# kylewray/epic

Measured on AMD Instinct MI355X. Metric: cell_updates_per_s_log_harmonic_relax_8192sq, higher is better.
Workload: dtype f32

## Files before the change

### epic_amd/csrc/driver.h

```cpp
#pragma once
#include <hip/hip_runtime.h>
#include <stdio.h>
#include <stdlib.h>
#include <string.h>

#include <algorithm>
#include <atomic>
#include <chrono>
#include <condition_variable>
#include <functional>
#include <map>
#include <string>
#include <thread>
#include <vector>
#include <mutex>
#include <tuple>
#include <unordered_map>

#include "../../include/epic/epic_abi.h"
#include "../../include/epic_hip.h"
#include "driver_config.h"
#include "kernels.h"

namespace epic_drv __attribute__((visibility("hidden"))) {

using epic::Harmonic;

struct DeviceGuard {
    int prev = -1;
    DeviceGuard() { if (hipGetDevice(&prev) != hipSuccess) { (void)hipGetLastError(); prev = -1; } }
    ~DeviceGuard() { if (prev >= 0) (void)hipSetDevice(prev); }
};
struct Crew;

struct Track {
    uint32_t *wake = nullptr;
    int phase = 0, rpt = 0, force = 2;
    size_t tiles = 0;
    static constexpr size_t kL = epic_hip::kWakeListCount, kCS = epic_hip::kWakeCounterStride;
    uint32_t *counter(int set) const { return wake + kL * kCS * set; }
    unsigned long long *total() const { return reinterpret_cast<unsigned long long *>(wake + 3 * kL * kCS); }
    uint32_t *queued(int i) const { return wake + 3 * kL * kCS + 2 + (size_t)i * tiles; }
    uint32_t *list(int i) const { return wake + 3 * kL * kCS + 2 + 2 * tiles + (size_t)i * kL * epic_hip::sweep_2d_list_cap(tiles); }
    static size_t words(size_t tiles) { return 3 * kL * kCS + 2 + 2 * tiles + 2 * kL * epic_hip::sweep_2d_list_cap(tiles); }
    static size_t zeroed_words(size_t tiles) { return 3 * kL * kCS + 2 + 2 * tiles; }
    void release()
    {
        if (wake) (void)hipFree(wake);
        wake = nullptr;
        tiles = 0;
    }
    epic_hip::Activity next(size_t tiles_now, int rpt_now, hipStream_t stream, bool *changed)
    {
        epic_hip::Activity act = {nullptr, nullptr, nullptr, nullptr, nullptr, nullptr, nullptr, nullptr};
        if (tiles_now != tiles || rpt_now != rpt) {
            if (changed) *changed = true;
            release();
            if (hipMalloc((void **)&wake, words(tiles_now) * sizeof(uint32_t)) == hipSuccess &&
                hipMemsetAsync(wake, 0, zeroed_words(tiles_now) * sizeof(uint32_t), stream) == hipSuccess) {
                tiles = tiles_now;
                rpt = rpt_now;
                phase = 0;
                force = 2;
            } else {
                (void)hipGetLastError();
                release();
            }
        }
        if (tiles) {
            const int li = phase & 1, ci = phase % 3;
            act.list_in = force > 0 ? nullptr : list(li);
            act.count_in = counter(ci);
            act.list_out = list(li ^ 1);
            act.count_out = counter((ci + 1) % 3);
            act.count_zero = counter((ci + 2) % 3);
            act.queued_in = queued(li);
            act.queued_out = queued(li ^ 1);
            act.total = total();
        }
        return act;
    }
    void advance()
    {
        phase = (phase + 1) % 6;
        if (force > 0) force--;
    }
    epic_hip::Activity upcoming() const
    {
        epic_hip::Activity act = {nullptr, nullptr, nullptr, nullptr, nullptr, nullptr, nullptr, nullptr};
        if (tiles) {
            act.list_out = list(phase & 1);
            act.count_out = counter(phase % 3);
            act.queued_out = queued(phase & 1);
        }
        return act;
    }
};

struct Ctx {
    int n = 0;
    int m[4] = {0, 0, 0, 0};
    int rows = 0;
    int cols = 0;
    int pitch = 0;
    float *buf[2] = {nullptr, nullptr};
    int cur = 0;
    uint32_t *maskw = nullptr;
    unsigned *d_m = nullptr;
    unsigned *d_delta = nullptr;
    float *h_delta = nullptr;
    float *h_tile_delta = nullptr;
    int tile_delta_n = 0;
    float *spare = nullptr;
    hipEvent_t ev_blk[2] = {nullptr, nullptr};
    hipStream_t stream = nullptr;
    int rows_per_task = 0;
    int tuned_rows[3] = {0, 0, 0};
    unsigned finish_from = 0;
    int math = 0;
    struct Replay { hipGraphExec_t exec; int cur_flip; double work; int tile_delta_n; };
    std::map<std::tuple<unsigned, int, int, int, int, int, int>, Replay> graphs;
    bool graphs_broken = false;
    int track_mode = 2;
    bool track = false;
    Track trk;
    Track trk_f;
    int last_lists = 0;
    unsigned seq_next = 0;
    bool seq_valid = false;
    int pair_rows = 0;
    static constexpr size_t kL = Track::kL, kCS = Track::kCS;
    double work_full = 0.0;
    bool redblack = true;
    struct Slab {
        int dev = 0;
        int lo = 0, hi = 0;
        int g_top = 0, g_bot = 0;
        int rows = 0;
        float *buf[2] = {nullptr, nullptr};
        uint32_t *maskw = nullptr;
        unsigned *d_delta = nullptr;
        float *h_delta = nullptr;
        hipStream_t stream = nullptr, comm = nullptr;
        hipEvent_t ev_prev = nullptr, ev_band = nullptr, ev_comm = nullptr, ev_stage = nullptr;
        Track trk;
        Track trk_f;
        bool peer_up = true;
        float *bounce[2] = {nullptr, nullptr};
        int first() const { return g_top; }
        int last() const { return rows - 1 - g_bot; }
        int top() const { return lo - g_top; }
    };
    std::vector<Slab> slabs;
    struct Probe { hipEvent_t int0 = nullptr, int1 = nullptr, cp0 = nullptr, cp1 = nullptr; };
    std::vector<Probe> probe;
    bool plan_failed = false;
    int slab_n = 0;
    Crew *crew = nullptr;
    std::vector<int> devices;
    int halo = 8, since = 0;
    int halo_env = 0;
    Config cfg;
    unsigned pending = 0, pending_first = 0, pending_cap = 1;
    bool defer_bypass = false;
    struct Ahead { bool live = false; unsigned first = 0, count = 0; } ahead;
    unsigned tick_plain = 0;
    bool multi() const { return !slabs.empty(); }
    size_t u_bytes() const { return (size_t)rows * pitch * sizeof(float); }
    static size_t mask_words_both_2d(int rows, int pitch) { return epic_hip::mask_words_2d(rows, pitch) + epic_hip::mask_words_fused_2d(rows, pitch); }
    size_t mask_bytes() const
    {
        if (n == 4) return 64;
        return sizeof(uint32_t) * (n == 2 ? mask_words_both_2d(rows, pitch) : epic_hip::mask_words_3d(m[0], m[1], pitch));
    }
    uint32_t *maskf() const { return n == 2 && maskw ? maskw + epic_hip::mask_words_2d(rows, pitch) : nullptr; }
    uint32_t *maskf(const Slab &sl) const { return sl.maskw ? sl.maskw + epic_hip::mask_words_2d(sl.rows, pitch) : nullptr; }
};

constexpr float kTolFinishOptionalBelow = 1e-5f;
constexpr size_t kTileDeltaCap = 4096;

void report(const char *fn, const char *msg);
void free_spare(Ctx *c);
Ctx *find_ctx(Harmonic *h);
bool dims_from(const Harmonic *h, Ctx *c);
bool dims_into_ctx(const Harmonic *h, Ctx *c);
bool same_dims(const Harmonic *h, const Ctx *c);
Ctx *get_ctx(Harmonic *h, bool create);
void drop_ctx_if_empty(Harmonic *h);
bool ready(const Harmonic *h, const Ctx *c);
float *current_u(const Ctx *c);
bool has_delta(const Ctx *c);
int upload_u(Harmonic *h, Ctx *c, const char *fn);
int upload_locked(Harmonic *h, Ctx *c, const char *fn);
void apply_config(Ctx *c);

void resolve_tracking(Ctx *c);
int auto_rows_per_task(const Ctx *c);
int fused_rows_per_task(const Ctx *c);
long long fuse_from_cells(const Ctx *c);
long long tile_up_to_cells(const Ctx *c);
long long tracked_pairs_from_cells(const Ctx *c);
bool fuses_tol(const Ctx *c);
bool fuses_jacobi(const Ctx *c);
bool fuses_rb_tol(const Ctx *c);
bool fuses_rb_precise(const Ctx *c);
int jacobi_fused_rows_per_task(const Ctx *c);
void tune_fused_rows(Ctx *c, int kind, unsigned iteration);
epic_hip::TilePlan tile_plan(const Ctx *c);
bool tile_checks(const Ctx *c, const epic_hip::TilePlan &tp);
bool rb_pairs_tracked(const Ctx *c);
bool rb_pairs_tracked_multi(const Ctx *c);
int rb_pairs_rows_per_task(const Ctx *c);
void rb_pairs_choose_rows(Ctx *c);
bool bypass_lists_for_batch(Ctx *c, bool pairs = false);
const char *plain_batch_path(const Ctx *c);

void note_iterations(Ctx *c, unsigned first, unsigned count);
hipError_t enqueue_sweep(Ctx *c, bool check, unsigned iteration);
hipError_t enqueue_check_sweep(Ctx *c, unsigned iteration);
void fold_listed_work(Ctx *c);
void drop_graphs(Ctx *c);
hipError_t enqueue_plain_run(Ctx *c, unsigned count, unsigned first, bool check_last = false);
hipError_t enqueue_rb_pairs_tracked(Ctx *c, unsigned npairs, unsigned first, bool check_last, bool bypass);
hipError_t enqueue_plain_batch(Ctx *c, unsigned count, unsigned first, bool check_last = false);
bool tiles_pipeline_ready(Ctx *c);
hipError_t enqueue_ahead(Ctx *c, unsigned first);
int read_tile_delta(Harmonic *h, Ctx *c, const char *fn, hipEvent_t after = nullptr);
int read_delta(Harmonic *h, Ctx *c, const char *fn);
void force_all(Ctx *c);
bool due_tiles(Ctx *c, unsigned long long *due, unsigned long long *tiles, bool forced_runs_all);

int run_block(Harmonic *h, Ctx *c, unsigned plain, unsigned first, bool check, const char *fn, int bypass, bool run_ahead = false);
inline bool jacobi_reference_checks(const Ctx *c) { return c->cfg.jacobi_ref_checks && !c->redblack && c->n != 4; }
unsigned defer_cap(const Harmonic *h, const Ctx *c);
int flush_pending(Harmonic *h, Ctx *c, const char *fn);

bool multi_plan(Ctx *c);
void multi_destroy(Ctx *c);
bool multi_holds_anything(const Ctx *c);
bool multi_ready(const Ctx *c);
void multi_sync(Ctx *c);
void multi_free_u(Ctx *c);
void multi_free_mask(Ctx *c);
void multi_free_delta(Ctx *c);
size_t unit_floats(const Ctx *c);
size_t unit_rows(const Ctx *c);
size_t slab_mask_words(const Ctx *c, const Ctx::Slab &sl);
bool multi_has_threads(const Ctx *c);
hipError_t multi_sweep(Ctx *c, bool check, unsigned iteration);
hipError_t multi_run(Ctx *c, unsigned count, unsigned first, bool check_first);
hipError_t multi_run_pairs(Ctx *c, unsigned npairs, unsigned first, bool check_last);
int multi_read_delta(Harmonic *h, Ctx *c, const char *fn);
int multi_upload_u(Harmonic *h, Ctx *c, const char *fn);
int multi_upload_locked(Harmonic *h, Ctx *c, const char *fn);
int multi_get_values(Harmonic *h, Ctx *c, const char *fn);
int multi_set_cells(Ctx *c, unsigned k, const unsigned *v, const unsigned *types, const char *fn);

}
```

### epic_amd/csrc/driver_config.cpp

```cpp
#include "driver_config.h"

#include <stdio.h>
#include <stdlib.h>
#include <string.h>

#include <memory>
#include <mutex>

namespace epic_drv {

namespace {
bool g_study = false;
std::mutex g_ignored_mu;
bool g_ignored_said = false;
const char *env(const char *name) { return getenv(name); }
const char *senv(const char *name)
{
    const char *v = getenv(name);
    if (v && !g_study) {
        std::lock_guard<std::mutex> lk(g_ignored_mu);
        if (!g_ignored_said) {
            g_ignored_said = true;
            fprintf(stderr, "Warning[epic_hip]: %s is a study knob and is ignored without EPIC_HIP_STUDY=1 (INTEGRATION.md section 6); further ones are not reported.\n", name);
        }
        return nullptr;
    }
    return v;
}
bool given(const char *name) { return env(name) != nullptr; }
bool sgiven(const char *name) { return senv(name) != nullptr; }
bool is_zero(const char *name) { const char *e = env(name); return e && e[0] == '0'; }
bool sis_zero(const char *name) { const char *e = senv(name); return e && e[0] == '0'; }
int sint_of(const char *name, int dflt) { const char *e = senv(name); return e ? atoi(e) : dflt; }
}

Config Config::from_env()
{
    Config c;
    {
        const char *st = env("EPIC_HIP_STUDY");
        c.study = g_study = st != nullptr && st[0] != '0';
    }
    const char *e = env("EPIC_HIP_MATH");
    if (e && strcmp(e, "fast") == 0) c.math = 1;
    if (e && strcmp(e, "tol") == 0) c.math = 4;
    e = env("EPIC_HIP_SCHEME");
    if (e && strcmp(e, "redblack") == 0) c.redblack = true;
    if (e && strcmp(e, "jacobi") == 0) c.redblack = false;
    e = env("EPIC_HIP_JACOBI_CHECKS");
    c.jacobi_ref_checks = e && (strcmp(e, "reference") == 0 || strcmp(e, "1") == 0);
    e = env("EPIC_HIP_TRACK");
    if (e && (strcmp(e, "0") == 0 || strcmp(e, "1") == 0)) c.track_mode = atoi(e);
    c.rows_per_task = sint_of("EPIC_HIP_ROWS_PER_TASK", 0);
    e = env("EPIC_HIP_HALO");
    if (e && atoi(e) >= 1) c.halo = atoi(e);
    e = env("EPIC_HIP_DEVICES");
    if (e && *e) {
        c.devices_text = e;
        for (const char *p = e; *p;) {
            char *end = nullptr;
            const long d = strtol(p, &end, 10);
            if (end == p || d < 0 || d > 1023) { c.devices_malformed = true; break; }
            c.devices.push_back((int)d);
            p = (*end == ',') ? end + 1 : end;
            if (*end && *end != ',') { c.devices_malformed = true; break; }
        }
        if (c.devices.size() > 64) c.devices_malformed = true;
        if (c.devices_malformed) c.devices.clear();
    }
    c.no_peer = given("EPIC_HIP_NO_PEER");
    e = env("EPIC_HIP_THREADS");
    c.threads = !(e && atoi(e) == 0);
    e = env("EPIC_HIP_SPIN_US");
    if (e && atoi(e) >= 0) c.spin_us = atoi(e) > 100000 ? 100000 : atoi(e);
    c.no_fuse = sgiven("EPIC_HIP_NO_FUSE");
    c.no_graph = sgiven("EPIC_HIP_NO_GRAPH");
    e = senv("EPIC_HIP_FUSE_MIN_CELLS");
    if (e && atoll(e) >= 0) c.fuse_min_cells = atoll(e);
    e = senv("EPIC_HIP_FUSED_ROWS");
    if (e && atoi(e) > 0) c.fused_rows = atoi(e);
    c.tune = !sis_zero("EPIC_HIP_TUNE");
    c.tune_debug = sgiven("EPIC_HIP_TUNE_DEBUG");
    c.tile = !sis_zero("EPIC_HIP_TILE");
    e = senv("EPIC_HIP_TILE_MAX_CELLS");
    if (e && atoll(e) >= 0) c.tile_max_cells = atoll(e);
    c.tile_rows = sint_of("EPIC_HIP_TILE_ROWS", 0);
    c.tile_width = sint_of("EPIC_HIP_TILE_WIDTH", 0);
    e = senv("EPIC_HIP_TILE_HALO");
    if (e && atoi(e) > 0) c.tile_halo = atoi(e);
    c.tile_pipeline = !sis_zero("EPIC_HIP_TILE_PIPELINE");
    c.defer = !is_zero("EPIC_HIP_DEFER");
    c.track_pairs = !sis_zero("EPIC_HIP_TRACK_PAIRS");
    e = senv("EPIC_HIP_TRACK_PAIR_ROWS");
    if (e && atoi(e) > 0) c.track_pair_rows = atoi(e);
    e = senv("EPIC_HIP_TRACK_SWITCH");
    if (e) c.track_switch = atof(e);
    e = env("EPIC_HIP_TOL_FINISH");
    if (e) c.tol_finish = e[0] == '0' ? 0 : 1;
    e = senv("EPIC_HIP_TOL_FINISH_FACTOR");
    if (e) {
        const float v = (float)atof(e);
        if (v >= 1.0f && v <= 1e9f) c.tol_finish_factor = v;
    }
    c.launch.flags = sint_of("EPIC_HIP_FLAGS", 7);
    e = senv("EPIC_HIP_LIST_WAVES");
    if (e && atol(e) >= 4) c.launch.list_waves = (size_t)atol(e);
    c.launch.pair3d = !sis_zero("EPIC_HIP_3D_PAIR");
    e = senv("EPIC_HIP_3D_PAIR_ROWS");
    if (e && atoi(e) > 0) c.launch.pair3d_rows = atoi(e);
    e = senv("EPIC_HIP_3D_MARCH");
    c.launch.march_x0 = e && e[0] == 'x' && e[1] == '0';
    return c;
}

std::string Config::json() const
{
    std::string dev;
    for (char ch : devices_text.substr(0, 256)) {
        if (ch == '"' || ch == '\\') { dev += '\\'; dev += ch; }
        else if ((unsigned char)ch < 0x20) dev += ' ';
        else dev += ch;
    }
    char t[1536];
    std::string out = "{";
    snprintf(t, sizeof t, "\"study\": %s, \"math\": %d, \"scheme\": \"%s\", \"jacobi_checks\": \"%s\", \"track_mode\": %d, \"rows_per_task\": %d, \"devices\": \"",
             study ? "true" : "false", math, redblack ? "redblack" : "jacobi", jacobi_ref_checks ? "reference" : "jacobi", track_mode, rows_per_task);
    out += t;
    out += dev;
    snprintf(t, sizeof t,
             "\", \"halo\": %d, \"no_peer\": %s, "
             "\"threads\": %s, \"spin_us\": %d, \"no_fuse\": %s, \"no_graph\": %s, \"fuse_min_cells\": %lld, \"fused_rows\": %d, \"tune\": %s, "
             "\"tile\": %s, \"tile_max_cells\": %lld, \"tile_rows\": %d, \"tile_width\": %d, \"tile_halo\": %d, \"tile_pipeline\": %s, \"defer\": %s, "
             "\"track_pairs\": %s, \"track_pair_rows\": %d, \"track_switch\": %g, \"tol_finish\": %d, \"tol_finish_factor\": %g, "
             "\"flags\": %d, \"list_waves\": %zu, \"pair3d\": %s, \"pair3d_rows\": %d, \"march_x0\": %s}",
             halo, no_peer ? "true" : "false",
             threads ? "true" : "false", spin_us, no_fuse ? "true" : "false", no_graph ? "true" : "false", fuse_min_cells, fused_rows,
             tune ? "true" : "false", tile ? "true" : "false", tile_max_cells, tile_rows, tile_width, tile_halo, tile_pipeline ? "true" : "false",
             defer ? "true" : "false",
             track_pairs ? "true" : "false", track_pair_rows, track_switch, tol_finish, (double)tol_finish_factor, launch.flags, launch.list_waves,
             launch.pair3d ? "true" : "false", launch.pair3d_rows, launch.march_x0 ? "true" : "false");
    out += t;
    return out;
}

namespace {
std::mutex g_process_mu;
Config *g_process = nullptr;
std::vector<std::unique_ptr<Config>> g_process_all;
}

void reload_process_config()
{
    std::unique_ptr<Config> fresh(new Config(Config::from_env()));
    std::lock_guard<std::mutex> lk(g_process_mu);
    g_process = fresh.get();
    g_process_all.push_back(std::move(fresh));
}

const Config &process_config()
{
    {
        std::lock_guard<std::mutex> lk(g_process_mu);
        if (g_process) return *g_process;
    }
    reload_process_config();
    std::lock_guard<std::mutex> lk(g_process_mu);
    return *g_process;
}

}

namespace epic_hip {
const LaunchKnobs &process_launch_knobs() { return epic_drv::process_config().launch; }
}
```

### epic_amd/csrc/driver_config.h

```cpp
#pragma once
#include <stddef.h>

#include <string>
#include <vector>

namespace epic_hip {
struct LaunchKnobs {
    int flags = 7;
    size_t list_waves = 0;
    bool pair3d = true;
    int pair3d_rows = 0;
    bool march_x0 = false;
};
const LaunchKnobs &process_launch_knobs();
}

namespace epic_drv {

struct Config {
    bool study = false;
    int math = 0;
    bool redblack = true;
    bool jacobi_ref_checks = false;
    int track_mode = 2;
    int rows_per_task = 0;
    std::string devices_text;
    std::vector<int> devices;
    bool devices_malformed = false;
    int halo = 0;
    bool no_peer = false;
    bool threads = true;
    int spin_us = 20;
    bool no_fuse = false;
    bool no_graph = false;
    long long fuse_min_cells = -1;
    int fused_rows = 0;
    bool tune = true;
    bool tune_debug = false;
    bool tile = true;
    long long tile_max_cells = -1;
    int tile_rows = 0, tile_width = 0, tile_halo = 0;
    bool tile_pipeline = true;
    bool defer = true;
    bool track_pairs = true;
    int track_pair_rows = 0;
    double track_switch = -1.0;
    int tol_finish = -1;
    float tol_finish_factor = 0.0f;
    epic_hip::LaunchKnobs launch;

    static Config from_env();
    std::string json() const;
};

const Config &process_config();
void reload_process_config();

}
```

### epic_amd/csrc/driver_enqueue.hip

```cpp
#include "driver.h"

namespace epic_drv {

static void expect_iteration(Ctx *c, unsigned first)
{
    if (c->track && c->redblack && c->seq_valid && ((first ^ c->seq_next) & 1u)) {
        force_all(c);
        c->seq_valid = false;
    }
}
void note_iterations(Ctx *c, unsigned first, unsigned count)
{
    expect_iteration(c, first);
    c->seq_next = first + count;
    c->seq_valid = true;
}

hipError_t enqueue_sweep(Ctx *c, bool check, unsigned iteration)
{
    if (c->n == 4) return hipSuccess;
    if (c->multi()) return multi_sweep(c, check, iteration);
    note_iterations(c, iteration, 1);
    hipError_t e;
    if (check) {
        e = hipMemsetAsync(c->d_delta, 0, sizeof(unsigned), c->stream);
        if (e != hipSuccess) return e;
    }
    const float *in = c->buf[c->cur];
    float *out = c->buf[c->cur ^ 1];
    epic_hip::Activity act = {nullptr, nullptr, nullptr, nullptr, nullptr, nullptr, nullptr, nullptr};
    if (c->track) {
        const int rpt = c->n == 2 ? auto_rows_per_task(c) : 32;
        const size_t tiles = c->n == 2 ? epic_hip::sweep_2d_tiles(c->rows, c->pitch, rpt)
                                       : epic_hip::sweep_3d_tiles(c->m[0], c->m[1], c->pitch);
        if (tiles != c->trk.tiles || rpt != c->trk.rpt) {
            drop_graphs(c);
            fold_listed_work(c);
        }
        if (c->last_lists == 2) c->trk.force = std::max(c->trk.force, 1);
        act = c->trk.next(tiles, rpt, c->stream, nullptr);
        c->last_lists = act.list_out ? 1 : 0;
    }
    if (!act.list_in) c->work_full += 1.0;
    auto advance = [&](hipError_t e) {
        if (e == hipSuccess && act.list_out) c->trk.advance();
        return e;
    };
    if (c->redblack) {
        float *inout = c->buf[c->cur];
        if (c->n == 2)
            return advance(epic_hip::launch_sweep_2d(inout, inout, c->maskw, c->rows, c->pitch, 0, c->rows,
                                                     auto_rows_per_task(c), c->math, (int)(iteration & 1u),
                                                     check ? c->d_delta : nullptr, c->stream, &act));
        return advance(epic_hip::launch_sweep_3d(inout, inout, c->maskw, c->m[0], c->m[1], c->pitch, 0, c->m[0], c->math,
                                                 (int)(iteration & 1u), check ? c->d_delta : nullptr, c->stream, &act, -1, -1, &c->cfg.launch));
    }
    if (c->n == 2)
        e = advance(epic_hip::launch_sweep_2d(in, out, c->maskw, c->rows, c->pitch, 0, c->rows, auto_rows_per_task(c),
                                              c->math, -1, check ? c->d_delta : nullptr, c->stream, &act));
    else
        e = advance(epic_hip::launch_sweep_3d(in, out, c->maskw, c->m[0], c->m[1], c->pitch, 0, c->m[0], c->math, -1,
                                              check ? c->d_delta : nullptr, c->stream, &act, -1, -1, &c->cfg.launch));
    if (e == hipSuccess) c->cur ^= 1;
    return e;
}

hipError_t enqueue_check_sweep(Ctx *c, unsigned iteration)
{
    if (!jacobi_reference_checks(c)) return enqueue_sweep(c, true, iteration);
    c->redblack = true;
    force_all(c);
    const hipError_t e = enqueue_sweep(c, true, iteration);
    c->redblack = false;
    force_all(c);
    return e;
}

void fold_listed_work(Ctx *c)
{
    auto fold = [&](Track &t, hipStream_t stream, double share) {
        if (!t.wake || t.tiles == 0) return;
        unsigned long long n = 0;
        if (hipStreamSynchronize(stream) == hipSuccess && hipMemcpy(&n, t.total(), sizeof n, hipMemcpyDeviceToHost) == hipSuccess &&
            hipMemset(t.total(), 0, sizeof n) == hipSuccess)
            c->work_full += share * (double)n / (double)t.tiles;
        else
            (void)hipGetLastError();
    };
    if (!c->multi()) {
        fold(c->trk, c->stream, 1.0);
        fold(c->trk_f, c->stream, 2.0);
        return;
    }
    DeviceGuard g;
    const int units = c->n == 2 ? c->rows : c->m[0];
    for (auto &sl : c->slabs)
        if (hipSetDevice(sl.dev) == hipSuccess) {
            fold(sl.trk, sl.stream, (double)sl.rows / (double)units);
            fold(sl.trk_f, sl.stream, 2.0 * (double)sl.rows / (double)units);
        }
}

void drop_graphs(Ctx *c)
{
    for (auto &g : c->graphs) (void)hipGraphExecDestroy(g.second.exec);
    c->graphs.clear();
}

hipError_t enqueue_plain_run(Ctx *c, unsigned count, unsigned first, bool check_last)
{
    if (c->n == 4) return check_last ? hipErrorInvalidValue : hipSuccess;
    if (c->multi()) return check_last ? hipErrorInvalidValue : multi_run(c, count, first, false);
    const epic_hip::TilePlan tp = tile_plan(c);
    if (check_last && !tile_checks(c, tp)) return hipErrorInvalidValue;
    if (tp.halo > 0 && (count >= 2 || check_last)) {
        const unsigned total = count + (check_last ? 1u : 0u);
        for (unsigned i = 0; i < total;) {
            const unsigned k = std::min<unsigned>(total - i, (unsigned)tp.halo);
            hipError_t e = epic_hip::launch_tile_2d(c->buf[c->cur], c->buf[c->cur ^ 1], c->maskw, c->rows, c->pitch, tp, (int)k, c->math,
                                                    c->redblack ? (int)((first + i) & 1u) : -1, nullptr, c->stream,
                                                    check_last && i + k == total ? c->h_tile_delta : nullptr);
            if (e != hipSuccess) return e;
            c->cur ^= 1;
            c->work_full += (double)k;
            i += k;
        }
        if (check_last) c->tile_delta_n = tp.tiles_r * tp.tiles_c;
        return hipSuccess;
    }
    const bool no_fuse = c->cfg.no_fuse;
    const bool fuse = fuses_rb_precise(c);
    unsigned i = 0;
    if (!no_fuse && fuses_jacobi(c)) {
        if (count >= 2) tune_fused_rows(c, 0, first);
        while (i < count) {
            if (count - i >= 2) {
                hipError_t e = epic_hip::launch_jacobi_fused_2d(c->buf[c->cur], c->buf[c->cur ^ 1], c->maskw, c->rows, c->pitch,
                                                                jacobi_fused_rows_per_task(c), c->math, c->stream, -1, c->maskf());
                if (e != hipSuccess) return e;
                c->cur ^= 1;
                c->work_full += 2.0;
                i += 2;
            } else {
                hipError_t e = enqueue_sweep(c, false, first + i);
                if (e != hipSuccess) return e;
                i++;
            }
        }
        return hipSuccess;
    }
    if (!no_fuse && fuses_rb_tol(c) && count - i >= 2) tune_fused_rows(c, 1, first);
    if (fuse && count - i >= 2) tune_fused_rows(c, 2, first);
    while (!no_fuse && fuses_rb_tol(c) && count - i >= 2) {
        hipError_t e = epic_hip::launch_jacobi_fused_2d(c->buf[c->cur], c->buf[c->cur ^ 1], c->maskw, c->rows, c->pitch,
                                                        jacobi_fused_rows_per_task(c), c->math, c->stream, (int)((first + i) & 1u),
                                                        c->maskf());
        if (e != hipSuccess) return e;
        c->cur ^= 1;
        c->work_full += 2.0;
        i += 2;
    }
    while (fuse && count - i >= 2) {
        hipError_t e = epic_hip::launch_rb_fused_2d(c->buf[c->cur], c->buf[c->cur ^ 1], c->maskw, c->rows, c->pitch,
                                                    fused_rows_per_task(c), c->math, (int)((first + i) & 1u), c->stream, c->maskf());
        if (e != hipSuccess) return e;
        c->cur ^= 1;
        c->work_full += 2.0;
        i += 2;
    }
    for (; i < count; i++) {
        hipError_t e = enqueue_sweep(c, false, first + i);
        if (e != hipSuccess) return e;
    }
    return hipSuccess;
}

hipError_t enqueue_rb_pairs_tracked(Ctx *c, unsigned npairs, unsigned first, bool check_last, bool bypass)
{
    note_iterations(c, first, 2 * npairs);
    const bool tol = c->math == 4;
    const int rpt = !bypass ? rb_pairs_rows_per_task(c) : tol ? jacobi_fused_rows_per_task(c) : fused_rows_per_task(c);
    const size_t tiles = epic_hip::rb_fused_2d_tiles(c->rows, c->pitch, rpt);
    for (unsigned p = 0; p < npairs; ++p) {
        const bool check = check_last && p + 1 == npairs;
        hipError_t e;
        if (check && (e = hipMemsetAsync(c->d_delta, 0, sizeof(unsigned), c->stream)) != hipSuccess) return e;
        epic_hip::Activity act = {nullptr, nullptr, nullptr, nullptr, nullptr, nullptr, nullptr, nullptr};
        if (!bypass) {
            if (tiles != c->trk_f.tiles || rpt != c->trk_f.rpt) fold_listed_work(c);
            if (c->last_lists != 2) c->trk_f.force = std::max(c->trk_f.force, 1);
            act = c->trk_f.next(tiles, rpt, c->stream, nullptr);
        }
        const int parity = (int)((first + 2 * p) & 1u);
        e = tol ? epic_hip::launch_jacobi_fused_2d(c->buf[c->cur], c->buf[c->cur ^ 1], c->maskw, c->rows, c->pitch, rpt, c->math, c->stream,
                                                   c->redblack ? parity : -1, c->maskf(), act.list_out ? &act : nullptr, check ? c->d_delta : nullptr)
                : epic_hip::launch_rb_fused_2d(c->buf[c->cur], c->buf[c->cur ^ 1], c->maskw, c->rows, c->pitch, rpt, c->math, parity, c->stream,
                                               c->maskf(), act.list_out ? &act : nullptr, check ? c->d_delta : nullptr);
        if (e != hipSuccess) return e;
        if (!act.list_in) c->work_full += 2.0;
        if (act.list_out) { c->trk_f.advance(); c->last_lists = 2; }
        else c->last_lists = 0;
        c->cur ^= 1;
    }
    return hipSuccess;
}

hipError_t enqueue_plain_batch(Ctx *c, unsigned count, unsigned first, bool check_last)
{
    if (c->n == 4) return enqueue_plain_run(c, count, first, check_last);
    expect_iteration(c, first);
    const bool small = (long long)c->rows * c->pitch <= (1ll << 22);
    const bool no_graph = c->cfg.no_graph;
    if (!small || count < 8 || no_graph || c->multi() || (c->track && (c->trk.force > 0 || c->trk.tiles == 0)))
        return enqueue_plain_run(c, count, first, check_last);
    const epic_hip::TilePlan tp = tile_plan(c);
    if (tp.halo > 0 && count + (check_last ? 1u : 0u) <= (unsigned)tp.halo) return enqueue_plain_run(c, count, first, check_last);
    const int fuse_cfg = tp.halo > 0 ? -((tp.halo * 1024 + tp.tile_rows) * 4 + tp.tile_cols / 64) : fuses_tol(c) ? jacobi_fused_rows_per_task(c) : 0;
    const auto key = std::make_tuple(2u * count + (check_last ? 1u : 0u), c->cur + 2 * (c->track ? 1 + c->trk.phase : 0), (int)(first & 1u), c->math,
                                     (int)c->redblack, auto_rows_per_task(c), fuse_cfg);
    if (c->graphs_broken) return enqueue_plain_run(c, count, first, check_last);
    auto it = c->graphs.find(key);
    if (it == c->graphs.end()) {
        const int cur0 = c->cur, phase0 = c->trk.phase, force0 = c->trk.force;
        const double work0 = c->work_full;
        hipGraph_t graph = nullptr;
        hipGraphExec_t exec = nullptr;
        hipError_t e = hipStreamBeginCapture(c->stream, hipStreamCaptureModeThreadLocal);
        if (e == hipSuccess) {
            e = enqueue_plain_run(c, count, first, check_last);
            hipError_t e2 = hipStreamEndCapture(c->stream, &graph);
            if (e == hipSuccess) e = e2;
        }
        const int cur_flip = c->cur ^ cur0;
        c->cur = cur0;
        c->trk.phase = phase0;
        c->trk.force = force0;
        const double work = c->work_full - work0;
        c->work_full = work0;
        if (e == hipSuccess) e = hipGraphInstantiate(&exec, graph, nullptr, nullptr, 0);
        if (graph) (void)hipGraphDestroy(graph);
        if (e != hipSuccess) {
            (void)hipGetLastError();
            c->graphs_broken = true;
            return enqueue_plain_run(c, count, first, check_last);
        }
        if (c->graphs.size() >= 16) drop_graphs(c);
        it = c->graphs.emplace(key, Ctx::Replay{exec, cur_flip, work, check_last ? c->tile_delta_n : 0}).first;
    }
    hipError_t e = hipGraphLaunch(it->second.exec, c->stream);
    if (e != hipSuccess) {
        (void)hipGetLastError();
        c->graphs_broken = true;
        return enqueue_plain_run(c, count, first, check_last);
    }
    c->seq_next = first + count + (check_last ? 1u : 0u);
    c->seq_valid = true;
    c->cur ^= it->second.cur_flip;
    c->work_full += it->second.work;
    if (check_last) c->tile_delta_n = it->second.tile_delta_n;
    if (c->track) c->trk.phase = (int)((c->trk.phase + count) % 6);
    return hipSuccess;
}

bool tiles_pipeline_ready(Ctx *c)
{
    if (!c->cfg.tile_pipeline) return false;
    for (hipEvent_t &ev : c->ev_blk)
        if (!ev && hipEventCreateWithFlags(&ev, hipEventDisableTiming) != hipSuccess) {
            (void)hipGetLastError();
            ev = nullptr;
            return false;
        }
    if (!c->spare) {
        if (hipMalloc((void **)&c->spare, c->u_bytes()) != hipSuccess) {
            (void)hipGetLastError();
            c->spare = nullptr;
            return false;
        }
        if (epic_hip::launch_fill(c->spare, (size_t)c->rows * c->pitch, -1e6f, c->stream) != hipSuccess) {
            (void)hipGetLastError();
            free_spare(c);
            return false;
        }
    }
    return true;
}

hipError_t enqueue_ahead(Ctx *c, unsigned first)
{
    c->ahead.live = false;
    const epic_hip::TilePlan tp = tile_plan(c);
    if (tp.halo <= 0 || !c->spare) return hipErrorInvalidValue;
    hipError_t e = epic_hip::launch_tile_2d(c->buf[c->cur], c->spare, c->maskw, c->rows, c->pitch, tp, tp.halo, c->math,
                                            c->redblack ? (int)(first & 1u) : -1, nullptr, c->stream, nullptr);
    if (e != hipSuccess) return e;
    c->ahead.live = true;
    c->ahead.first = first;
    c->ahead.count = (unsigned)tp.halo;
    return hipSuccess;
}

int read_tile_delta(Harmonic *h, Ctx *c, const char *fn, hipEvent_t after)
{
    hipError_t e = hipSuccess;
    if (after) {
        const auto until = std::chrono::steady_clock::now() + std::chrono::microseconds(200);
        do e = hipEventQuery(after);
        while (e == hipErrorNotReady && std::chrono::steady_clock::now() < until);
        if (e == hipErrorNotReady) { (void)hipGetLastError(); e = hipEventSynchronize(after); }
    } else {
        e = hipStreamSynchronize(c->stream);
    }
    if (e != hipSuccess) {
        report(fn, "Failed to synchronize the device after the 'update and check' kernel.");
        return EPIC_ERROR_DEVICE_SYNCHRONIZE;
    }
    float d = 0.0f;
    for (int t = 0; t < c->tile_delta_n; ++t) d = std::max(d, c->h_tile_delta[t]);
    h->delta = d;
    return EPIC_SUCCESS;
}

int read_delta(Harmonic *h, Ctx *c, const char *fn)
{
    if (c->n == 4) return EPIC_SUCCESS;
    if (c->multi()) return multi_read_delta(h, c, fn);
    if (hipMemcpyAsync(c->h_delta, c->d_delta, sizeof(float), hipMemcpyDeviceToHost, c->stream) != hipSuccess) {
        report(fn, "Failed to copy memory from device to host for the max delta.");
        return EPIC_ERROR_MEMCPY_TO_HOST;
    }
    if (hipStreamSynchronize(c->stream) != hipSuccess) {
        report(fn, "Failed to synchronize the device after the 'update and check' kernel.");
        return EPIC_ERROR_DEVICE_SYNCHRONIZE;
    }
    h->delta = *c->h_delta;
    return EPIC_SUCCESS;
}

void force_all(Ctx *c)
{
    c->trk.force = 2;
    c->trk_f.force = std::max(c->trk_f.force, 1);
    c->last_lists = 0;
    for (auto &sl : c->slabs) {
        sl.trk.force = 2;
        sl.trk_f.force = std::max(sl.trk_f.force, 1);
    }
}

bool due_tiles(Ctx *c, unsigned long long *due, unsigned long long *tiles, bool forced_runs_all)
{
    *due = *tiles = 0;
    auto one = [&](const Track &t) {
        if (t.tiles == 0) return false;
        uint32_t counts[Ctx::kL * Ctx::kCS];
        if (hipMemcpy(counts, t.counter(t.phase % 3), sizeof(counts), hipMemcpyDeviceToHost) != hipSuccess) {
            (void)hipGetLastError();
            return false;
        }
        unsigned long long d = 0;
        for (size_t i = 0; i < Ctx::kL; i++) d += counts[i * Ctx::kCS];
        *due += (forced_runs_all && t.force > 0) ? t.tiles : d;
        *tiles += t.tiles;
        return true;
    };
    if (!c->multi()) return one(c->last_lists == 2 ? c->trk_f : c->trk);
    DeviceGuard g;
    for (auto &sl : c->slabs)
        if (hipSetDevice(sl.dev) != hipSuccess || hipStreamSynchronize(sl.stream) != hipSuccess || !one(c->last_lists == 2 ? sl.trk_f : sl.trk)) return false;
    return true;
}

}
```

### epic_amd/csrc/driver_multi.hip

```cpp
#include "driver.h"

namespace epic_drv {

struct Crew {
    int spin_us = 20;
    template <class F> void spin_for(F done) const
    {
        if (spin_us <= 0 || done()) return;
        const auto until = std::chrono::steady_clock::now() + std::chrono::microseconds(spin_us);
        for (;;) {
            for (int i = 0; i < 32; i++) {
                if (done()) return;
                __builtin_ia32_pause();
            }
            if (std::chrono::steady_clock::now() >= until) return;
        }
    }
    std::vector<std::thread> threads;
    std::mutex mu;
    std::condition_variable cv_go, cv_done;
    std::atomic<unsigned> generation{0};
    std::atomic<int> pending{0};
    std::function<hipError_t(int)> job;
    std::vector<hipError_t> result;
    bool quit = false;

    void start(const std::vector<int> &devices)
    {
        result.assign(devices.size(), hipSuccess);
        for (size_t k = 0; k < devices.size(); k++)
            threads.emplace_back([this, k, dev = devices[k]] {
                (void)hipSetDevice(dev);
                unsigned seen = 0;
                for (;;) {
                    spin_for([&] { return generation.load(std::memory_order_acquire) != seen; });
                    if (generation.load(std::memory_order_acquire) == seen) {
                        std::unique_lock<std::mutex> lk(mu);
                        cv_go.wait(lk, [&] { return generation.load(std::memory_order_acquire) != seen; });
                    }
                    seen = generation.load(std::memory_order_acquire);
                    if (quit) return;
                    result[k] = job((int)k);
                    if (pending.fetch_sub(1, std::memory_order_acq_rel) == 1) {
                        std::lock_guard<std::mutex> lk(mu);
                        cv_done.notify_all();
                    }
                }
            });
    }
    hipError_t run(std::function<hipError_t(int)> f)
    {
        {
            std::lock_guard<std::mutex> lk(mu);
            job = std::move(f);
            pending.store((int)threads.size(), std::memory_order_release);
            generation.fetch_add(1, std::memory_order_acq_rel);
        }
        cv_go.notify_all();
        spin_for([&] { return pending.load(std::memory_order_acquire) == 0; });
        if (pending.load(std::memory_order_acquire) != 0) {
            std::unique_lock<std::mutex> lk(mu);
            cv_done.wait(lk, [&] { return pending.load(std::memory_order_acquire) == 0; });
        }
        for (hipError_t e : result)
            if (e != hipSuccess) return e;
        return hipSuccess;
    }
    void stop()
    {
        if (threads.empty()) return;
        {
            std::lock_guard<std::mutex> lk(mu);
            quit = true;
            generation.fetch_add(1, std::memory_order_acq_rel);
        }
        cv_go.notify_all();
        for (auto &t : threads) t.join();
        threads.clear();
    }
};

hipError_t for_each_slab(Ctx *c, const std::function<hipError_t(int)> &f)
{
    if (c->crew && !c->crew->threads.empty()) return c->crew->run(f);
    DeviceGuard g;
    for (int k = 0; k < (int)c->slabs.size(); k++) {
        hipError_t e = hipSetDevice(c->slabs[k].dev);
        if (e == hipSuccess) e = f(k);
        if (e != hipSuccess) return e;
    }
    return hipSuccess;
}

void multi_free_u(Ctx *c)
{
    for (auto &sl : c->slabs) {
        (void)hipSetDevice(sl.dev);
        if (sl.stream) (void)hipStreamSynchronize(sl.stream);
        if (sl.comm) (void)hipStreamSynchronize(sl.comm);
        for (float *&b : sl.buf) { if (b) (void)hipFree(b); b = nullptr; }
    }
}
void multi_free_mask(Ctx *c)
{
    for (auto &sl : c->slabs) {
        (void)hipSetDevice(sl.dev);
        if (sl.stream) (void)hipStreamSynchronize(sl.stream);
        if (sl.maskw) (void)hipFree(sl.maskw);
        sl.maskw = nullptr;
    }
}
void multi_free_delta(Ctx *c)
{
    for (auto &sl : c->slabs) {
        (void)hipSetDevice(sl.dev);
        if (sl.stream) (void)hipStreamSynchronize(sl.stream);
        if (sl.d_delta) (void)hipFree(sl.d_delta);
        sl.d_delta = nullptr;
    }
}
bool multi_holds_anything(const Ctx *c)
{
    for (const auto &sl : c->slabs)
        if (sl.buf[0] || sl.maskw || sl.d_delta) return true;
    return false;
}
void multi_destroy(Ctx *c)
{
    DeviceGuard g;
    if (c->crew) { c->crew->stop(); delete c->crew; c->crew = nullptr; }
    multi_free_u(c); multi_free_mask(c); multi_free_delta(c);
    for (auto &sl : c->slabs) {
        (void)hipSetDevice(sl.dev);
        sl.trk.release();
        sl.trk_f.release();
        if (sl.stream) (void)hipStreamDestroy(sl.stream);
        if (sl.comm) (void)hipStreamDestroy(sl.comm);
        for (hipEvent_t e : {sl.ev_prev, sl.ev_band, sl.ev_comm, sl.ev_stage}) if (e) (void)hipEventDestroy(e);
        if (sl.h_delta) (void)hipHostFree(sl.h_delta);
        for (float *&b : sl.bounce) { if (b) (void)hipHostFree(b); b = nullptr; }
    }
    c->slabs.clear();
}

bool multi_plan(Ctx *c)
{
    const int want = (int)c->devices.size();
    const int units = c->n == 2 ? c->rows : c->m[0];
    const bool multi = want >= 2 && (c->n == 2 || c->n == 3) && units >= 4 * want;
    c->plan_failed = false;
    if (!multi) {
        if (!c->slabs.empty() && !multi_holds_anything(c)) multi_destroy(c);
        return false;
    }
    if ((int)c->slabs.size() == want && c->slabs.back().hi == units && c->slab_n == c->n) return true;
    if (!c->slabs.empty()) multi_destroy(c);
    c->tuned_rows[0] = c->tuned_rows[1] = c->tuned_rows[2] = 0;
    DeviceGuard g;
    const int base = units / want, rem = units % want;
    const int want_halo = c->halo_env > 0 ? c->halo_env : c->n == 3 ? 2 : base >= 4096 ? 8 : base >= 2048 ? 16 : 32;
    const int halo = std::max(1, std::min(want_halo, base / 2));
    const bool no_peer = c->cfg.no_peer;
    int lo = 0;
    c->slabs.resize(want);
    for (int k = 0; k < want; k++) {
        Ctx::Slab &sl = c->slabs[k];
        sl.dev = c->devices[k];
        sl.lo = lo;
        sl.hi = lo + base + (k < rem ? 1 : 0);
        lo = sl.hi;
        sl.g_top = k > 0 ? halo : 0;
        sl.g_bot = k < want - 1 ? halo : 0;
        sl.rows = (sl.hi - sl.lo) + sl.g_top + sl.g_bot;
        bool ok = hipSetDevice(sl.dev) == hipSuccess &&
                  hipStreamCreateWithFlags(&sl.stream, hipStreamNonBlocking) == hipSuccess &&
                  hipStreamCreateWithFlags(&sl.comm, hipStreamNonBlocking) == hipSuccess &&
                  hipEventCreateWithFlags(&sl.ev_prev, hipEventDisableTiming) == hipSuccess &&
                  hipEventCreateWithFlags(&sl.ev_band, hipEventDisableTiming) == hipSuccess &&
                  hipEventCreateWithFlags(&sl.ev_comm, hipEventDisableTiming) == hipSuccess &&
                  hipEventCreateWithFlags(&sl.ev_stage, hipEventDisableTiming) == hipSuccess &&
                  hipHostMalloc((void **)&sl.h_delta, 64, hipHostMallocPortable) == hipSuccess;
        if (!ok) {
            (void)hipGetLastError();
            multi_destroy(c);
            c->plan_failed = true;
            return false;
        }
        sl.peer_up = true;
        if (k > 0) {
            Ctx::Slab &up = c->slabs[k - 1];
            bool direct = !no_peer;
            if (direct && up.dev != sl.dev) {
                auto enable = [](int from, int to) {
                    int can = 0;
                    if (hipSetDevice(from) != hipSuccess || hipDeviceCanAccessPeer(&can, from, to) != hipSuccess || !can) {
                        (void)hipGetLastError();
                        return false;
                    }
                    const hipError_t e = hipDeviceEnablePeerAccess(to, 0);
                    (void)hipGetLastError();
                    return e == hipSuccess || e == hipErrorPeerAccessAlreadyEnabled;
                };
                direct = enable(sl.dev, up.dev) && enable(up.dev, sl.dev);
                (void)hipSetDevice(sl.dev);
                if (!direct)
                    fprintf(stderr, "Warning[epic_hip]: no peer access between devices %d and %d: halo units are staged through pinned host memory.\n",
                            up.dev, sl.dev);
            }
            sl.peer_up = direct;
            if (!direct) {
                const size_t bytes = (size_t)halo * (c->n == 2 ? 1 : c->m[1]) * c->pitch * sizeof(float);
                if (hipHostMalloc((void **)&sl.bounce[0], bytes, hipHostMallocPortable) != hipSuccess ||
                    hipHostMalloc((void **)&sl.bounce[1], bytes, hipHostMallocPortable) != hipSuccess) {
                    (void)hipGetLastError();
                    multi_destroy(c);
                    c->plan_failed = true;
                    return false;
                }
            }
        }
    }
    c->halo = halo;
    c->since = 0;
    c->slab_n = c->n;
    if (c->cfg.threads) {
        c->crew = new Crew();
        c->crew->spin_us = c->cfg.spin_us;
        c->crew->start(c->devices);
    }
    resolve_tracking(c);
    return true;
}

bool multi_ready(const Ctx *c)
{
    if (c->slabs.empty()) return false;
    for (const auto &sl : c->slabs)
        if (!sl.buf[0] || !sl.buf[1] || !sl.maskw) return false;
    return true;
}

void multi_sync(Ctx *c)
{
    for (auto &sl : c->slabs) {
        (void)hipSetDevice(sl.dev);
        (void)hipStreamSynchronize(sl.comm);
        (void)hipStreamSynchronize(sl.stream);
    }
}

size_t unit_floats(const Ctx *c) { return (size_t)(c->n == 2 ? 1 : c->m[1]) * c->pitch; }
size_t unit_rows(const Ctx *c) { return (size_t)(c->n == 2 ? 1 : c->m[1]); }

int multi_upload_u(Harmonic *h, Ctx *c, const char *fn)
{
    DeviceGuard g;
    for (auto &sl : c->slabs) {
        if (hipSetDevice(sl.dev) != hipSuccess) return EPIC_ERROR_DEVICE_MALLOC;
        for (int b = 0; b < 2; b++)
            if (epic_hip::launch_fill(sl.buf[b], (size_t)sl.rows * unit_floats(c), -1e6f, sl.stream) != hipSuccess) {
                report(fn, "Failed to initialise device-side memory for the potential values.");
                return EPIC_ERROR_KERNEL_EXECUTION;
            }
        if (hipStreamSynchronize(sl.stream) != hipSuccess) return EPIC_ERROR_DEVICE_SYNCHRONIZE;
        if (hipMemcpy2D(sl.buf[0], (size_t)c->pitch * sizeof(float), h->u + (size_t)sl.top() * unit_rows(c) * c->cols,
                        (size_t)c->cols * sizeof(float), (size_t)c->cols * sizeof(float), (size_t)sl.rows * unit_rows(c),
                        hipMemcpyHostToDevice) != hipSuccess) {
            report(fn, "Failed to copy memory from host to device for the potential values.");
            return EPIC_ERROR_MEMCPY_TO_DEVICE;
        }
        sl.trk.force = 2;
        sl.trk_f.force = std::max(sl.trk_f.force, 1);
    }
    c->cur = 0;
    c->since = 0;
    h->d_u = c->slabs[0].buf[0];
    return EPIC_SUCCESS;
}

size_t slab_mask_words(const Ctx *c, const Ctx::Slab &sl)
{
    return c->n == 2 ? Ctx::mask_words_both_2d(sl.rows, c->pitch) : epic_hip::mask_words_3d(sl.rows, c->m[1], c->pitch);
}

int multi_upload_locked(Harmonic *h, Ctx *c, const char *fn)
{
    DeviceGuard g;
    for (auto &sl : c->slabs) {
        if (hipSetDevice(sl.dev) != hipSuccess) return EPIC_ERROR_DEVICE_MALLOC;
        const size_t cells = (size_t)sl.rows * unit_rows(c) * c->cols;
        uint32_t *tmp = nullptr;
        if (hipMalloc((void **)&tmp, cells * sizeof(uint32_t)) != hipSuccess) {
            (void)hipGetLastError();
            report(fn, "Failed to allocate device-side staging memory for the locked cells.");
            return EPIC_ERROR_DEVICE_MALLOC;
        }
        int rc = EPIC_SUCCESS;
        if (hipMemcpy(tmp, h->locked + (size_t)sl.top() * unit_rows(c) * c->cols, cells * sizeof(uint32_t), hipMemcpyHostToDevice) != hipSuccess) {
            report(fn, "Failed to copy memory from host to device for the locked cells.");
            rc = EPIC_ERROR_MEMCPY_TO_DEVICE;
        } else {
            hipError_t e = c->n == 2 ? epic_hip::launch_pack_mask_2d(tmp, sl.rows, c->cols, c->pitch, sl.g_top > 0, sl.g_bot > 0, sl.maskw, sl.stream)
                                     : epic_hip::launch_pack_mask_3d(tmp, sl.rows, c->m[1], c->m[2], c->pitch, sl.maskw, sl.stream);
            if (e == hipSuccess && c->n == 2) e = epic_hip::launch_fuse_masks_2d(sl.maskw, sl.rows, c->pitch, c->maskf(sl), sl.stream);
            if (e != hipSuccess || hipStreamSynchronize(sl.stream) != hipSuccess) {
                report(fn, "Failed to execute the 'pack mask' kernel.");
                rc = EPIC_ERROR_KERNEL_EXECUTION;
            }
        }
        (void)hipFree(tmp);
        if (rc != EPIC_SUCCESS) return rc;
        sl.trk.force = 2;
        sl.trk_f.force = std::max(sl.trk_f.force, 1);
    }
    return EPIC_SUCCESS;
}

hipError_t multi_copy_units(const Ctx *c, Ctx::Slab &dst, float *dbuf, int dunit, Ctx::Slab &src, const float *sbuf, int sunit, int n,
                            hipEvent_t after, bool direct, float *bounce)
{
    const size_t bytes = (size_t)n * unit_floats(c) * sizeof(float);
    float *d = dbuf + (size_t)dunit * unit_floats(c);
    const float *sp = sbuf + (size_t)sunit * unit_floats(c);
    hipError_t e;
    if (direct) {
        if ((e = hipSetDevice(dst.dev)) != hipSuccess || (e = hipStreamWaitEvent(dst.comm, after, 0)) != hipSuccess) return e;
        return dst.dev == src.dev ? hipMemcpyAsync(d, sp, bytes, hipMemcpyDeviceToDevice, dst.comm)
                                  : hipMemcpyPeerAsync(d, dst.dev, sp, src.dev, bytes, dst.comm);
    }
    if ((e = hipSetDevice(src.dev)) != hipSuccess || (e = hipStreamWaitEvent(src.comm, after, 0)) != hipSuccess ||
        (e = hipMemcpyAsync(bounce, sp, bytes, hipMemcpyDeviceToHost, src.comm)) != hipSuccess ||
        (e = hipEventRecord(src.ev_stage, src.comm)) != hipSuccess)
        return e;
    if ((e = hipSetDevice(dst.dev)) != hipSuccess || (e = hipStreamWaitEvent(dst.comm, src.ev_stage, 0)) != hipSuccess) return e;
    return hipMemcpyAsync(d, bounce, bytes, hipMemcpyHostToDevice, dst.comm);
}

hipError_t slab_launch(Ctx *c, Ctx::Slab &sl, int lo, int hi, unsigned *d, int clo, int chi, unsigned iteration, hipStream_t st,
                       const epic_hip::Activity *act)
{
    float *src = sl.buf[c->cur], *dst = c->redblack ? src : sl.buf[c->cur ^ 1];
    const int parity = c->redblack ? (int)((iteration + (unsigned)sl.top()) & 1u) : -1;
    if (c->n == 2)
        return epic_hip::launch_sweep_2d(src, dst, sl.maskw, sl.rows, c->pitch, lo, hi, auto_rows_per_task(c), c->math, parity, d, st, act, clo, chi);
    return epic_hip::launch_sweep_3d(src, dst, sl.maskw, sl.rows, c->m[1], c->pitch, lo, hi, c->math, parity, d, st, act, clo, chi, &c->cfg.launch);
}

size_t slab_tiles(const Ctx *c, const Ctx::Slab &sl, int rpt)
{
    return c->n == 2 ? epic_hip::sweep_2d_tiles(sl.rows, c->pitch, rpt) : epic_hip::sweep_3d_tiles(sl.rows, c->m[1], c->pitch);
}

hipError_t multi_run(Ctx *c, unsigned count, unsigned first, bool check_first)
{
    const int G = c->halo;
    const bool tracked = c->track;
    const bool fuse_rb = !tracked && c->redblack && c->n == 2 && c->math != 4 && !c->cfg.no_fuse && (long long)c->rows * c->pitch >= (1ll << 22);
    const bool fuse = !tracked && (fuses_tol(c) || fuse_rb);
    const int rpt_track = c->n == 2 ? auto_rows_per_task(c) : 32;
    note_iterations(c, first, count);
    if (tracked) {
        if (c->last_lists == 2)
            for (auto &sl : c->slabs) sl.trk.force = std::max(sl.trk.force, 1);
        c->last_lists = 1;
    } else {
        c->last_lists = 0;
    }
    unsigned done = 0;
    while (done < count) {
        const unsigned calm = (unsigned)std::max(0, G - 1 - c->since);
        const unsigned n_calm = std::min(count - done, calm);
        if (n_calm > 0) {
            const unsigned it0 = first + done;
            const bool chk = check_first && done == 0;
            const int cur0 = c->cur;
            if (fuse && n_calm >= 2) tune_fused_rows(c, fuse_rb ? 2 : c->redblack ? 1 : 0, it0);
            const int fused_rpt = !fuse ? 0 : fuse_rb ? fused_rows_per_task(c) : jacobi_fused_rows_per_task(c);
            hipError_t e = for_each_slab(c, [&, it0, chk, cur0, fused_rpt, n_calm](int k) -> hipError_t {
                Ctx::Slab &sl = c->slabs[k];
                int cur = cur0;
                hipError_t e = hipSuccess;
                for (unsigned i = 0; i < n_calm && e == hipSuccess;) {
                    const bool check = chk && i == 0;
                    if (fuse && !check && n_calm - i >= 2) {
                        const int parity = c->redblack ? (int)((it0 + i + (unsigned)sl.top()) & 1u) : -1;
                        e = fuse_rb ? epic_hip::launch_rb_fused_2d(sl.buf[cur], sl.buf[cur ^ 1], sl.maskw, sl.rows, c->pitch, fused_rpt, c->math,
                                                                   parity, sl.stream, c->maskf(sl))
                                    : epic_hip::launch_jacobi_fused_2d(sl.buf[cur], sl.buf[cur ^ 1], sl.maskw, sl.rows, c->pitch, fused_rpt,
                                                                       c->math, sl.stream, parity, c->maskf(sl));
                        cur ^= 1;
                        i += 2;
                        continue;
                    }
                    if (check) e = hipMemsetAsync(sl.d_delta, 0, sizeof(unsigned), sl.stream);
                    epic_hip::Activity act = {nullptr, nullptr, nullptr, nullptr, nullptr, nullptr, nullptr, nullptr};
                    if (tracked) act = sl.trk.next(slab_tiles(c, sl, rpt_track), rpt_track, sl.stream, nullptr);
                    if (e == hipSuccess) {
                        float *src = sl.buf[cur], *dst = c->redblack ? src : sl.buf[cur ^ 1];
                        const int parity = c->redblack ? (int)((it0 + i + (unsigned)sl.top()) & 1u) : -1;
                        unsigned *d = check ? sl.d_delta : nullptr;
                        e = c->n == 2 ? epic_hip::launch_sweep_2d(src, dst, sl.maskw, sl.rows, c->pitch, 0, sl.rows, auto_rows_per_task(c), c->math,
                                                                  parity, d, sl.stream, &act, sl.first(), sl.last() + 1)
                                      : epic_hip::launch_sweep_3d(src, dst, sl.maskw, sl.rows, c->m[1], c->pitch, 0, sl.rows, c->math, parity, d,
                                                                  sl.stream, &act, sl.first(), sl.last() + 1, &c->cfg.launch);
                    }
                    if (e == hipSuccess && act.list_out) sl.trk.advance();
                    if (!c->redblack) cur ^= 1;
                    i++;
                }
                return e;
            });
            if (e != hipSuccess) return e;
            for (unsigned i = 0; i < n_calm;) {
                const bool check = chk && i == 0;
                if (fuse && !check && n_calm - i >= 2) { c->cur ^= 1; c->since += 2; c->work_full += tracked ? 0.0 : 2.0; i += 2; continue; }
                if (!c->redblack) c->cur ^= 1;
                c->since++;
                if (!tracked) c->work_full += 1.0;
                i++;
            }
            done += n_calm;
            if (done >= count) break;
        }
        const unsigned it = first + done;
        const bool check = check_first && done == 0;
        const int cur = c->cur;
        hipError_t e = for_each_slab(c, [&, it, check, cur](int k) -> hipError_t {
            Ctx::Slab &sl = c->slabs[k];
            hipError_t e = hipSuccess;
            auto fail = [&](hipError_t x) { if (e == hipSuccess && x != hipSuccess) e = x; return x != hipSuccess; };
            unsigned *d = check ? sl.d_delta : nullptr;
            if (check && fail(hipMemsetAsync(sl.d_delta, 0, sizeof(unsigned), sl.stream))) return e;
            (void)cur;
            if (tracked) {
                epic_hip::Activity act = sl.trk.next(slab_tiles(c, sl, rpt_track), rpt_track, sl.stream, nullptr);
                if (fail(slab_launch(c, sl, 0, sl.rows, d, sl.first(), sl.last() + 1, it, sl.stream, &act))) return e;
                if (act.list_out) sl.trk.advance();
                if (fail(hipEventRecord(sl.ev_band, sl.stream))) return e;
                return e;
            }
            const int top_hi = sl.g_top ? sl.first() + G : sl.first();
            const int bot_lo = sl.g_bot ? sl.last() + 1 - G : sl.last() + 1;
            const Ctx::Probe *pr = c->probe.empty() ? nullptr : &c->probe[k];
            if (fail(hipEventRecord(sl.ev_prev, sl.stream)) || fail(hipStreamWaitEvent(sl.comm, sl.ev_prev, 0))) return e;
            if (pr && fail(hipEventRecord(pr->cp0, sl.comm))) return e;
            if (sl.g_top && fail(slab_launch(c, sl, sl.first(), top_hi, d, -1, -1, it, sl.comm, nullptr))) return e;
            if (sl.g_bot && fail(slab_launch(c, sl, bot_lo, sl.last() + 1, d, -1, -1, it, sl.comm, nullptr))) return e;
            if (fail(hipEventRecord(sl.ev_band, sl.comm))) return e;
            if (pr && fail(hipEventRecord(pr->int0, sl.stream))) return e;
            if (fail(slab_launch(c, sl, top_hi, bot_lo, d, -1, -1, it, sl.stream, nullptr))) return e;
            if (pr && fail(hipEventRecord(pr->int1, sl.stream))) return e;
            return e;
        });
        if (e != hipSuccess) return e;
        e = for_each_slab(c, [&, cur](int k) -> hipError_t {
            Ctx::Slab &sl = c->slabs[k];
            const int out = c->redblack ? cur : cur ^ 1;
            hipError_t e = tracked ? hipStreamWaitEvent(sl.comm, sl.ev_band, 0) : hipSuccess;
            if (e == hipSuccess && k > 0) {
                Ctx::Slab &up = c->slabs[k - 1];
                e = multi_copy_units(c, sl, sl.buf[out], 0, up, up.buf[out], up.last() + 1 - G, G, up.ev_band, sl.peer_up, sl.bounce[0]);
            }
            if (e == hipSuccess && k + 1 < (int)c->slabs.size()) {
                Ctx::Slab &dn = c->slabs[k + 1];
                e = multi_copy_units(c, sl, sl.buf[out], sl.rows - G, dn, dn.buf[out], dn.first(), G, dn.ev_band, dn.peer_up, dn.bounce[1]);
            }
            if (e == hipSuccess) e = hipSetDevice(sl.dev);
            if (e == hipSuccess) e = hipEventRecord(sl.ev_comm, sl.comm);
            if (e == hipSuccess && !c->probe.empty() && !tracked) e = hipEventRecord(c->probe[k].cp1, sl.comm);
            return e;
        });
        if (e != hipSuccess) return e;
        e = for_each_slab(c, [&](int k) -> hipError_t {
            Ctx::Slab &sl = c->slabs[k];
            hipError_t e = hipStreamWaitEvent(sl.stream, sl.ev_comm, 0);
            if (e == hipSuccess && k > 0) e = hipStreamWaitEvent(sl.stream, c->slabs[k - 1].ev_comm, 0);
            if (e == hipSuccess && k + 1 < (int)c->slabs.size()) e = hipStreamWaitEvent(sl.stream, c->slabs[k + 1].ev_comm, 0);
            if (e == hipSuccess && tracked && sl.trk.tiles && sl.trk.force == 0) {
                const epic_hip::Activity next = sl.trk.upcoming();
                const int per_unit = c->n == 2 ? 0 : (int)(sl.trk.tiles / (size_t)sl.rows);
                auto wake_units = [&](int lo, int hi) {
                    lo = std::max(lo, 0);
                    hi = std::min(hi, sl.rows);
                    if (hi <= lo) return hipSuccess;
                    const int nstrips = c->pitch / 256;
                    const int t_lo = c->n == 2 ? (lo / sl.trk.rpt) * nstrips : lo * per_unit;
                    const int t_hi = c->n == 2 ? ((hi - 1) / sl.trk.rpt + 1) * nstrips : hi * per_unit;
                    return epic_hip::launch_wake_tile_range(&next, sl.trk.tiles, t_lo, t_hi, sl.stream);
                };
                if (sl.g_top) e = wake_units(0, G + 1);
                if (e == hipSuccess && sl.g_bot) e = wake_units(sl.rows - G - 1, sl.rows);
            }
            return e;
        });
        if (e != hipSuccess) return e;
        if (!c->redblack) c->cur ^= 1;
        c->since = 0;
        if (!tracked) c->work_full += 1.0;
        done++;
    }
    return hipSuccess;
}

hipError_t multi_run_pairs(Ctx *c, unsigned npairs, unsigned first, bool check_last)
{
    const int G = c->halo;
    if (c->n != 2 || G < 2) return hipErrorInvalidValue;
    note_iterations(c, first, 2 * npairs);
    const bool tol = c->math == 4;
    const int rpt = rb_pairs_rows_per_task(c);
    const int nstrips_f = epic_hip::fused_2d_strips(c->pitch);
    if (c->last_lists != 2)
        for (auto &sl : c->slabs) sl.trk_f.force = std::max(sl.trk_f.force, 1);
    c->last_lists = 2;
    auto exchange = [&]() -> hipError_t {
        const int cur = c->cur;
        hipError_t e = for_each_slab(c, [&, cur](int k) -> hipError_t {
            Ctx::Slab &sl = c->slabs[k];
            hipError_t e = hipStreamWaitEvent(sl.comm, sl.ev_band, 0);
            if (e == hipSuccess && k > 0) {
                Ctx::Slab &up = c->slabs[k - 1];
                e = multi_copy_units(c, sl, sl.buf[cur], 0, up, up.buf[cur], up.last() + 1 - G, G, up.ev_band, sl.peer_up, sl.bounce[0]);
            }
            if (e == hipSuccess && k + 1 < (int)c->slabs.size()) {
                Ctx::Slab &dn = c->slabs[k + 1];
                e = multi_copy_units(c, sl, sl.buf[cur], sl.rows - G, dn, dn.buf[cur], dn.first(), G, dn.ev_band, dn.peer_up, dn.bounce[1]);
            }
            if (e == hipSuccess) e = hipSetDevice(sl.dev);
            if (e == hipSuccess) e = hipEventRecord(sl.ev_comm, sl.comm);
            return e;
        });
        if (e != hipSuccess) return e;
        e = for_each_slab(c, [&](int k) -> hipError_t {
            Ctx::Slab &sl = c->slabs[k];
            hipError_t e = hipStreamWaitEvent(sl.stream, sl.ev_comm, 0);
            if (e == hipSuccess && k > 0) e = hipStreamWaitEvent(sl.stream, c->slabs[k - 1].ev_comm, 0);
            if (e == hipSuccess && k + 1 < (int)c->slabs.size()) e = hipStreamWaitEvent(sl.stream, c->slabs[k + 1].ev_comm, 0);
            if (e == hipSuccess && sl.trk_f.tiles && sl.trk_f.force == 0) {
                const epic_hip::Activity next = sl.trk_f.upcoming();
                auto wake_rows = [&](int lo, int hi) {
                    lo = std::max(lo, 0);
                    hi = std::min(hi, sl.rows);
                    if (hi <= lo) return hipSuccess;
                    return epic_hip::launch_wake_tile_range(&next, sl.trk_f.tiles, (lo / sl.trk_f.rpt) * nstrips_f, ((hi - 1) / sl.trk_f.rpt + 1) * nstrips_f, sl.stream);
                };
                if (sl.g_top) e = wake_rows(0, G + 2);
                if (e == hipSuccess && sl.g_bot) e = wake_rows(sl.rows - G - 2, sl.rows);
            }
            return e;
        });
        c->since = 0;
        return e;
    };
    auto record_bands = [&]() -> hipError_t {
        return for_each_slab(c, [&](int k) -> hipError_t { return hipEventRecord(c->slabs[k].ev_band, c->slabs[k].stream); });
    };
    unsigned p = 0;
    bool bands_recorded = false;
    while (p < npairs) {
        if (c->since + 2 > G) {
            hipError_t e = bands_recorded ? hipSuccess : record_bands();
            if (e == hipSuccess) e = exchange();
            if (e != hipSuccess) return e;
        }
        const unsigned n = std::min<unsigned>(npairs - p, (unsigned)((G - c->since) / 2));
        const unsigned it0 = first + 2 * p;
        const int cur0 = c->cur;
        const bool last_stretch = p + n == npairs;
        hipError_t e = for_each_slab(c, [&, n, it0, cur0, last_stretch](int k) -> hipError_t {
            Ctx::Slab &sl = c->slabs[k];
            const size_t tiles = epic_hip::rb_fused_2d_tiles(sl.rows, c->pitch, rpt);
            int cur = cur0;
            hipError_t e = hipSuccess;
            for (unsigned i = 0; i < n && e == hipSuccess; i++) {
                const bool check = check_last && last_stretch && i + 1 == n;
                if (check) e = hipMemsetAsync(sl.d_delta, 0, sizeof(unsigned), sl.stream);
                if (e != hipSuccess) break;
                epic_hip::Activity act = sl.trk_f.next(tiles, rpt, sl.stream, nullptr);
                const int parity = (int)((it0 + 2 * i + (unsigned)sl.top()) & 1u);
                e = tol ? epic_hip::launch_jacobi_fused_2d(sl.buf[cur], sl.buf[cur ^ 1], sl.maskw, sl.rows, c->pitch, rpt, c->math, sl.stream,
                                                           c->redblack ? parity : -1, c->maskf(sl), act.list_out ? &act : nullptr,
                                                           check ? sl.d_delta : nullptr, sl.first(), sl.last() + 1)
                        : epic_hip::launch_rb_fused_2d(sl.buf[cur], sl.buf[cur ^ 1], sl.maskw, sl.rows, c->pitch, rpt, c->math, parity, sl.stream,
                                                       c->maskf(sl), act.list_out ? &act : nullptr, check ? sl.d_delta : nullptr, sl.first(), sl.last() + 1);
                if (e == hipSuccess && act.list_out) sl.trk_f.advance();
                cur ^= 1;
            }
            if (e == hipSuccess) e = hipEventRecord(sl.ev_band, sl.stream);
            return e;
        });
        if (e != hipSuccess) return e;
        bands_recorded = true;
        if (n & 1u) c->cur ^= 1;
        c->since += 2 * (int)n;
        p += n;
    }
    if (c->since >= G) return exchange();
    return hipSuccess;
}

hipError_t multi_sweep(Ctx *c, bool check, unsigned iteration) { return multi_run(c, 1, iteration, check); }

int multi_read_delta(Harmonic *h, Ctx *c, const char *fn)
{
    DeviceGuard g;
    for (auto &sl : c->slabs) {
        if (hipSetDevice(sl.dev) != hipSuccess ||
            hipStreamSynchronize(sl.comm) != hipSuccess ||
            hipMemcpyAsync(sl.h_delta, sl.d_delta, sizeof(float), hipMemcpyDeviceToHost, sl.stream) != hipSuccess) {
            report(fn, "Failed to copy memory from device to host for the max delta.");
            return EPIC_ERROR_MEMCPY_TO_HOST;
        }
    }
    float d = 0.0f;
    for (auto &sl : c->slabs) {
        if (hipSetDevice(sl.dev) != hipSuccess || hipStreamSynchronize(sl.stream) != hipSuccess) {
            report(fn, "Failed to synchronize the device after the 'update and check' kernel.");
            return EPIC_ERROR_DEVICE_SYNCHRONIZE;
        }
        d = std::max(d, *sl.h_delta);
    }
    h->delta = d;
    return EPIC_SUCCESS;
}

int multi_get_values(Harmonic *h, Ctx *c, const char *fn)
{
    DeviceGuard g;
    multi_sync(c);
    for (auto &sl : c->slabs) {
        if (hipSetDevice(sl.dev) != hipSuccess ||
            hipMemcpy2D(h->u + (size_t)sl.lo * unit_rows(c) * c->cols, (size_t)c->cols * sizeof(float),
                        sl.buf[c->cur] + (size_t)sl.first() * unit_floats(c), (size_t)c->pitch * sizeof(float),
                        (size_t)c->cols * sizeof(float), (size_t)(sl.hi - sl.lo) * unit_rows(c), hipMemcpyDeviceToHost) != hipSuccess) {
            report(fn, "Failed to copy memory from device to host for the potential values.");
            return EPIC_ERROR_MEMCPY_TO_HOST;
        }
    }
    return EPIC_SUCCESS;
}

int multi_set_cells(Ctx *c, unsigned k, const unsigned *v, const unsigned *types, const char *fn)
{
    DeviceGuard g;
    multi_sync(c);
    int rc = EPIC_SUCCESS;
    for (auto &sl : c->slabs) {
        unsigned *d_v = nullptr, *d_types = nullptr;
        sl.trk.force = 2;
        sl.trk_f.force = std::max(sl.trk_f.force, 1);
        if (hipSetDevice(sl.dev) != hipSuccess || hipMalloc((void **)&d_v, 2 * (size_t)k * sizeof(unsigned)) != hipSuccess ||
            hipMalloc((void **)&d_types, (size_t)k * sizeof(unsigned)) != hipSuccess) {
            (void)hipGetLastError();
            report(fn, "Failed to allocate device-side memory for the cell locations and types.");
            rc = EPIC_ERROR_DEVICE_MALLOC;
        } else if (hipMemcpyAsync(d_v, v, 2 * (size_t)k * sizeof(unsigned), hipMemcpyHostToDevice, sl.stream) != hipSuccess ||
                   hipMemcpyAsync(d_types, types, (size_t)k * sizeof(unsigned), hipMemcpyHostToDevice, sl.stream) != hipSuccess) {
            report(fn, "Failed to copy memory from host to device for the cell locations and types.");
            rc = EPIC_ERROR_MEMCPY_TO_DEVICE;
        } else if (epic_hip::launch_set_cells_2d(sl.buf[c->cur], sl.maskw, sl.rows, c->cols, c->pitch, k, d_v, d_types, sl.stream,
                                                 sl.top(), c->rows, sl.g_top > 0, sl.g_bot > 0) != hipSuccess ||
                   epic_hip::launch_fuse_masks_2d(sl.maskw, sl.rows, c->pitch, c->maskf(sl), sl.stream) != hipSuccess) {
            report(fn, "Failed to execute the 'set cells' kernel.");
            rc = EPIC_ERROR_KERNEL_EXECUTION;
        }
        if (hipStreamSynchronize(sl.stream) != hipSuccess && rc == EPIC_SUCCESS) rc = EPIC_ERROR_DEVICE_SYNCHRONIZE;
        if (d_v) (void)hipFree(d_v);
        if (d_types) (void)hipFree(d_types);
        if (rc != EPIC_SUCCESS) break;
    }
    return rc;
}

bool multi_has_threads(const Ctx *c) { return c->crew && !c->crew->threads.empty(); }

}
```

### epic_amd/csrc/driver_plan.hip

```cpp
#include "driver.h"

namespace epic_drv {

void resolve_tracking(Ctx *c)
{
    c->track = c->n != 4 && (c->track_mode == 1 || (c->track_mode == 2 && (long long)c->rows * c->pitch > (1ll << 22)));
}

int auto_rows_per_task(const Ctx *c)
{
    if (c->rows_per_task > 0) return c->rows_per_task;
    const long long nstrips = (c->pitch + 255) / 256;
    long long r = (long long)c->rows * nstrips / 32768;
    constexpr int trip = epic_hip::kTolTripRows;
    if (c->math == 4 && (long long)c->rows / trip * nstrips >= 6144) return trip;
    if (r >= 8) r = r / 8 * 8;
    else if (r >= 4) r = 4;
    else if (r >= 2) r = 2;
    else r = 1;
    return (int)std::min<long long>(64, r);
}

int fused_rows_per_task(const Ctx *c)
{
    if (c->rows_per_task > 0) return std::max(c->rows_per_task, 4);
    if (c->tuned_rows[2] > 0) return c->tuned_rows[2];
    const long long nstrips = epic_hip::fused_2d_strips(c->pitch);
    long long r = (long long)c->rows * nstrips / 8192 / 8 * 8;
    return (int)std::min<long long>(64, std::max<long long>(16, r));
}

long long fuse_from_cells(const Ctx *c)
{
    if (c->cfg.fuse_min_cells >= 0) return c->cfg.fuse_min_cells;
    if (c->math == 4) return c->redblack ? (2ll << 20) : (3ll << 19);
    return 11ll << 19;
}
long long tile_up_to_cells(const Ctx *c)
{
    if (c->cfg.tile_max_cells >= 0) return c->cfg.tile_max_cells;
    if (c->math != 4 && !c->redblack) return 5ll << 17;
    return 3ll << 20;
}
long long tracked_pairs_from_cells(const Ctx *c) { return c->cfg.fuse_min_cells >= 0 ? c->cfg.fuse_min_cells : (1ll << 22); }

bool fuses_tol(const Ctx *c)
{
    if (c->cfg.no_fuse) return false;
    return c->n == 2 && !c->track && c->math == 4 && (long long)c->rows * c->pitch >= fuse_from_cells(c);
}
bool fuses_jacobi(const Ctx *c) { return !c->redblack && fuses_tol(c); }
bool fuses_rb_precise(const Ctx *c)
{
    return c->redblack && c->n == 2 && !c->cfg.no_fuse && !c->track && c->math != 4 && (long long)c->rows * c->pitch >= fuse_from_cells(c);
}
bool fuses_rb_tol(const Ctx *c) { return c->redblack && fuses_tol(c); }

int jacobi_fused_rows_per_task(const Ctx *c)
{
    if (c->cfg.fused_rows > 0) return c->cfg.fused_rows;
    const int tuned = c->tuned_rows[c->redblack ? 1 : 0];
    if (tuned > 0) return tuned;
    const long long rows = c->multi() ? c->rows / (long long)c->slabs.size() : c->rows;
    return epic_hip::jacobi_fused_auto_rows((int)rows, c->pitch);
}

void tune_fused_rows(Ctx *c, int kind, unsigned iteration)
{
    if (c->tuned_rows[kind] != 0) return;
    if (iteration < (unsigned)std::min(c->rows, c->cols) / 2) return;
    c->tuned_rows[kind] = -1;
    if (!c->cfg.tune || c->n != 2 || c->rows_per_task > 0 || c->cfg.fused_rows > 0) return;
    const bool multi = c->multi();
    DeviceGuard restore_device;
    if (multi && hipSetDevice(c->slabs[0].dev) != hipSuccess) { (void)hipGetLastError(); return; }
    const int rows = multi ? c->slabs[0].rows : c->rows;
    const hipStream_t stream = multi ? c->slabs[0].stream : c->stream;
    const float *in = multi ? c->slabs[0].buf[c->cur] : c->buf[c->cur];
    float *out = multi ? c->slabs[0].buf[c->cur ^ 1] : c->buf[c->cur ^ 1];
    const uint32_t *maskw = multi ? c->slabs[0].maskw : c->maskw, *maskf = multi ? c->maskf(c->slabs[0]) : c->maskf();
    if ((long long)rows * c->pitch < (1ll << 22)) return;
    hipStreamCaptureStatus cap = hipStreamCaptureStatusNone;
    if (hipStreamIsCapturing(stream, &cap) != hipSuccess || cap != hipStreamCaptureStatusNone) { c->tuned_rows[kind] = 0; return; }
    const int dflt = kind == 2 ? fused_rows_per_task(c) : jacobi_fused_rows_per_task(c);
    hipEvent_t e0 = nullptr, e1 = nullptr;
    if (hipEventCreate(&e0) != hipSuccess) return;
    if (hipEventCreate(&e1) != hipSuccess) { (void)hipEventDestroy(e0); return; }
    auto launch = [&](int height) -> hipError_t {
        if (kind == 2) return epic_hip::launch_rb_fused_2d(in, out, maskw, rows, c->pitch, height, c->math, 0, stream, maskf);
        return epic_hip::launch_jacobi_fused_2d(in, out, maskw, rows, c->pitch, height, c->math, stream, kind == 1 ? 0 : -1, maskf);
    };
    auto timed = [&](int height, float *ms) -> bool {
        if (launch(height) != hipSuccess) return false;
        if (hipEventRecord(e0, stream) != hipSuccess) return false;
        for (int i = 0; i < 2; ++i)
            if (launch(height) != hipSuccess) return false;
        return hipEventRecord(e1, stream) == hipSuccess && hipEventSynchronize(e1) == hipSuccess &&
               hipEventElapsedTime(ms, e0, e1) == hipSuccess;
    };
    static const int kCandidates[] = {20, 23, 26, 29, 32, 35, 38, 40, 41, 43, 46, 49, 52, 58, 64, 80, 96, 128};
    const bool say = c->cfg.tune_debug;
    float best_ms = 0.0f, dflt_ms = 0.0f;
    int best = 0;
    bool ok = timed(dflt, &dflt_ms);
    if (say && ok) fprintf(stderr, "[epic_hip tune] kind %d, %d x %d%s: rule %d rows %.1f us", kind, rows, c->cols, multi ? " (first slab)" : "", dflt, dflt_ms * 500.0f);
    for (int r : kCandidates) {
        if (!ok) break;
        if (r == dflt || r > rows) continue;
        float ms = 0.0f;
        ok = timed(r, &ms);
        if (say && ok) fprintf(stderr, ", %d: %.1f", r, ms * 500.0f);
        if (ok && (best == 0 || ms < best_ms)) { best = r; best_ms = ms; }
    }
    if (say) fprintf(stderr, "\n");
    (void)hipEventDestroy(e0);
    (void)hipEventDestroy(e1);
    if (!ok) { (void)hipGetLastError(); return; }
    c->tuned_rows[kind] = (best > 0 && best_ms < 0.99f * dflt_ms) ? best : dflt;
}

epic_hip::TilePlan tile_plan(const Ctx *c)
{
    epic_hip::TilePlan none = {0, 0, 0, 0, 0};
    if (c->n != 2 || c->multi() || c->track || c->math == 2) return none;
    if (fuses_tol(c)) return none;
    if (!c->cfg.tile) return none;
    if ((long long)c->rows * c->cols > tile_up_to_cells(c)) return none;
    const int want_rows = c->cfg.tile_rows;
    const int only_width = c->cfg.tile_width;
    const int only_halo = c->cfg.tile_halo;
    epic_hip::TilePlan best = none;
    double best_cost = 0.0;
    for (int width : {epic_hip::kTile2dCols, epic_hip::kTile2dWideCols}) {
        if (only_width && width != only_width) continue;
        const int max_rows = epic_hip::tile_2d_max_rows(c->math, c->redblack, width);
        if (max_rows == 0) continue;
        for (int halo : {8, 10, 12, 14, 16}) {
            if (only_halo && halo != only_halo && halo != 8) continue;
            const int h = only_halo ? only_halo : halo;
            const epic_hip::TilePlan p = epic_hip::tile_2d_plan(c->rows, c->cols, h, want_rows, width, max_rows);
            if (p.halo == 0) continue;
            const int s_r = p.tile_rows + 2 * h;
            const double units = (c->redblack ? s_r / 2.0 : (double)s_r) * (width / 64), per_simd = units / 4.0;
            const double rounds = std::max(1.0, (double)p.tiles_r * p.tiles_c / 256.0);
            const double step = std::max(0.84 + 0.055 * per_simd, 0.2 + (c->math == 4 ? 0.17 : 0.21) * per_simd);
            const double cost = (rounds > 1.0 ? 1.6 * rounds / 2.0 + 0.2 : 1.0) * ((2.7 + 0.00006 * s_r * width) / h + step);
            if (best.halo == 0 || cost < best_cost) { best = p; best_cost = cost; }
            if (only_halo) break;
        }
    }
    return best;
}

bool tile_checks(const Ctx *c, const epic_hip::TilePlan &tp)
{
    return tp.halo > 0 && c->h_tile_delta != nullptr && (size_t)tp.tiles_r * tp.tiles_c <= kTileDeltaCap;
}

bool rb_pairs_tracked(const Ctx *c)
{
    if (!c->track || c->n != 2 || c->multi() || c->math == 2) return false;
    if (!c->redblack && c->math != 4) return false;
    if (c->cfg.no_fuse || !c->cfg.track_pairs) return false;
    return (long long)c->rows * c->pitch >= tracked_pairs_from_cells(c);
}

bool rb_pairs_tracked_multi(const Ctx *c)
{
    if (!c->track || c->n != 2 || !c->multi() || c->halo < 2 || c->math == 2) return false;
    if (!c->redblack && c->math != 4) return false;
    if (c->cfg.no_fuse || !c->cfg.track_pairs) return false;
    return (long long)c->rows * c->pitch >= tracked_pairs_from_cells(c);
}

int rb_pairs_rows_per_task(const Ctx *c)
{
    if (c->cfg.track_pair_rows > 0) return std::max(c->cfg.track_pair_rows, 2);
    if (c->rows_per_task > 0) return std::max(c->rows_per_task, 2);
    return c->pair_rows > 0 ? c->pair_rows : 16;
}

void rb_pairs_choose_rows(Ctx *c)
{
    if (c->cfg.track_pair_rows > 0 || c->rows_per_task > 0) return;
    if (c->pair_rows == 0) c->pair_rows = 16;
    if (c->last_lists != 2) return;
    unsigned long long due = 0, tiles = 0;
    if (!due_tiles(c, &due, &tiles, false) || tiles == 0) return;
    const double share = (double)due / (double)tiles;
    if (c->pair_rows == 16 && share < 0.04) c->pair_rows = 4;
    else if (c->pair_rows == 4 && share > 0.20) c->pair_rows = 16;
}

bool bypass_lists_for_batch(Ctx *c, bool pairs)
{
    if (!c->track || c->track_mode != 2 || c->n != 2) return false;
    if (pairs && c->last_lists != 2) return false;
    const double given = c->cfg.track_switch;
    const bool tol = c->math == 4;
    const double rule = pairs ? 0.85 : c->redblack ? (tol ? 0.45 : 0.6) : (tol ? 0.7 : 0.85);
    const double limit = given >= 0.0 ? given : rule;
    unsigned long long due = 0, tiles = 0;
    if (!due_tiles(c, &due, &tiles, false) || tiles == 0) return false;
    return (double)due > limit * (double)tiles;
}

const char *plain_batch_path(const Ctx *c)
{
    if (c->n == 4) return "none (n = 4: a counting no-op)";
    if (c->multi()) {
        if (rb_pairs_tracked_multi(c)) return c->math == 4 ? "slabs: tracked pairs of list-driven fused tol passes per slab" : "slabs: tracked pairs of list-driven fused red-black passes per slab";
        if (c->track) return "slabs: list-driven single sweeps per slab";
        if (fuses_tol(c)) return c->redblack ? "slabs: fused tol red-black pairs between exchanges" : "slabs: fused tol Jacobi pairs between exchanges";
        if (c->redblack && c->n == 2 && c->math != 4 && !c->cfg.no_fuse && (long long)c->rows * c->pitch >= (1ll << 22)) return "slabs: fused red-black pairs between exchanges";
        return c->n == 3 ? "slabs of planes: single 3-D sweeps" : "slabs: single sweeps";
    }
    if (rb_pairs_tracked(c)) return c->math == 4 ? "tracked pairs of list-driven fused tol passes" : "tracked pairs of list-driven fused red-black passes";
    const epic_hip::TilePlan tp = tile_plan(c);
    if (tp.halo > 0) return tile_checks(c, tp) ? (c->cfg.tile_pipeline ? "LDS tiles, several iterations per launch, check folded in, pipelined blocks" : "LDS tiles, several iterations per launch, check folded in")
                                               : "LDS tiles, several iterations per launch";
    if (fuses_jacobi(c)) return "fused tol Jacobi pairs (jacobi_fused2d_kernel)";
    if (fuses_rb_tol(c)) return "fused tol red-black pairs (rb_tol_fused2d_kernel)";
    if (fuses_rb_precise(c)) return "fused red-black pairs (rb_fused2d_kernel)";
    if (c->track) return c->n == 3 ? "list-driven single 3-D sweeps" : "list-driven single sweeps";
    if (c->n == 3) return c->math == 4 && c->cfg.launch.pair3d ? "single 3-D sweeps, two planes per wave (sweep3d_pair_kernel)" : "single 3-D sweeps (sweep3d_kernel)";
    const bool graphs = (long long)c->rows * c->pitch <= (1ll << 22) && !c->cfg.no_graph && !c->graphs_broken;
    return graphs ? "single sweeps replayed from a captured hipGraph" : "single sweeps";
}

}
```

### epic_amd/csrc/driver_registry.hip

```cpp
#include "driver.h"

namespace epic_drv {

std::mutex g_mu;
std::unordered_map<Harmonic *, Ctx *> g_ctx;

void report(const char *fn, const char *msg) { fprintf(stderr, "Error[%s]: %s\n", fn, msg); }

void free_spare(Ctx *c)
{
    if (c->spare) (void)hipFree(c->spare);
    c->spare = nullptr;
}

Ctx *find_ctx(Harmonic *h)
{
    std::lock_guard<std::mutex> lk(g_mu);
    auto it = g_ctx.find(h);
    return it == g_ctx.end() ? nullptr : it->second;
}

bool dims_from(const Harmonic *h, Ctx *c)
{
    if (h->n != 2 && h->n != 3 && h->n != 4) return false;
    for (unsigned i = 0; i < h->n; i++)
        if (h->m[i] < (h->n == 4 ? 1u : 3u) || h->m[i] > (1u << 30)) return false;
    c->n = (int)h->n;
    for (unsigned i = 0; i < 4; i++) c->m[i] = i < h->n ? (int)h->m[i] : 0;
    c->cols = c->m[c->n - 1];
    long long rows = 1;
    for (int i = 0; i + 1 < c->n; i++) {
        rows *= c->m[i];
        if (rows > 0x7fffffffLL) return false;
    }
    c->rows = (int)rows;
    c->pitch = epic_hip::pitch_for_cols(c->cols);
    resolve_tracking(c);
    return true;
}

bool dims_into_ctx(const Harmonic *h, Ctx *c)
{
    const int rows0 = c->rows, cols0 = c->cols, n0 = c->n;
    if (!dims_from(h, c)) return false;
    if (c->rows != rows0 || c->cols != cols0 || c->n != n0) c->tuned_rows[0] = c->tuned_rows[1] = c->tuned_rows[2] = c->pair_rows = 0;
    if (!c->devices.empty()) multi_plan(c);
    return true;
}

bool same_dims(const Harmonic *h, const Ctx *c)
{
    if ((int)h->n != c->n) return false;
    for (unsigned i = 0; i < h->n; i++)
        if ((int)h->m[i] != c->m[i]) return false;
    return true;
}

Ctx *get_ctx(Harmonic *h, bool create)
{
    std::lock_guard<std::mutex> lk(g_mu);
    auto it = g_ctx.find(h);
    if (it != g_ctx.end()) {
        Ctx *c = it->second;
        if (h->d_m == nullptr && h->d_u == nullptr && h->d_locked == nullptr && h->d_delta == nullptr &&
            (c->buf[0] || c->maskw || c->d_m || c->d_delta || multi_holds_anything(c))) {
            drop_graphs(c);
            if (c->multi()) multi_destroy(c);
            for (float *&b : c->buf) { if (b) (void)hipFree(b); b = nullptr; }
            free_spare(c);
            if (c->maskw) (void)hipFree(c->maskw);
            if (c->d_m) (void)hipFree(c->d_m);
            if (c->d_delta) (void)hipFree(c->d_delta);
            c->maskw = nullptr; c->d_m = nullptr; c->d_delta = nullptr;
            c->pending = 0;
            c->ahead.live = false;
            c->tick_plain = 0;
            c->defer_bypass = false;
            c->cfg = Config::from_env();
            apply_config(c);
            c->tuned_rows[0] = c->tuned_rows[1] = c->tuned_rows[2] = c->pair_rows = 0;
            c->graphs_broken = false;
        }
        return c;
    }
    if (!create) return nullptr;
    Ctx *c = new Ctx();
    if (hipStreamCreateWithFlags(&c->stream, hipStreamNonBlocking) != hipSuccess) {
        (void)hipGetLastError();
        delete c;
        return nullptr;
    }
    if (hipHostMalloc((void **)&c->h_delta, 64, hipHostMallocDefault) != hipSuccess) {
        (void)hipGetLastError();
        (void)hipStreamDestroy(c->stream);
        delete c;
        return nullptr;
    }
    if (hipHostMalloc((void **)&c->h_tile_delta, 2 * kTileDeltaCap * sizeof(float), hipHostMallocDefault) != hipSuccess) {
        (void)hipGetLastError();
        c->h_tile_delta = nullptr;
    }
    c->cfg = Config::from_env();
    apply_config(c);
    g_ctx[h] = c;
    return c;
}

void apply_config(Ctx *c)
{
    const Config &cfg = c->cfg;
    c->rows_per_task = cfg.rows_per_task;
    c->math = cfg.math;
    c->redblack = cfg.redblack;
    c->track_mode = cfg.track_mode;
    c->halo_env = cfg.halo;
    c->devices.clear();
    if (!cfg.devices_text.empty()) {
        int ndev = 0;
        if (hipGetDeviceCount(&ndev) != hipSuccess) { (void)hipGetLastError(); ndev = 0; }
        bool ok = !cfg.devices_malformed && !cfg.devices.empty();
        for (int d : cfg.devices)
            if (d >= ndev) ok = false;
        if (ok) c->devices = cfg.devices;
        else fprintf(stderr, "Warning[epic_hip]: EPIC_HIP_DEVICES=%s ignored (%d device(s) visible)\n", cfg.devices_text.c_str(), ndev);
    }
}

void drop_ctx_if_empty(Harmonic *h)
{
    std::lock_guard<std::mutex> lk(g_mu);
    auto it = g_ctx.find(h);
    if (it == g_ctx.end()) return;
    Ctx *c = it->second;
    if (c->buf[0] || c->maskw || c->d_m || c->d_delta || multi_holds_anything(c)) return;
    drop_graphs(c);
    if (c->multi()) multi_destroy(c);
    c->trk.release();
    c->trk_f.release();
    if (c->stream) { (void)hipStreamSynchronize(c->stream); (void)hipStreamDestroy(c->stream); }
    if (c->h_delta) (void)hipHostFree(c->h_delta);
    if (c->h_tile_delta) (void)hipHostFree(c->h_tile_delta);
    free_spare(c);
    for (hipEvent_t &e : c->ev_blk) { if (e) (void)hipEventDestroy(e); e = nullptr; }
    delete c;
    g_ctx.erase(it);
}

bool ready(const Harmonic *h, const Ctx *c)
{
    if (c && c->multi()) return multi_ready(c) && h->d_u && h->d_locked;
    return c && c->buf[0] && c->buf[1] && c->maskw && h->d_u && h->d_locked;
}

float *current_u(const Ctx *c) { return c->multi() ? c->slabs[0].buf[c->cur] : c->buf[c->cur]; }
bool has_delta(const Ctx *c) { return c->multi() ? c->slabs[0].d_delta != nullptr : c->d_delta != nullptr; }

int upload_u(Harmonic *h, Ctx *c, const char *fn)
{
    if (c->multi()) return multi_upload_u(h, c, fn);
    force_all(c);
    if (c->pitch != c->cols) {
        for (int b = 0; b < 2; b++)
            if (epic_hip::launch_fill(c->buf[b], (size_t)c->rows * c->pitch, -1e6f, c->stream) != hipSuccess) {
                report(fn, "Failed to initialise device-side memory for the potential values.");
                return EPIC_ERROR_KERNEL_EXECUTION;
            }
        if (hipStreamSynchronize(c->stream) != hipSuccess) return EPIC_ERROR_DEVICE_SYNCHRONIZE;
    }
    c->cur = 0;
    if (hipMemcpy2D(c->buf[0], (size_t)c->pitch * sizeof(float), h->u, (size_t)c->cols * sizeof(float),
                    (size_t)c->cols * sizeof(float), (size_t)c->rows, hipMemcpyHostToDevice) != hipSuccess) {
        report(fn, "Failed to copy memory from host to device for the potential values.");
        return EPIC_ERROR_MEMCPY_TO_DEVICE;
    }
    h->d_u = c->buf[0];
    return EPIC_SUCCESS;
}

int upload_locked(Harmonic *h, Ctx *c, const char *fn)
{
    if (c->multi()) return multi_upload_locked(h, c, fn);
    force_all(c);
    if (c->n == 4) return EPIC_SUCCESS;
    const size_t cells = (size_t)c->rows * c->cols;
    uint32_t *tmp = nullptr;
    if (hipMalloc((void **)&tmp, cells * sizeof(uint32_t)) != hipSuccess) {
        (void)hipGetLastError();
        report(fn, "Failed to allocate device-side staging memory for the locked cells.");
        return EPIC_ERROR_DEVICE_MALLOC;
    }
    int rc = EPIC_SUCCESS;
    if (hipMemcpy(tmp, h->locked, cells * sizeof(uint32_t), hipMemcpyHostToDevice) != hipSuccess) {
        report(fn, "Failed to copy memory from host to device for the locked cells.");
        rc = EPIC_ERROR_MEMCPY_TO_DEVICE;
    } else {
        hipError_t e = c->n == 2
                           ? epic_hip::launch_pack_mask_2d(tmp, c->rows, c->cols, c->pitch, 0, 0, c->maskw, c->stream)
                           : epic_hip::launch_pack_mask_3d(tmp, c->m[0], c->m[1], c->m[2], c->pitch, c->maskw, c->stream);
        if (e == hipSuccess && c->n == 2) e = epic_hip::launch_fuse_masks_2d(c->maskw, c->rows, c->pitch, c->maskf(), c->stream);
        if (e != hipSuccess || hipStreamSynchronize(c->stream) != hipSuccess) {
            report(fn, "Failed to execute the 'pack mask' kernel.");
            rc = EPIC_ERROR_KERNEL_EXECUTION;
        }
    }
    (void)hipFree(tmp);
    return rc;
}

}

using namespace epic_drv;

namespace epic {
extern "C" {


int harmonic_initialize_dimension_size_gpu(Harmonic *harmonic)
{
    static const char *fn = "harmonic_initialize_dimension_size_gpu";
    if (harmonic == nullptr || harmonic->n == 0 || harmonic->m == nullptr) {
        report(fn, "Invalid input.");
        return EPIC_ERROR_INVALID_DATA;
    }
    Ctx *c = get_ctx(harmonic, true);
    if (c == nullptr) {
        report(fn, "Failed to allocate device-side memory for the dimension size.");
        return EPIC_ERROR_DEVICE_MALLOC;
    }
    {
        const int frc = flush_pending(harmonic, c, fn);
        if (frc != EPIC_SUCCESS) return frc;
    }
    if (c->d_m) { (void)hipFree(c->d_m); c->d_m = nullptr; }
    if (hipMalloc((void **)&c->d_m, harmonic->n * sizeof(unsigned)) != hipSuccess) {
        (void)hipGetLastError();
        report(fn, "Failed to allocate device-side memory for the dimension size.");
        drop_ctx_if_empty(harmonic);
        return EPIC_ERROR_DEVICE_MALLOC;
    }
    if (hipMemcpy(c->d_m, harmonic->m, harmonic->n * sizeof(unsigned), hipMemcpyHostToDevice) != hipSuccess) {
        report(fn, "Failed to copy memory from host to device for the dimension size.");
        (void)hipFree(c->d_m);
        c->d_m = nullptr;
        harmonic->d_m = nullptr;
        drop_ctx_if_empty(harmonic);
        return EPIC_ERROR_MEMCPY_TO_DEVICE;
    }
    harmonic->d_m = c->d_m;
    return EPIC_SUCCESS;
}

int harmonic_uninitialize_dimension_size_gpu(Harmonic *harmonic)
{
    if (harmonic == nullptr) return EPIC_ERROR_INVALID_DATA;
    Ctx *c = find_ctx(harmonic);
    int rc = flush_pending(harmonic, c, "harmonic_uninitialize_dimension_size_gpu");
    if (c && c->d_m) {
        if (hipFree(c->d_m) != hipSuccess) {
            report("harmonic_uninitialize_dimension_size_gpu", "Failed to free device-side memory for the dimension size.");
            rc = EPIC_ERROR_DEVICE_FREE;
        }
        c->d_m = nullptr;
    }
    harmonic->d_m = nullptr;
    drop_ctx_if_empty(harmonic);
    return rc;
}

int harmonic_initialize_potential_values_gpu(Harmonic *harmonic)
{
    static const char *fn = "harmonic_initialize_potential_values_gpu";
    if (harmonic == nullptr || harmonic->n == 0 || harmonic->m == nullptr || harmonic->u == nullptr) {
        report(fn, "Invalid input.");
        return EPIC_ERROR_INVALID_DATA;
    }
    Ctx probe;
    if (!dims_from(harmonic, &probe)) {
        report(fn, "Invalid input (n = 2 and n = 3 need every m[i] >= 3; n = 4 is held but never swept; other n are not supported).");
        return EPIC_ERROR_INVALID_DATA;
    }
    Ctx *c = get_ctx(harmonic, true);
    if (c == nullptr) {
        report(fn, "Failed to allocate device-side memory for the potential values.");
        return EPIC_ERROR_DEVICE_MALLOC;
    }
    if ((c->maskw || (c->multi() && c->slabs[0].maskw)) && !same_dims(harmonic, c)) {
        report(fn, "Invalid input (dimensions differ from the locked cells already on the device).");
        return EPIC_ERROR_INVALID_DATA;
    }
    c->pending = 0;
    c->ahead.live = false;
    drop_graphs(c);
    for (float *&b : c->buf) { if (b) (void)hipFree(b); b = nullptr; }
    free_spare(c);
    if (c->multi()) { DeviceGuard g; multi_free_u(c); }
    dims_into_ctx(harmonic, c);
    if (c->plan_failed) {
        report(fn, "Failed to create the streams, events and staging buffers of the device slabs.");
        harmonic->d_u = nullptr;
        drop_ctx_if_empty(harmonic);
        return EPIC_ERROR_DEVICE_MALLOC;
    }
    if (c->multi()) {
        DeviceGuard g;
        for (auto &sl : c->slabs)
            for (int b = 0; b < 2; b++)
                if (hipSetDevice(sl.dev) != hipSuccess ||
                    hipMalloc((void **)&sl.buf[b], (size_t)sl.rows * unit_floats(c) * sizeof(float)) != hipSuccess) {
                    (void)hipGetLastError();
                    report(fn, "Failed to allocate device-side memory for the potential values.");
                    multi_free_u(c);
                    harmonic->d_u = nullptr;
                    drop_ctx_if_empty(harmonic);
                    return EPIC_ERROR_DEVICE_MALLOC;
                }
        return upload_u(harmonic, c, fn);
    }
    for (int b = 0; b < 2; b++) {
        if (hipMalloc((void **)&c->buf[b], c->u_bytes()) != hipSuccess) {
            (void)hipGetLastError();
            report(fn, "Failed to allocate device-side memory for the potential values.");
            for (float *&bb : c->buf) { if (bb) (void)hipFree(bb); bb = nullptr; }
            harmonic->d_u = nullptr;
            drop_ctx_if_empty(harmonic);
            return EPIC_ERROR_DEVICE_MALLOC;
        }
    }
    return upload_u(harmonic, c, fn);
}

int harmonic_uninitialize_potential_values_gpu(Harmonic *harmonic)
{
    if (harmonic == nullptr) return EPIC_ERROR_INVALID_DATA;
    int rc = EPIC_SUCCESS;
    Ctx *c = find_ctx(harmonic);
    if (c) {
        c->pending = 0;
        c->ahead.live = false;
        if (c->stream) (void)hipStreamSynchronize(c->stream);
        drop_graphs(c);
        if (c->multi()) { DeviceGuard g; multi_free_u(c); }
        for (float *&b : c->buf) {
            if (b && hipFree(b) != hipSuccess) {
                report("harmonic_uninitialize_potential_values_gpu", "Failed to free device-side memory for the potential values.");
                rc = EPIC_ERROR_DEVICE_FREE;
            }
            b = nullptr;
        }
        free_spare(c);
    }
    harmonic->d_u = nullptr;
    drop_ctx_if_empty(harmonic);
    return rc;
}

int harmonic_initialize_locked_gpu(Harmonic *harmonic)
{
    static const char *fn = "harmonic_initialize_locked_gpu";
    if (harmonic == nullptr || harmonic->n == 0 || harmonic->m == nullptr || harmonic->locked == nullptr) {
        report(fn, "Invalid input.");
        return EPIC_ERROR_INVALID_DATA;
    }
    Ctx probe;
    if (!dims_from(harmonic, &probe)) {
        report(fn, "Invalid input (n = 2 and n = 3 need every m[i] >= 3; n = 4 is held but never swept; other n are not supported).");
        return EPIC_ERROR_INVALID_DATA;
    }
    Ctx *c = get_ctx(harmonic, true);
    if (c == nullptr) {
        report(fn, "Failed to allocate device-side memory for the locked cells.");
        return EPIC_ERROR_DEVICE_MALLOC;
    }
    if ((c->buf[0] || (c->multi() && c->slabs[0].buf[0])) && !same_dims(harmonic, c)) {
        report(fn, "Invalid input (dimensions differ from the potential values already on the device).");
        return EPIC_ERROR_INVALID_DATA;
    }
    {
        const int frc = flush_pending(harmonic, c, fn);
        if (frc != EPIC_SUCCESS) return frc;
    }
    drop_graphs(c);
    if (c->maskw) { (void)hipFree(c->maskw); c->maskw = nullptr; }
    if (c->multi()) { DeviceGuard g; multi_free_mask(c); }
    dims_into_ctx(harmonic, c);
    if (c->plan_failed) {
        report(fn, "Failed to create the streams, events and staging buffers of the device slabs.");
        harmonic->d_locked = nullptr;
        drop_ctx_if_empty(harmonic);
        return EPIC_ERROR_DEVICE_MALLOC;
    }
    if (c->multi()) {
        {
            DeviceGuard g;
            for (auto &sl : c->slabs)
                if (hipSetDevice(sl.dev) != hipSuccess ||
                    hipMalloc((void **)&sl.maskw, sizeof(uint32_t) * slab_mask_words(c, sl)) != hipSuccess) {
                    (void)hipGetLastError();
                    report(fn, "Failed to allocate device-side memory for the locked cells.");
                    multi_free_mask(c);
                    harmonic->d_locked = nullptr;
                    drop_ctx_if_empty(harmonic);
                    return EPIC_ERROR_DEVICE_MALLOC;
                }
        }
        int rc = upload_locked(harmonic, c, fn);
        if (rc == EPIC_SUCCESS) harmonic->d_locked = c->slabs[0].maskw;
        return rc;
    }
    if (hipMalloc((void **)&c->maskw, c->mask_bytes()) != hipSuccess) {
        (void)hipGetLastError();
        report(fn, "Failed to allocate device-side memory for the locked cells.");
        harmonic->d_locked = nullptr;
        drop_ctx_if_empty(harmonic);
        return EPIC_ERROR_DEVICE_MALLOC;
    }
    int rc = upload_locked(harmonic, c, fn);
    if (rc == EPIC_SUCCESS) harmonic->d_locked = c->maskw;
    return rc;
}

int harmonic_uninitialize_locked_gpu(Harmonic *harmonic)
{
    if (harmonic == nullptr) return EPIC_ERROR_INVALID_DATA;
    Ctx *c = find_ctx(harmonic);
    int rc = flush_pending(harmonic, c, "harmonic_uninitialize_locked_gpu");
    if (c && c->multi()) { DeviceGuard g; multi_free_mask(c); }
    if (c && c->maskw) {
        if (c->stream) (void)hipStreamSynchronize(c->stream);
        drop_graphs(c);
        if (hipFree(c->maskw) != hipSuccess) {
            report("harmonic_uninitialize_locked_gpu", "Failed to free device-side memory for the locked cells.");
            rc = EPIC_ERROR_DEVICE_FREE;
        }
        c->maskw = nullptr;
    }
    harmonic->d_locked = nullptr;
    drop_ctx_if_empty(harmonic);
    return rc;
}

int harmonic_update_model_gpu(Harmonic *harmonic)
{
    static const char *fn = "harmonic_update_model_gpu";
    if (harmonic == nullptr || harmonic->n == 0 || harmonic->m == nullptr || harmonic->u == nullptr ||
        harmonic->d_u == nullptr || harmonic->locked == nullptr || harmonic->d_locked == nullptr) {
        report(fn, "Invalid data.");
        return EPIC_ERROR_INVALID_DATA;
    }
    Ctx *c = find_ctx(harmonic);
    if (!ready(harmonic, c) || !same_dims(harmonic, c)) {
        report(fn, "Invalid data.");
        return EPIC_ERROR_INVALID_DATA;
    }
    c->pending = 0;
    c->ahead.live = false;
    if (c->multi()) { DeviceGuard g; multi_sync(c); }
    if (hipStreamSynchronize(c->stream) != hipSuccess) return EPIC_ERROR_DEVICE_SYNCHRONIZE;
    int rc = upload_u(harmonic, c, fn);
    if (rc != EPIC_SUCCESS) return rc;
    return upload_locked(harmonic, c, fn);
}

int harmonic_initialize_gpu(Harmonic *harmonic, unsigned int numThreads)
{
    static const char *fn = "harmonic_initialize_gpu";
    (void)numThreads;
    if (harmonic == nullptr || harmonic->n == 0 || harmonic->m == nullptr || harmonic->d_delta != nullptr) {
        report(fn, "Invalid input.");
        return EPIC_ERROR_INVALID_DATA;
    }
    Ctx *c = get_ctx(harmonic, true);
    if (c == nullptr) {
        report(fn, "Failed to allocate device-side memory for delta.");
        return EPIC_ERROR_DEVICE_MALLOC;
    }
    if (c->d_delta) { (void)hipFree(c->d_delta); c->d_delta = nullptr; }
    if (c->multi()) {
        DeviceGuard g;
        multi_free_delta(c);
        for (auto &sl : c->slabs)
            if (hipSetDevice(sl.dev) != hipSuccess || hipMalloc((void **)&sl.d_delta, 64) != hipSuccess) {
                (void)hipGetLastError();
                report(fn, "Failed to allocate device-side memory for delta.");
                multi_free_delta(c);
                drop_ctx_if_empty(harmonic);
                return EPIC_ERROR_DEVICE_MALLOC;
            }
        harmonic->d_delta = reinterpret_cast<float *>(c->slabs[0].d_delta);
        return EPIC_SUCCESS;
    }
    if (hipMalloc((void **)&c->d_delta, 64) != hipSuccess) {
        (void)hipGetLastError();
        report(fn, "Failed to allocate device-side memory for delta.");
        drop_ctx_if_empty(harmonic);
        return EPIC_ERROR_DEVICE_MALLOC;
    }
    harmonic->d_delta = reinterpret_cast<float *>(c->d_delta);
    return EPIC_SUCCESS;
}

int harmonic_uninitialize_gpu(Harmonic *harmonic)
{
    if (harmonic == nullptr) return EPIC_ERROR_INVALID_DATA;
    Ctx *c = find_ctx(harmonic);
    int rc = flush_pending(harmonic, c, "harmonic_uninitialize_gpu");
    if (c && c->multi()) { DeviceGuard g; multi_free_delta(c); }
    if (c && c->d_delta) {
        if (c->stream) (void)hipStreamSynchronize(c->stream);
        if (hipFree(c->d_delta) != hipSuccess) {
            report("harmonic_uninitialize_gpu", "Failed to free device-side memory for delta.");
            rc = EPIC_ERROR_DEVICE_FREE;
        }
        c->d_delta = nullptr;
    }
    harmonic->d_delta = nullptr;
    drop_ctx_if_empty(harmonic);
    return rc;
}

int harmonic_get_potential_values_gpu(Harmonic *harmonic)
{
    static const char *fn = "harmonic_get_potential_values_gpu";
    Ctx *c = harmonic ? find_ctx(harmonic) : nullptr;
    if (!harmonic || harmonic->u == nullptr || !c || !(c->buf[0] || (c->multi() && c->slabs[0].buf[0])) || harmonic->d_u == nullptr) {
        report(fn, "Invalid data.");
        return EPIC_ERROR_INVALID_DATA;
    }
    {
        const int frc = flush_pending(harmonic, c, fn);
        if (frc != EPIC_SUCCESS) return frc;
    }
    if (c->multi()) return multi_get_values(harmonic, c, fn);
    if (hipStreamSynchronize(c->stream) != hipSuccess) {
        report(fn, "Failed to synchronize the device before reading the potential values.");
        return EPIC_ERROR_DEVICE_SYNCHRONIZE;
    }
    if (hipMemcpy2D(harmonic->u, (size_t)c->cols * sizeof(float), c->buf[c->cur], (size_t)c->pitch * sizeof(float),
                    (size_t)c->cols * sizeof(float), (size_t)c->rows, hipMemcpyDeviceToHost) != hipSuccess) {
        report(fn, "Failed to copy memory from device to host for the potential values.");
        return EPIC_ERROR_MEMCPY_TO_HOST;
    }
    return EPIC_SUCCESS;
}

}
}
```

### epic_amd/csrc/kernels.h

```cpp
#pragma once
#include <hip/hip_runtime.h>
#include <stddef.h>
#include <stdint.h>
#include <stdlib.h>

#include "driver_config.h"

namespace epic_hip {

constexpr int kWakeListCount = 256;
constexpr int kWakeCounterStride = 32;
struct Activity {
    const uint32_t *list_in;
    const uint32_t *count_in;
    uint32_t *list_out;
    uint32_t *count_out;
    uint32_t *count_zero;
    uint32_t *queued_in;
    uint32_t *queued_out;
    unsigned long long *total;
};
inline size_t sweep_2d_tiles(int rows, int pitch, int rows_per_task)
{
    return (size_t)((pitch + 255) / 256) * (size_t)((rows + rows_per_task - 1) / rows_per_task);
}
inline size_t sweep_2d_list_cap(size_t tiles) { return (tiles + kWakeListCount - 1) / kWakeListCount; }
inline int sweep_2d_list_blocks(size_t tiles, int resident_blocks)
{
    const size_t forced = process_launch_knobs().list_waves;
    const size_t waves = forced ? forced : (size_t)(resident_blocks > 0 ? resident_blocks : 2048) * 4;
    return (int)(((tiles < waves ? tiles : waves) + 31) / 32) * 8;
}
int resident_blocks_of(const void *kernel);
hipError_t launch_sweep_2d(const float *in, float *out, const uint32_t *maskw, int rows, int pitch, int row_begin,
                           int row_end, int rows_per_task, int math, int parity, unsigned *delta_bits,
                           hipStream_t stream, const Activity *act = nullptr, int check_begin = -1, int check_end = -1);
hipError_t launch_wake_tile_range(const Activity *next_as_out, size_t tiles, int t_lo, int t_hi, hipStream_t stream);
hipError_t launch_rb_fused_2d(const float *in, float *out, const uint32_t *maskw, int rows, int pitch, int rows_per_task,
                              int math, int parity, hipStream_t stream, const uint32_t *maskf = nullptr, const Activity *act = nullptr,
                              unsigned *delta_bits = nullptr, int check_begin = -1, int check_end = -1);
constexpr int kFusedLaneCols = 4;
constexpr int kFusedStrideQuads = 62;
constexpr int kFusedStride = kFusedStrideQuads * kFusedLaneCols;
__host__ __device__ inline int fused_2d_strips(int pitch)
{
    if (pitch <= 2 * kFusedLaneCols) return 1;
    if ((pitch - 2 * kFusedLaneCols) % kFusedStride == 0) return (pitch - 2 * kFusedLaneCols) / kFusedStride;
    return (pitch - kFusedLaneCols + kFusedStride - 1) / kFusedStride;
}
__host__ __device__ inline int fused_2d_quad0(int strip) { return strip * kFusedStrideQuads; }
__host__ __device__ inline int fused_2d_col(int strip, int lane) { return (fused_2d_quad0(strip) + lane) * kFusedLaneCols; }
__host__ __device__ inline bool fused_2d_owns(int strip, int lane, int col, int pitch)
{
    return col < pitch && (lane >= 1 || strip == 0) && (lane <= kFusedStrideQuads || col + kFusedLaneCols == pitch);
}
inline size_t rb_fused_2d_tiles(int rows, int pitch, int rows_per_task)
{
    return (size_t)fused_2d_strips(pitch) * (size_t)((rows + rows_per_task - 1) / rows_per_task);
}
hipError_t launch_jacobi_fused_2d(const float *in, float *out, const uint32_t *maskw, int rows, int pitch, int rows_per_task,
                                  int math, hipStream_t stream, int parity = -1, const uint32_t *maskf = nullptr,
                                  const Activity *act = nullptr, unsigned *delta_bits = nullptr, int check_begin = -1, int check_end = -1);
inline size_t mask_words_fused_2d(int rows, int pitch) { return (size_t)rows * (size_t)fused_2d_strips(pitch) * 8u; }
hipError_t launch_fuse_masks_2d(const uint32_t *maskw, int rows, int pitch, uint32_t *maskf, hipStream_t stream);
hipError_t launch_eval_math(const float *in, float *out, size_t n, int which, hipStream_t stream);
hipError_t launch_pack_mask_2d(const uint32_t *locked, int rows, int cols, int pitch, int ghost_top,
                               int ghost_bottom, uint32_t *maskw, hipStream_t stream);
hipError_t launch_fill(float *p, size_t n, float v, hipStream_t stream);
hipError_t launch_set_cells_2d(float *u, uint32_t *maskw, int rows, int cols, int pitch, unsigned k,
                               const unsigned *v, const unsigned *types, hipStream_t stream, int row0 = 0, int grid_rows = 0,
                               int pin_top = 0, int pin_bottom = 0);

constexpr int kOccCounters = 256, kOccCounterStride = 16;
constexpr size_t kOccCounterBytes = (size_t)kOccCounters * kOccCounterStride * sizeof(unsigned long long);
hipError_t launch_occupancy_2d(float *u, uint32_t *maskw, const unsigned char *d_occ, size_t occ_pitch, int rows, int cols, int pitch,
                               int obstacle_threshold, int no_change, unsigned flags, unsigned long long *d_changed, hipStream_t stream);
hipError_t launch_reset_free_cells_2d(float *u, const uint32_t *maskw, int rows, int cols, int pitch, hipStream_t stream);

struct TilePlan { int halo, tile_rows, tile_cols, tiles_r, tiles_c; };
constexpr int kTile2dCols = 64, kTile2dMaxRows = 64;
constexpr int kTile2dWideCols = 128;
inline int tile_2d_max_rows(int math, bool redblack, int width)
{
    if (width == kTile2dCols) return kTile2dMaxRows;
    if (width != kTile2dWideCols) return 0;
    if (math == 4) return redblack ? 64 : 0;
    return 128;
}
inline TilePlan tile_2d_plan(int rows, int cols, int halo, int tile_rows = 0, int width = kTile2dCols, int max_rows = kTile2dMaxRows)
{
    TilePlan p = {0, 0, 0, 0, 0};
    if (halo < 1 || 2 * halo >= width - 8 || 2 * halo >= max_rows - 1 || rows < 3 || cols < 3) return p;
    const int tc = width - 2 * halo;
    const int tiles_c = (cols + tc - 1) / tc;
    const int max_tr = max_rows - 2 * halo;
    int tr = tile_rows;
    if (tr <= 0) {
        static const int cus = [] {
            int n = 256, dev = 0;
            if (hipGetDevice(&dev) != hipSuccess || hipDeviceGetAttribute(&n, hipDeviceAttributeMultiprocessorCount, dev) != hipSuccess || n < 1) {
                (void)hipGetLastError();
                n = 256;
            }
            return n;
        }();
        const int tiles_r_max = cus / tiles_c > 1 ? cus / tiles_c : 1;
        tr = (rows + tiles_r_max - 1) / tiles_r_max;
        tr = (tr + 1) / 2 * 2;
        if (tr < 8) tr = 8;
    }
    tr = (tr < max_tr ? tr : max_tr) / 2 * 2;
    if (tr < 2) return p;
    p.halo = halo;
    p.tile_rows = tr;
    p.tile_cols = tc;
    p.tiles_r = (rows + tr - 1) / tr;
    p.tiles_c = tiles_c;
    return p;
}
hipError_t launch_tile_2d(const float *in, float *out, const uint32_t *maskw, int rows, int pitch, const TilePlan &plan, int steps,
                          int math, int parity, unsigned *delta_bits, hipStream_t stream, float *tile_delta = nullptr);

hipError_t launch_follow_paths_2d(const float *u, const uint32_t *maskw, int rows, int cols, int pitch, unsigned n_paths,
                                  const float *d_starts, float step, float cd, unsigned max_points, float *d_pts,
                                  unsigned *d_k, int *d_rc, hipStream_t stream);

#ifndef EPIC_TOL_AHEAD
#define EPIC_TOL_AHEAD 2
#endif
constexpr int kTolRowsAhead = EPIC_TOL_AHEAD;
constexpr int kTolTripRows = (kTolRowsAhead + 3) % 2 == 0 ? kTolRowsAhead + 3 : 2 * (kTolRowsAhead + 3);
inline int jacobi_fused_auto_rows(int rows, int pitch)
{
    const long long nstrips = fused_2d_strips(pitch), slots = 4096;
    const long long r = (long long)rows * nstrips / slots;
    return (int)(r < 12 ? 12 : r > 40 ? 40 : r);
}
inline int pitch_for_cols(int cols) { return (cols + 255) / 256 * 256; }
inline size_t mask_words_2d(int rows, int pitch) { return (size_t)rows * (size_t)(pitch / 256) * 8u; }
__host__ __device__ inline size_t mask_word_2d(unsigned r, unsigned c, unsigned pitch)
{
    return (((size_t)r * (pitch >> 8) + (c >> 8)) * 4u + (c & 3u)) * 2u + ((c >> 7) & 1u);
}
__host__ __device__ inline unsigned mask_bit_2d(unsigned c) { return (c >> 2) & 31u; }

hipError_t launch_sweep_3d(const float *in, float *out, const uint32_t *maskw, int m0, int m1, int pitch,
                           int plane_begin, int plane_end, int math, int parity, unsigned *delta_bits,
                           hipStream_t stream, const Activity *act = nullptr, int check_begin = -1, int check_end = -1,
                           const LaunchKnobs *knobs = nullptr);
inline size_t sweep_3d_tiles(int m0, int m1, int pitch)
{
    return (size_t)m0 * (size_t)((m1 + 31) / 32) * (size_t)((pitch + 255) / 256);
}
hipError_t launch_pack_mask_3d(const uint32_t *locked, int m0, int m1, int m2, int pitch, uint32_t *maskw,
                               hipStream_t stream);
inline size_t mask_words_3d(int m0, int m1, int pitch) { return (size_t)m0 * (size_t)m1 * (size_t)(pitch / 32); }

hipError_t launch_follow_paths_3d(const float *u, const uint32_t *maskw, int m0, int m1, int m2, int pitch, unsigned n_paths,
                                  const float *d_starts, float step, float cd, unsigned max_points, float *d_pts, unsigned *d_k,
                                  int *d_rc, hipStream_t stream);
hipError_t launch_pack_paths_3d(const float *d_pts, size_t row, unsigned n_paths, const unsigned *d_k, const unsigned long long *d_offset,
                                float *d_packed, hipStream_t stream);
hipError_t launch_set_cells_3d(float *u, uint32_t *maskw, int m0, int m1, int m2, int pitch, unsigned k, const unsigned *v,
                               const unsigned *types, hipStream_t stream);

struct OccRegion {
    int m0, m1, cols;
    int origin[3], extent[3];
    bool faces0;
};
hipError_t launch_occupancy_region(float *u, uint32_t *maskw, const unsigned char *d_occ, const OccRegion &region, int pitch,
                                   int obstacle_threshold, int no_change, unsigned flags, unsigned long long *d_changed, hipStream_t stream);

struct QueryField {
    const float *u;
    const uint32_t *maskw;
    int n;
    int m0, m1, m2, pitch;
};
hipError_t launch_sample_points(const QueryField &field, unsigned n_points, const float *d_points, bool gradient, float cd, float *d_out,
                                unsigned char *d_status, hipStream_t stream);
hipError_t launch_flow_field(const QueryField &field, const unsigned origin[3], const unsigned extent[3], float cd, float *d_gradient,
                             unsigned char *d_status, hipStream_t stream);
hipError_t launch_gather_region(const QueryField &field, const unsigned origin[3], const unsigned extent[3], float *d_u, unsigned *d_locked,
                                hipStream_t stream);
hipError_t launch_gather_cells(const QueryField &field, unsigned k, const unsigned *d_v, float *d_u, unsigned *d_locked, hipStream_t stream);

}
```

### epic_amd/csrc/kernels_2d.hip

```cpp
#include <type_traits>
#include <hip/hip_runtime.h>
#include <stdint.h>
#include <stdlib.h>

#include <algorithm>
#include <map>
#include <mutex>

#include "cell_update.h"
#include "kernels.h"
#include "wake.h"

#ifndef EPIC_CONSTS_SWEEP2D
#define EPIC_CONSTS_SWEEP2D(RB, TRACK) ((RB) && !(TRACK) ? kConstsKeep : kConstsPlain)
#endif
#ifndef EPIC_CONSTS_RBPAIR
#define EPIC_CONSTS_RBPAIR(TRACK, CHECK) kConstsKeep
#endif
namespace epic_hip {

namespace {

constexpr int kWave = 64;
constexpr int kColsPerLane = 4;
constexpr int kStripCols = kWave * kColsPerLane;
constexpr int kWavesPerBlock = 4;
constexpr int kNumXcd = 8;
static_assert(kWakeLists == kWave * kWavesPerBlock, "one thread per work list resets the counters");

struct Sweep2dArgs {
    const float *in;
    float *out;
    const uint32_t *maskw;
    const uint32_t *maskf;
    unsigned *delta_bits;
    int rows;
    int pitch;
    int row_begin, row_end;
    int rows_per_task;
    int chunk_rem;
    int nstrips;
    int ntasks;
    int parity;
    int flags;
    WakeArgs wake;
    int nchunks;
    int nblocks;
    int check_lo, check_hi;
};

__device__ __forceinline__ int xcd_contiguous_block(int b, int nblk)
{
    int x = b % kNumXcd, i = b / kNumXcd;
    int q = nblk / kNumXcd, rem = nblk % kNumXcd;
    return x * q + (x < rem ? x : rem) + i;
}

#ifdef EPIC_SWEEP_WAVES
#define EPIC_SWEEP_OCC __attribute__((amdgpu_waves_per_eu(EPIC_SWEEP_WAVES, EPIC_SWEEP_WAVES)))
#else
#define EPIC_SWEEP_OCC
#endif
template <bool CHECK, int MATH, bool RB, bool TRACK> struct SweepOcc {
    static constexpr int kMinWaves = (MATH == kMathTol && !TRACK && !(RB && CHECK)) ? (CHECK ? 5 : 6) : 1;
};
template <bool CHECK, int MATH, bool RB, bool TRACK>
__global__ __launch_bounds__(kWave * kWavesPerBlock, (SweepOcc<CHECK, MATH, RB, TRACK>::kMinWaves)) EPIC_SWEEP_OCC void sweep2d_kernel(Sweep2dArgs a)
{
    constexpr bool TOL = MATH == kMathTol;
    __shared__ __attribute__((aligned(16))) char math_lds_bytes[TOL ? TolLn<4>::kLdsBytes : kMathLdsDoubles * (int)sizeof(double)];
    double *const math_lds = reinterpret_cast<double *>(math_lds_bytes);
    const TolLnEntry *const tl = reinterpret_cast<const TolLnEntry *>(math_lds_bytes);
    if (TOL) TolLn<4>::stage(reinterpret_cast<TolLnEntry *>(math_lds_bytes));
    const MathTab lds = math_tables_at(math_lds, EPIC_CONSTS_SWEEP2D(RB, TRACK));
    MathTabRegs tab_regs = {};
    if (MATH == kMathPrecise) tab_regs = math_tables_fetch();
    bool tables_pending = MATH == kMathPrecise;
    const int lane = threadIdx.x & (kWave - 1);
    const int wave = __builtin_amdgcn_readfirstlane(threadIdx.x >> 6);
    if (TRACK) wake_reset_next(a.wake);
    const bool listed = TRACK && a.wake.list_in != nullptr;
    WakeCursor cursor = {};
    if (listed && !wake_begin(a.wake, lane, wave, kWavesPerBlock, cursor)) return;
    float dmax = 0.0f;
    const int rlast = a.rows - 1;
    const size_t pitch = (size_t)a.pitch;

    int vb = blockIdx.x;
    for (;;) {
    int task;
    if (listed) task = wake_tile(a.wake, cursor);
    else task = xcd_contiguous_block(vb, a.nblocks) * kWavesPerBlock + wave;
    if (task >= a.ntasks) {
        if (listed) break;
        vb += gridDim.x;
        if (vb >= a.nblocks) break;
        continue;
    }
    if (TRACK && lane == 0) a.wake.queued_in[task] = 0;
    const int strip = task % a.nstrips;
    const int chunk = task / a.nstrips;
    const int r0 = a.row_begin + chunk * a.rows_per_task;
    const int r1 = min(r0 + a.rows_per_task, a.row_end);

    const int col0 = strip * kStripCols;

    const int rlo = max(r0 - 8, 0);
    const __amdgpu_buffer_rsrc_t rin = raw_buffer(a.in + (size_t)rlo * pitch), rout = raw_buffer(a.out + (size_t)rlo * pitch);
    const unsigned lane16 = (unsigned)lane * 16u;
    typedef unsigned vu4 __attribute__((ext_vector_type(4)));
    auto row_off = [&](int r) -> unsigned { return (unsigned)((r - rlo) * a.pitch + col0) * 4u; };

    auto ld = [&](int r) -> float4 {
        r = min(max(r, 0), rlast);
        const vu4 q = __builtin_amdgcn_raw_buffer_load_b128(rin, lane16, row_off(r), 0);
        return make_float4(u2f(q.x), u2f(q.y), u2f(q.z), u2f(q.w));
    };
    typedef const __attribute__((address_space(4))) float cfloat;
    typedef const __attribute__((address_space(4))) uint64_t cu64;
    const int hcol_l = max(col0 - 1, 0), hcol_r = min(col0 + kStripCols, a.pitch - 1);
    struct RowSide { float l, r; lmask m0, m1, m2, m3; };
    auto side = [&](int r) -> RowSide {
        r = min(max(r, 0), rlast);
        cfloat *row = (cfloat *)(a.in + (size_t)r * pitch);
        cu64 *mk = (cu64 *)a.maskw + ((size_t)r * a.nstrips + strip) * 4;
        return RowSide{row[hcol_l], row[hcol_r], mk[0], mk[1], mk[2], mk[3]};
    };
    struct EdgeSplit { float ql, qr, zl, zr; };
    auto edge_split = [&](const RowSide &h) -> EdgeSplit {
        const Split2 hs = tol_split2(v2f{h.l, h.r});
        return EdgeSplit{hs.q.x, hs.q.y, hs.zm.x, hs.zm.y};
    };
    auto masks = [&](int r) -> RowSide {
        r = min(max(r, 0), rlast);
        cu64 *mk = (cu64 *)a.maskw + ((size_t)r * a.nstrips + strip) * 4;
        return RowSide{0.0f, 0.0f, mk[0], mk[1], mk[2], mk[3]};
    };

    const int dir = ((a.flags & 1) && (chunk & 1)) ? -1 : 1;
    const int rfirst = dir > 0 ? r0 : r1 - 1;
    const int nrows = r1 - r0;

    lmask chg_any = 0, chg_x = 0, chg_w = 0, chg_top = 0, chg_bot = 0;
    auto row_step = [&](int r, const float4 &up, const float4 &c, const float4 &dn, const RowSide &h, const Split4 &su,
                        const Split4 &sc, const Split4 &sd, const EdgeSplit &he) {
        const float lf = wave_from_left(c.w, h.l);
        const float rt = wave_from_right(c.x, h.r);
        float4 o;
        if (TOL) {
            const float ql = wave_from_left(sc.qw, he.ql), qr = wave_from_right(sc.qx, he.qr);
            const uint32_t nl = f2u(wave_from_left(u2f(sc.nw), he.zl)), nr = f2u(wave_from_right(u2f(sc.nx), he.zr));
            o = c;
            const bool odd_cols = !RB || ((r + a.parity) & 1) == 0, even_cols = !RB || !odd_cols;
            auto pre_xz = [&] {
                return tol_pre2_2d(up.x, dn.x, lf, c.y, su.qx, su.nx, sd.qx, sd.nx, ql, nl, sc.qy, sc.ny,
                                   up.z, dn.z, c.y, c.w, su.qz, su.nz, sd.qz, sd.nz, sc.qy, sc.ny, sc.qw, sc.nw);
            };
            auto pre_yw = [&] {
                return tol_pre2_2d(up.y, dn.y, c.x, c.z, su.qy, su.ny, sd.qy, sd.ny, sc.qx, sc.nx, sc.qz, sc.nz,
                                   up.w, dn.w, c.z, rt, su.qw, su.nw, sd.qw, sd.nw, sc.qz, sc.nz, qr, nr);
            };
            float nx, ny, nz, nw;
            TolLnRaw ea, eb;
            if (!RB) {
                const TolPre2 pxz = pre_xz();
                TolLnPair f0 = tol_ln_issue<4>(pxz, tl);
                const TolPre2 pyw = pre_yw();
                TolLnPair f1 = tol_ln_issue<4>(pyw, tl);
                tol_ln_wait<2>(f0, ea, eb);
                tol_post2(pxz, ea, eb, kLn4, nx, nz);
                o.x = sel(h.m0, c.x, nx);
                o.z = sel(h.m2, c.z, nz);
                tol_ln_wait<0>(f1, ea, eb);
                tol_post2(pyw, ea, eb, kLn4, ny, nw);
                o.y = sel(h.m1, c.y, ny);
                o.w = sel(h.m3, c.w, nw);
            } else if (even_cols) {
                const TolPre2 pxz = pre_xz();
                TolLnPair f0 = tol_ln_issue<4>(pxz, tl);
                tol_ln_wait<0>(f0, ea, eb);
                tol_post2(pxz, ea, eb, kLn4, nx, nz);
                o.x = sel(h.m0, c.x, nx);
                o.z = sel(h.m2, c.z, nz);
            } else {
                const TolPre2 pyw = pre_yw();
                TolLnPair f1 = tol_ln_issue<4>(pyw, tl);
                tol_ln_wait<0>(f1, ea, eb);
                tol_post2(pyw, ea, eb, kLn4, ny, nw);
                o.y = sel(h.m1, c.y, ny);
                o.w = sel(h.m3, c.w, nw);
            }
        } else if (RB) {
            o = c;
            if (((r + a.parity) & 1) == 0) {
                const float ny = cell_update_2d<MATH>(up.y, dn.y, c.x, c.z, lds);
                const float nw = cell_update_2d<MATH>(up.w, dn.w, c.z, rt, lds);
                o.y = sel(h.m1, c.y, ny);
                o.w = sel(h.m3, c.w, nw);
            } else {
                const float nx = cell_update_2d<MATH>(up.x, dn.x, lf, c.y, lds);
                const float nz = cell_update_2d<MATH>(up.z, dn.z, c.y, c.w, lds);
                o.x = sel(h.m0, c.x, nx);
                o.z = sel(h.m2, c.z, nz);
            }
        } else {
            o.x = cell_update_2d<MATH>(up.x, dn.x, lf, c.y, lds);
            o.y = cell_update_2d<MATH>(up.y, dn.y, c.x, c.z, lds);
            o.z = cell_update_2d<MATH>(up.z, dn.z, c.y, c.w, lds);
            o.w = cell_update_2d<MATH>(up.w, dn.w, c.z, rt, lds);
        }
        if (!RB && !TOL) {
            o.x = sel(h.m0, c.x, o.x);
            o.y = sel(h.m1, c.y, o.y);
            o.z = sel(h.m2, c.z, o.z);
            o.w = sel(h.m3, c.w, o.w);
        }
        if (CHECK && r >= a.check_lo && r < a.check_hi) {
            dmax = max2(dmax, fabsf(c.x - o.x));
            dmax = max2(dmax, fabsf(c.y - o.y));
            dmax = max2(dmax, fabsf(c.z - o.z));
            dmax = max2(dmax, fabsf(c.w - o.w));
        }
        if (TRACK) {
            const lmask cx = lanes_ne(o.x, c.x), cw = lanes_ne(o.w, c.w);
            const lmask rc = cx | cw | lanes_ne(o.y, c.y) | lanes_ne(o.z, c.z);
            chg_any |= rc;
            chg_x |= cx;
            chg_w |= cw;
            if (r == r0) chg_top = rc;
            if (r == r1 - 1) chg_bot = rc;
        }
        store_row(rout, o.x, o.y, o.z, o.w, lane16, row_off(r));
    };

    auto row_at = [&](int i) { return rfirst + dir * i; };
    auto split = [&](const float4 &q) { return TOL ? tol_split4(q) : Split4{}; };
    constexpr bool DEEP = TOL || MATH == kMathTraffic;
    if constexpr (DEEP) {
        constexpr int kAhead = kTolRowsAhead, kRing = kAhead + 3, kTrip = kTolTripRows;
        static_assert(kTrip % kRing == 0 && kTrip % 2 == 0, "the rings close after a trip");
        float4 q[kRing];
        Split4 s[kRing];
        RowSide h[2];
#pragma unroll
        for (int k = 0; k < kAhead + 2; ++k) q[k] = ld(row_at(k - 1));
        h[0] = TOL ? masks(row_at(0)) : side(row_at(0));
        if (tables_pending) {
            math_tables_commit(tab_regs, math_lds);
            tables_pending = false;
        }
        const int ntrip = nrows / kTrip * kTrip;
        if (ntrip > 0) {
            const int hk = min(lane & 31, kTrip - 1);
            const int hcol = lane < 32 ? hcol_l : hcol_r;
            auto edge_ld = [&](int i0) -> float {
                const int r = rfirst + dir * (i0 + hk);
                return u2f(__builtin_amdgcn_raw_buffer_load_b32(rin, (unsigned)((r - rlo) * a.pitch + hcol) * 4u, 0, 0));
            };
            int lane_zero;
            asm("v_mov_b32 %0, 0" : "=v"(lane_zero));
            float ev_next = edge_ld(0);
            s[0] = split(q[0]); s[1] = split(q[1]);
            for (int i = 0; i < ntrip; i += kTrip) {
                const float ev = ev_next;
                const Split1 es = tol_split1(ev);
                if (i + kTrip < ntrip) ev_next = edge_ld(i + kTrip);
                auto trip_row = [&](auto jc) {
                    constexpr int j = decltype(jc)::value;
                    q[(j + 2 + kAhead) % kRing] = ld(row_at(i + j + 1 + kAhead));
                    h[(j + 1) & 1] = TOL ? masks(row_at(i + j + 1)) : side(row_at(i + j + 1));
                    s[(j + 2) % kRing] = split(q[(j + 2) % kRing]);
                    RowSide hj = h[j & 1];
                    EdgeSplit he = {};
                    if constexpr (TOL) edge_from_lanes<j>(lane_zero, ev, es.q, es.zm, hj.l, hj.r, he.ql, he.qr, he.zl, he.zr);
                    row_step(row_at(i + j), q[j % kRing], q[(j + 1) % kRing], q[(j + 2) % kRing], hj, s[j % kRing],
                             s[(j + 1) % kRing], s[(j + 2) % kRing], he);
                };
                unrolled<kTrip>(trip_row);
            }
        }
        for (int i = ntrip; i < nrows; ++i) {
            const int r = row_at(i);
            const float4 ru = ld(r - dir), rc = ld(r), rd = ld(r + dir);
            const RowSide hr = side(r);
            row_step(r, ru, rc, rd, hr, split(ru), split(rc), split(rd), TOL ? edge_split(hr) : EdgeSplit{});
        }
    } else {
    const int nfull = nrows & ~3;
    float4 q0 = ld(row_at(-1)), q1 = ld(row_at(0)), q2 = ld(row_at(1)), q3;
    RowSide sa = side(row_at(0)), sb;
    if (tables_pending) {
        math_tables_commit(tab_regs, math_lds);
        tables_pending = false;
    }
    const Split4 none = {};
    const EdgeSplit no_edge = {};
    if (nfull > 0) {
        for (int i = 0; i < nfull; i += 4) {
            q3 = ld(row_at(i + 2)); sb = side(row_at(i + 1));
            row_step(row_at(i), q0, q1, q2, sa, none, none, none, no_edge);
            q0 = ld(row_at(i + 3)); sa = side(row_at(i + 2));
            row_step(row_at(i + 1), q1, q2, q3, sb, none, none, none, no_edge);
            q1 = ld(row_at(i + 4)); sb = side(row_at(i + 3));
            row_step(row_at(i + 2), q2, q3, q0, sa, none, none, none, no_edge);
            q2 = ld(row_at(i + 5)); sa = side(row_at(i + 4));
            row_step(row_at(i + 3), q3, q0, q1, sb, none, none, none, no_edge);
        }
    }
    if (nfull == 0 && nrows > 0) row_step(row_at(0), q0, q1, q2, sa, none, none, none, no_edge);
    for (int i = nfull == 0 ? 1 : nfull; i < nrows; ++i) {
        const int r = row_at(i);
        row_step(r, ld(r - dir), ld(r), ld(r + dir), side(r), none, none, none, no_edge);
    }
    }

    if (TRACK) {
        const bool any = chg_any != 0;
        const bool first_col = (chg_x & 1ull) != 0;
        const bool last_col = (chg_w >> 63) != 0;
        const bool first_row = chg_top != 0, last_row = chg_bot != 0;
        int t = task;
        bool want = any;
        if (lane == 1) { t = task - 1; want = strip > 0 && first_col; }
        if (lane == 2) { t = task + 1; want = strip + 1 < a.nstrips && last_col; }
        if (lane == 3) { t = task - a.nstrips; want = chunk > 0 && first_row; }
        if (lane == 4) { t = task + a.nstrips; want = chunk + 1 < a.nchunks && last_row; }
        wake_push(a.wake, t, want && lane < 5);
    }
    if (listed) { if (!wake_next(cursor)) break; }
    else { vb += gridDim.x; if (vb >= a.nblocks) break; }
    }

    if (CHECK) {
        dmax = wave_max(dmax);
        if (lane == 0 && dmax > 0.0f &&
            __float_as_uint(dmax) > __hip_atomic_load(a.delta_bits, __ATOMIC_RELAXED, __HIP_MEMORY_SCOPE_AGENT))
            atomicMax(a.delta_bits, __float_as_uint(dmax));
    }
}

static_assert(kFusedLaneCols == kColsPerLane && kFusedStrideQuads == kWave - 2, "kernels.h states the strip geometry for this wave");

template <int MATH, bool FMASK, bool TRACK, bool CHECK>
__global__ __launch_bounds__(kWave * kWavesPerBlock) void rb_fused2d_kernel(Sweep2dArgs a)
{
    __shared__ __attribute__((aligned(16))) double math_lds[kMathLdsDoubles];
    MathTab lds = {};
    if (MATH == kMathPrecise) lds = math_tables_load(math_lds, EPIC_CONSTS_RBPAIR(TRACK, CHECK));
    const int lane = threadIdx.x & (kWave - 1);
    const int wave = __builtin_amdgcn_readfirstlane(threadIdx.x >> 6);
    if (TRACK) wake_reset_next(a.wake);
    const bool listed = TRACK && a.wake.list_in != nullptr;
    WakeCursor cursor = {};
    if (listed && !wake_begin(a.wake, lane, wave, kWavesPerBlock, cursor)) return;
    float dmax = 0.0f;
    const int rlast = a.rows - 1;
    const size_t pitch = (size_t)a.pitch;
    const int it = a.parity;
    typedef unsigned vu4 __attribute__((ext_vector_type(4)));
    typedef const __attribute__((address_space(4))) uint64_t cu64;
    const int nstd = a.pitch >> 8;

    int vb = blockIdx.x;
    for (;;) {
    int task;
    if (listed) task = wake_tile(a.wake, cursor);
    else task = xcd_contiguous_block(vb, a.nblocks) * kWavesPerBlock + wave;
    if (task >= a.ntasks) {
        if (listed) break;
        vb += gridDim.x;
        if (vb >= a.nblocks) break;
        continue;
    }
    if (TRACK && lane == 0) a.wake.queued_in[task] = 0;
    const int strip = task % a.nstrips;
    const int chunk = task / a.nstrips;
    const int r0 = a.row_begin + chunk * a.rows_per_task + min(chunk, a.chunk_rem);
    const int r1 = min(r0 + a.rows_per_task + (chunk < a.chunk_rem ? 1 : 0), a.row_end);
    const int col = fused_2d_col(strip, lane);
    const int lcol = min(col, a.pitch - kColsPerLane);
    const bool owner = fused_2d_owns(strip, lane, col, a.pitch);
    const lmask owners = (TRACK || CHECK) ? __builtin_amdgcn_ballot_w64(owner) : 0;

    const int rlo = max(r0 - 2, 0);
    const __amdgpu_buffer_rsrc_t rin = raw_buffer(a.in + (size_t)rlo * pitch), rout = raw_buffer(a.out + (size_t)rlo * pitch);
    const unsigned lane_off = (unsigned)lcol * 4u;
    const unsigned store_off = owner ? lane_off : 0x80000000u;
    auto row_off = [&](int r) -> unsigned { return (unsigned)((r - rlo) * a.pitch) * 4u; };
    auto ld = [&](int r) -> float4 {
        r = min(max(r, 0), rlast);
        const vu4 q = __builtin_amdgcn_raw_buffer_load_b128(rin, lane_off, row_off(r), 0);
        return make_float4(u2f(q.x), u2f(q.y), u2f(q.z), u2f(q.w));
    };
    struct RowMask { lmask m0, m1, m2, m3; };
    struct RowMaskRaw { lmask lo0, lo1, lo2, lo3, hi0, hi1, hi2, hi3; };
    const int g0 = fused_2d_quad0(strip);
    const int sw = g0 >> 6, sh = g0 & 63, sw1 = min(sw + 1, nstd - 1);
    auto mask_fetch = [&](int r) -> RowMaskRaw {
        r = min(max(r, 0), rlast);
        if (FMASK) {
            cu64 *mk = (cu64 *)a.maskf + ((size_t)r * a.nstrips + strip) * 4;
            return RowMaskRaw{mk[0], mk[1], mk[2], mk[3], 0, 0, 0, 0};
        }
        cu64 *lo = (cu64 *)a.maskw + ((size_t)r * nstd + sw) * 4, *hi = (cu64 *)a.maskw + ((size_t)r * nstd + sw1) * 4;
        return RowMaskRaw{lo[0], lo[1], lo[2], lo[3], hi[0], hi[1], hi[2], hi[3]};
    };
    auto mask_cut = [&](const RowMaskRaw &w) -> RowMask {
        if (FMASK) return RowMask{w.lo0, w.lo1, w.lo2, w.lo3};
        auto cut = [&](lmask lo, lmask hi) -> lmask {
            return (lo >> sh) | ((hi << 1) << (63 - sh));
        };
        return RowMask{cut(w.lo0, w.hi0), cut(w.lo1, w.hi1), cut(w.lo2, w.hi2), cut(w.lo3, w.hi3)};
    };
    auto row_mask = [&](int r) -> RowMask { return mask_cut(mask_fetch(r)); };
    lmask chg_any = 0, chg_top = 0, chg_bot = 0;
    bool chg_left = false, chg_right = false, c_tl = false, c_tr = false, c_bl = false, c_br = false;
    constexpr lmask kFirstOwned = 2ull, kLastOwned = 1ull << (kWave - 2);
    auto stage = [&](int r, bool second, bool owned, const float4 &up, const float4 &c, const float4 &dn, const RowMask &k) -> float4 {
        float4 o = c;
        const bool odd_cols = ((((r + it) & 1) == 0) != second);
        const bool counts = CHECK && r >= a.check_lo && r < a.check_hi;
        lmask e0 = 0, e1 = 0;
        if (odd_cols) {
            const float rt = wave_from_right(c.x, 0.0f);
            const float ny = cell_update_2d<MATH>(up.y, dn.y, c.x, c.z, lds);
            const float nw = cell_update_2d<MATH>(up.w, dn.w, c.z, rt, lds);
            o.y = sel(k.m1, c.y, ny);
            o.w = sel(k.m3, c.w, nw);
            if (TRACK) { e0 = lanes_ne(o.y, c.y); e1 = lanes_ne(o.w, c.w); }
            if (CHECK && second && counts) dmax = max2(dmax, sel(owners, max2(fabsf(c.y - o.y), fabsf(c.w - o.w)), 0.0f));
        } else {
            const float lf = wave_from_left(c.w, 0.0f);
            const float nx = cell_update_2d<MATH>(up.x, dn.x, lf, c.y, lds);
            const float nz = cell_update_2d<MATH>(up.z, dn.z, c.y, c.w, lds);
            o.x = sel(k.m0, c.x, nx);
            o.z = sel(k.m2, c.z, nz);
            if (TRACK) { e0 = lanes_ne(o.x, c.x); e1 = lanes_ne(o.z, c.z); }
            if (CHECK && second && counts) dmax = max2(dmax, sel(owners, max2(fabsf(c.x - o.x), fabsf(c.z - o.z)), 0.0f));
        }
        if (TRACK && owned) {
            const lmask rc = (e0 | e1) & owners;
            chg_any |= rc;
            if (r < r0 + 2) chg_top |= rc;
            if (r >= r1 - 2) chg_bot |= rc;
            const bool l = (e0 & kFirstOwned) != 0, rr = (e1 & kLastOwned & owners) != 0;
            chg_left |= l;
            chg_right |= rr;
            if (r == r0) { c_tl |= l && !odd_cols; c_tr |= rr && odd_cols; }
            if (r == r1 - 1) { c_bl |= l && !odd_cols; c_br |= rr && odd_cols; }
        }
        return o;
    };

    const float4 om2 = ld(r0 - 2), om1 = ld(r0 - 1), o0 = ld(r0);
    float4 oa = ld(r0 + 1), ob = ld(r0 + 2), oc;
    RowMask kcur = row_mask(r0), knext = row_mask(r0 + 1);
    float4 ma = stage(r0 - 1, false, false, om2, om1, o0, row_mask(r0 - 1)), mb = stage(r0, false, true, om1, o0, oa, kcur), mc;
    auto step = [&](int r, const float4 &mp, const float4 &mq, float4 &mr, const float4 &o1, const float4 &o2, float4 &o3) {
        o3 = ld(r + 3);
        const RowMaskRaw kraw = mask_fetch(r + 2);
        mr = stage(r + 1, false, r + 1 < r1, mq, o1, o2, knext);
        const float4 x = stage(r, true, true, mp, mq, mr, kcur);
        kcur = knext;
        knext = mask_cut(kraw);
        store_row(rout, x.x, x.y, x.z, x.w, store_off, row_off(r));
    };
    int r = r0;
    for (; r + 3 <= r1; r += 3) {
        step(r, ma, mb, mc, oa, ob, oc);
        step(r + 1, mb, mc, ma, ob, oc, oa);
        step(r + 2, mc, ma, mb, oc, oa, ob);
    }
    for (; r < r1; ++r) {
        step(r, ma, mb, mc, oa, ob, oc);
        ma = mb; mb = mc; oa = ob; ob = oc;
    }

    if (TRACK) {
        const bool up_ok = chunk > 0, dn_ok = chunk + 1 < a.nchunks, lf_ok = strip > 0, rt_ok = strip + 1 < a.nstrips;
        int t = task;
        bool want = chg_any != 0;
        if (lane == 1) { t = task - 1; want = lf_ok && chg_left; }
        if (lane == 2) { t = task + 1; want = rt_ok && chg_right; }
        if (lane == 3) { t = task - a.nstrips; want = up_ok && chg_top != 0; }
        if (lane == 4) { t = task + a.nstrips; want = dn_ok && chg_bot != 0; }
        if (lane == 5) { t = task - a.nstrips - 1; want = up_ok && lf_ok && c_tl; }
        if (lane == 6) { t = task - a.nstrips + 1; want = up_ok && rt_ok && c_tr; }
        if (lane == 7) { t = task + a.nstrips - 1; want = dn_ok && lf_ok && c_bl; }
        if (lane == 8) { t = task + a.nstrips + 1; want = dn_ok && rt_ok && c_br; }
        wake_push(a.wake, t, want && lane < 9);
    }
    if (listed) { if (!wake_next(cursor)) break; }
    else { vb += gridDim.x; if (vb >= a.nblocks) break; }
    }

    if (CHECK) {
        dmax = wave_max(dmax);
        if (lane == 0 && dmax > 0.0f &&
            __float_as_uint(dmax) > __hip_atomic_load(a.delta_bits, __ATOMIC_RELAXED, __HIP_MEMORY_SCOPE_AGENT))
            atomicMax(a.delta_bits, __float_as_uint(dmax));
    }
}

#ifndef EPIC_FUSED_MIN_WAVES
#define EPIC_FUSED_MIN_WAVES 4
#endif
template <bool RB, bool FMASK, bool TRACK = false, bool CHECK = false>
__device__ __forceinline__ void tol_fused_pass(const Sweep2dArgs &a, TolLnEntry *math_lds)
{
    TolLn<4>::stage(math_lds);
    const TolLnEntry *const tl = math_lds;
    const int lane = threadIdx.x & (kWave - 1);
    const int wave = __builtin_amdgcn_readfirstlane(threadIdx.x >> 6);
    if (TRACK) wake_reset_next(a.wake);
    const bool listed = TRACK && a.wake.list_in != nullptr;
    WakeCursor cursor = {};
    float dmax = 0.0f;
    const bool have_work = !listed || wake_begin(a.wake, lane, wave, kWavesPerBlock, cursor);
    if (have_work)
    for (int vb = blockIdx.x;;) {
    int task;
    if (listed) task = wake_tile(a.wake, cursor);
    else task = xcd_contiguous_block(vb, a.nblocks) * kWavesPerBlock + wave;
    if (task >= a.ntasks) {
        if (listed) break;
        vb += gridDim.x;
        if (vb >= a.nblocks) break;
        continue;
    }
    if (TRACK && lane == 0) a.wake.queued_in[task] = 0;
    const int strip = task % a.nstrips;
    const int chunk = task / a.nstrips;
    const int r0 = a.row_begin + chunk * a.rows_per_task + min(chunk, a.chunk_rem);
    const int r1 = min(r0 + a.rows_per_task + (chunk < a.chunk_rem ? 1 : 0), a.row_end);
    const int col = fused_2d_col(strip, lane);
    const int lcol = min(col, a.pitch - kColsPerLane);
    const bool owner = fused_2d_owns(strip, lane, col, a.pitch);
    const lmask owners = (TRACK || CHECK) ? __builtin_amdgcn_ballot_w64(owner) : 0;
    lmask chg_any = 0, chg_top = 0, chg_bot = 0;
    bool chg_left = false, chg_right = false, c_tl = false, c_tr = false, c_bl = false, c_br = false;
    constexpr lmask kFirstOwned = 2ull, kLastOwned = 1ull << (kWave - 2);
    const int rlast = a.rows - 1;
    const size_t pitch = (size_t)a.pitch;
    typedef unsigned vu4 __attribute__((ext_vector_type(4)));

    const int rlo = max(r0 - 2, 0);
    const __amdgpu_buffer_rsrc_t rin = raw_buffer(a.in + (size_t)rlo * pitch), rout = raw_buffer(a.out + (size_t)rlo * pitch);
    const unsigned lane_off = (unsigned)lcol * 4u;
    const unsigned store_off = owner ? lane_off : 0x80000000u;
    auto row_off = [&](int r) -> unsigned { return (unsigned)((r - rlo) * a.pitch) * 4u; };
    auto ld = [&](int r) -> float4 {
        r = min(max(r, 0), rlast);
        const vu4 q = __builtin_amdgcn_raw_buffer_load_b128(rin, lane_off, row_off(r), 0);
        return make_float4(u2f(q.x), u2f(q.y), u2f(q.z), u2f(q.w));
    };
    typedef const __attribute__((address_space(4))) uint64_t cu64;
    struct RowMask { lmask m0, m1, m2, m3; };
    struct RowMaskRaw { lmask lo0, lo1, lo2, lo3, hi0, hi1, hi2, hi3; };
    const int nstd = a.pitch >> 8;
    const int g0 = fused_2d_quad0(strip);
    const int sw = g0 >> 6, sh = g0 & 63, sw1 = min(sw + 1, nstd - 1);
    auto mask_fetch = [&](int r) -> RowMaskRaw {
        r = min(max(r, 0), rlast);
        if (FMASK) {
            cu64 *mk = (cu64 *)a.maskf + ((size_t)r * a.nstrips + strip) * 4;
            return RowMaskRaw{mk[0], mk[1], mk[2], mk[3], 0, 0, 0, 0};
        }
        cu64 *lo = (cu64 *)a.maskw + ((size_t)r * nstd + sw) * 4, *hi = (cu64 *)a.maskw + ((size_t)r * nstd + sw1) * 4;
        return RowMaskRaw{lo[0], lo[1], lo[2], lo[3], hi[0], hi[1], hi[2], hi[3]};
    };
    auto mask_cut = [&](const RowMaskRaw &w) -> RowMask {
        if (FMASK) return RowMask{w.lo0, w.lo1, w.lo2, w.lo3};
        auto cut = [&](lmask lo, lmask hi) -> lmask { return (lo >> sh) | ((hi << 1) << (63 - sh)); };
        return RowMask{cut(w.lo0, w.hi0), cut(w.lo1, w.hi1), cut(w.lo2, w.hi2), cut(w.lo3, w.hi3)};
    };
    auto row_mask = [&](int r) -> RowMask { return mask_cut(mask_fetch(r)); };
    auto shl = [](float v) { return u2f(__builtin_amdgcn_mov_dpp(f2u(v), 0x138 , 0xf, 0xf, true)); };
    auto shr = [](float v) { return u2f(__builtin_amdgcn_mov_dpp(f2u(v), 0x130 , 0xf, 0xf, true)); };
    auto level = [&](const float4 &up, const float4 &c, const float4 &dn, const Split4 &su, const Split4 &sc, const Split4 &sd,
                     const RowMask &k, bool odd_cols, int row, bool second, bool owned) -> float4 {
        float4 o = c;
        const bool even = !RB || !odd_cols;
        auto pre_xz = [&] {
            return tol_pre2_2d_left(up.x, dn.x, c.w, c.y, su.qx, su.nx, sd.qx, sd.nx, shl(sc.qw), sc.nw, sc.qy, sc.ny,
                                    up.z, dn.z, c.y, c.w, su.qz, su.nz, sd.qz, sd.nz, sc.qy, sc.ny, sc.qw, sc.nw);
        };
        auto pre_yw = [&] {
            return tol_pre2_2d_right(up.y, dn.y, c.x, c.z, su.qy, su.ny, sd.qy, sd.ny, sc.qx, sc.nx, sc.qz, sc.nz,
                                     up.w, dn.w, c.z, c.x, su.qw, su.nw, sd.qw, sd.nw, sc.qz, sc.nz, shr(sc.qx), sc.nx);
        };
        float nx, ny, nz, nw;
        TolLnRaw ea, eb;
        if (!RB) {
            const TolPre2 pxz = pre_xz();
            TolLnPair f0 = tol_ln_issue<4>(pxz, tl);
            const TolPre2 pyw = pre_yw();
            TolLnPair f1 = tol_ln_issue<4>(pyw, tl);
            tol_ln_wait<2>(f0, ea, eb);
            tol_post2(pxz, ea, eb, kLn4, nx, nz);
            o.x = sel(k.m0, c.x, nx);
            o.z = sel(k.m2, c.z, nz);
            tol_ln_wait<0>(f1, ea, eb);
            tol_post2(pyw, ea, eb, kLn4, ny, nw);
            o.y = sel(k.m1, c.y, ny);
            o.w = sel(k.m3, c.w, nw);
        } else if (even) {
            const TolPre2 pxz = pre_xz();
            TolLnPair f0 = tol_ln_issue<4>(pxz, tl);
            tol_ln_wait<0>(f0, ea, eb);
            tol_post2(pxz, ea, eb, kLn4, nx, nz);
            o.x = sel(k.m0, c.x, nx);
            o.z = sel(k.m2, c.z, nz);
        } else {
            const TolPre2 pyw = pre_yw();
            TolLnPair f1 = tol_ln_issue<4>(pyw, tl);
            tol_ln_wait<0>(f1, ea, eb);
            tol_post2(pyw, ea, eb, kLn4, ny, nw);
            o.y = sel(k.m1, c.y, ny);
            o.w = sel(k.m3, c.w, nw);
        }
        if (CHECK && second && row >= a.check_lo && row < a.check_hi) {
            const float d = max2(max2(fabsf(c.x - o.x), fabsf(c.y - o.y)), max2(fabsf(c.z - o.z), fabsf(c.w - o.w)));
            dmax = max2(dmax, sel(owners, d, 0.0f));
        }
        if (TRACK && owned) {
            const lmask e0 = lanes_ne(o.x, c.x) | lanes_ne(o.y, c.y), e1 = lanes_ne(o.z, c.z) | lanes_ne(o.w, c.w);
            const lmask rc = (e0 | e1) & owners;
            chg_any |= rc;
            if (row < r0 + 2) chg_top |= rc;
            if (row >= r1 - 2) chg_bot |= rc;
            chg_left |= (e0 & kFirstOwned) != 0;
            chg_right |= (e1 & kLastOwned & owners) != 0;
            if (row == r0 || row == r1 - 1) {
                const bool cl = (lanes_ne(o.x, c.x) & kFirstOwned) != 0, cr = (lanes_ne(o.w, c.w) & kLastOwned & owners) != 0;
                if (row == r0) { c_tl |= cl; c_tr |= cr; }
                if (row == r1 - 1) { c_bl |= cl; c_br |= cr; }
            }
        }
        return o;
    };
    auto odd_cols_of = [&](int row, int level_index) { return ((row + a.parity + level_index) & 1) == 0; };

    constexpr int kTrip = 6;
    float4 u[6], m[3];
    Split4 su[3], sm[3];
    RowMask k[3];
#pragma unroll
    for (int x = 0; x < 6; ++x) u[x] = ld(min(r0 - 2 + x, r1 + 1));
    k[0] = row_mask(r0 - 1); k[1] = row_mask(r0); k[2] = row_mask(r0 + 1);
    su[0] = tol_split4(u[0]); su[1] = tol_split4(u[1]); su[2] = tol_split4(u[2]);
    m[0] = level(u[0], u[1], u[2], su[0], su[1], su[2], k[0], odd_cols_of(r0 - 1, 0), r0 - 1, false, false);
    sm[0] = tol_split4(m[0]);
    su[0] = tol_split4(u[3]);
    m[1] = level(u[1], u[2], u[3], su[1], su[2], su[0], k[1], odd_cols_of(r0, 0), r0, false, true);
    sm[1] = tol_split4(m[1]);
    const int nrows = r1 - r0;
    for (int i = 0; i < nrows; i += kTrip) {
        auto step = [&](auto jc) {
            constexpr int j = decltype(jc)::value;
            if (i + j < nrows) {
                const int r = r0 + i + j;
                u[j % 6] = ld(min(r + 4, r1 + 1));
                const RowMaskRaw kraw = mask_fetch(r + 2);
                su[(j + 1) % 3] = tol_split4(u[(j + 4) % 6]);
                m[(j + 2) % 3] = level(u[(j + 2) % 6], u[(j + 3) % 6], u[(j + 4) % 6], su[(j + 2) % 3], su[j % 3],
                                       su[(j + 1) % 3], k[(j + 2) % 3], odd_cols_of(r + 1, 0), r + 1, false, r + 1 < r1);
                sm[(j + 2) % 3] = tol_split4(m[(j + 2) % 3]);
                const float4 x = level(m[j % 3], m[(j + 1) % 3], m[(j + 2) % 3], sm[j % 3], sm[(j + 1) % 3], sm[(j + 2) % 3],
                                       k[(j + 1) % 3], odd_cols_of(r, 1), r, true, true);
                k[j % 3] = mask_cut(kraw);
                store_row(rout, x.x, x.y, x.z, x.w, store_off, row_off(r));
            }
        };
        unrolled<kTrip>(step);
    }
    if (TRACK) {
        const int nchunks = a.nchunks;
        const bool up_ok = chunk > 0, dn_ok = chunk + 1 < nchunks, lf_ok = strip > 0, rt_ok = strip + 1 < a.nstrips;
        int t = task;
        bool want = chg_any != 0;
        if (lane == 1) { t = task - 1; want = lf_ok && chg_left; }
        if (lane == 2) { t = task + 1; want = rt_ok && chg_right; }
        if (lane == 3) { t = task - a.nstrips; want = up_ok && chg_top != 0; }
        if (lane == 4) { t = task + a.nstrips; want = dn_ok && chg_bot != 0; }
        if (lane == 5) { t = task - a.nstrips - 1; want = up_ok && lf_ok && c_tl; }
        if (lane == 6) { t = task - a.nstrips + 1; want = up_ok && rt_ok && c_tr; }
        if (lane == 7) { t = task + a.nstrips - 1; want = dn_ok && lf_ok && c_bl; }
        if (lane == 8) { t = task + a.nstrips + 1; want = dn_ok && rt_ok && c_br; }
        wake_push(a.wake, t, want && lane < 9);
    }
    if (listed) { if (!wake_next(cursor)) break; }
    else { vb += gridDim.x; if (vb >= a.nblocks) break; }
    }
    if (CHECK) {
        dmax = wave_max(dmax);
        if (lane == 0 && dmax > 0.0f &&
            __float_as_uint(dmax) > __hip_atomic_load(a.delta_bits, __ATOMIC_RELAXED, __HIP_MEMORY_SCOPE_AGENT))
            atomicMax(a.delta_bits, __float_as_uint(dmax));
    }
}

template <int MATH, bool FMASK>
__global__ __launch_bounds__(kWave * kWavesPerBlock, EPIC_FUSED_MIN_WAVES) void jacobi_fused2d_kernel(Sweep2dArgs a)
{
    static_assert(MATH == kMathTol, "the fused Jacobi pass exists for the tol math");
    __shared__ TolLnEntry math_lds[TolLn<4>::kEntries];
    tol_fused_pass<false, FMASK>(a, math_lds);
}

template <bool FMASK>
__global__ __launch_bounds__(kWave * kWavesPerBlock, EPIC_FUSED_MIN_WAVES) void rb_tol_fused2d_kernel(Sweep2dArgs a)
{
    __shared__ TolLnEntry math_lds[TolLn<4>::kEntries];
    tol_fused_pass<true, FMASK>(a, math_lds);
}

template <bool RB, bool TRACK, bool CHECK>
__global__ __launch_bounds__(kWave * kWavesPerBlock, 3) void tol_fused2d_tracked_kernel(Sweep2dArgs a)
{
    __shared__ TolLnEntry math_lds[TolLn<4>::kEntries];
    tol_fused_pass<RB, true, TRACK, CHECK>(a, math_lds);
}

__global__ void fuse_masks_2d_kernel(const uint32_t *maskw, int rows, int pitch, uint32_t *maskf)
{
    const int nstd = pitch >> 8, nfused = fused_2d_strips(pitch);
    const size_t n = (size_t)rows * nfused * 4, i = (size_t)blockIdx.x * blockDim.x + threadIdx.x;
    if (i >= n) return;
    const int j = (int)(i & 3), strip = (int)((i >> 2) % nfused);
    const size_t r = (i >> 2) / nfused;
    const int g0 = fused_2d_quad0(strip);
    const int sw = g0 >> 6, sh = g0 & 63, sw1 = min(sw + 1, nstd - 1);
    const unsigned long long *std64 = reinterpret_cast<const unsigned long long *>(maskw);
    const unsigned long long lo = std64[(r * nstd + sw) * 4 + j], hi = std64[(r * nstd + sw1) * 4 + j];
    reinterpret_cast<unsigned long long *>(maskf)[i] = (lo >> sh) | ((hi << 1) << (63 - sh));
}

__global__ __launch_bounds__(kWave * kWavesPerBlock) void pack_mask_2d_kernel(const uint32_t *locked, int rows, int cols,
                                                                              int pitch, int ghost_top, int ghost_bottom,
                                                                              uint32_t *maskw)
{
    const int lane = threadIdx.x & (kWave - 1);
    const int nstrips = pitch >> 8;
    const int strip = blockIdx.y * kWavesPerBlock + (threadIdx.x >> 6);
    const int r = blockIdx.x;
    if (strip >= nstrips || r >= rows) return;
    const bool ghost = (ghost_top && r == 0) || (ghost_bottom && r == rows - 1);
    const bool border_row = (!ghost_top && r == 0) || (!ghost_bottom && r == rows - 1);
    unsigned long long *out = reinterpret_cast<unsigned long long *>(maskw) + ((size_t)r * nstrips + strip) * 4;
#pragma unroll
    for (int j = 0; j < kColsPerLane; ++j) {
        const int c = strip * kStripCols + lane * kColsPerLane + j;
        bool lk = true;
        if (c < cols && !border_row && !ghost && c != 0 && c != cols - 1) lk = locked[(size_t)r * cols + c] != 0;
        const unsigned long long m = __ballot(lk);
        if (lane == j) out[j] = m;
    }
}

__global__ void fill_kernel(float *p, size_t n, float v)
{
    size_t i = (size_t)blockIdx.x * blockDim.x + threadIdx.x;
    const size_t stride = (size_t)gridDim.x * blockDim.x;
    for (; i < n; i += stride) p[i] = v;
}

__global__ void set_cells_2d_kernel(float *u, uint32_t *maskw, int rows, int cols, int pitch, unsigned k,
                                    const unsigned *v, const unsigned *types, int row0, int grid_rows, int pin_top,
                                    int pin_bottom)
{
    const unsigned i = blockIdx.x * blockDim.x + threadIdx.x;
    if (i >= k) return;
    const unsigned x = v[2 * i], gy = v[2 * i + 1];
    if (gy >= (unsigned)grid_rows || x >= (unsigned)cols) return;
    const int y = (int)gy - row0;
    if (y < 0 || y >= rows) return;
    const unsigned t = types[i];
    if (t > 2u) return;
    const float val = (t == 0u) ? 0.0f : -1e6f;
    const bool lock = (t != 2u) || x == 0 || gy == 0 || x == (unsigned)cols - 1 || gy == (unsigned)grid_rows - 1 ||
                      (pin_top && y == 0) || (pin_bottom && y == rows - 1);
    u[(size_t)y * pitch + x] = val;
    uint32_t *w = maskw + mask_word_2d((unsigned)y, x, (unsigned)pitch);
    const uint32_t bit = 1u << mask_bit_2d(x);
    if (lock) atomicOr(w, bit);
    else atomicAnd(w, ~bit);
}

__global__ void eval_math_kernel(const float *in, float *out, size_t n, int which)
{
    __shared__ __attribute__((aligned(16))) double math_lds[kMathLdsDoubles];
    const MathTab plain = math_tables_load(math_lds), keep = math_tables_at(math_lds, kConstsKeep);
    const size_t stride = (size_t)gridDim.x * blockDim.x;
    const size_t first = (size_t)blockIdx.x * blockDim.x + threadIdx.x;
    const size_t trips = (n + stride - 1) / stride;
    for (size_t t = 0; t < trips; t++) {
        const size_t i = first + t * stride;
        const float x = in[i < n ? i : n - 1];
        float r;
        if (which & 2) r = (which & 1) == 0 ? precise_exp(x, keep) : precise_ln(x, keep);
        else r = (which & 1) == 0 ? precise_exp(x, plain) : precise_ln(x, plain);
        if (i < n) out[i] = r;
    }
}

}

static int current_device_cus(int *dev_out = nullptr)
{
    static std::mutex mu;
    static std::map<int, int> cache;
    int dev = 0;
    if (hipGetDevice(&dev) != hipSuccess) {
        (void)hipGetLastError();
        return 0;
    }
    if (dev_out) *dev_out = dev;
    std::lock_guard<std::mutex> lk(mu);
    auto it = cache.find(dev);
    if (it != cache.end()) return it->second;
    int n = 0;
    if (hipDeviceGetAttribute(&n, hipDeviceAttributeMultiprocessorCount, dev) != hipSuccess || n < 1) {
        (void)hipGetLastError();
        n = 0;
    }
    return cache[dev] = n;
}

int resident_blocks_of(const void *kernel)
{
    static std::mutex mu;
    static std::map<std::pair<int, const void *>, int> cache;
    int dev = 0;
    const int cus = current_device_cus(&dev);
    std::lock_guard<std::mutex> lk(mu);
    const auto key = std::make_pair(dev, kernel);
    auto it = cache.find(key);
    if (it != cache.end()) return it->second;
    int blocks = 0;
    if (cus < 1 || hipOccupancyMaxActiveBlocksPerMultiprocessor(&blocks, kernel, kWave * kWavesPerBlock, 0) != hipSuccess || blocks < 1) {
        (void)hipGetLastError();
        return cache[key] = 0;
    }
    return cache[key] = blocks * cus;
}

void tighten_chunks(Sweep2dArgs &a, int rows)
{
    a.chunk_rem = 0;
    if (!(a.flags & 4)) return;
    const int cus = current_device_cus();
    if (cus <= 0 || a.nstrips <= 0) return;
    const long long blocks = ((long long)a.nchunks * a.nstrips + kWavesPerBlock - 1) / kWavesPerBlock;
    const long long per_cu = (blocks + cus - 1) / cus;
    long long n = per_cu * cus * kWavesPerBlock / a.nstrips;
    n = std::min<long long>(n, rows / std::max(8, a.rows_per_task / 2));
    if (n <= a.nchunks) return;
    a.nchunks = (int)n;
    a.rows_per_task = rows / (int)n;
    a.chunk_rem = rows % (int)n;
}

hipError_t launch_eval_math(const float *in, float *out, size_t n, int which, hipStream_t stream)
{
    if (n == 0) return hipSuccess;
    hipLaunchKernelGGL(eval_math_kernel, dim3(4096), dim3(256), 0, stream, in, out, n, which);
    return hipGetLastError();
}

namespace {
int sweep_flags() { return process_launch_knobs().flags; }

int resident_grid(int nblocks, const void *kernel)
{
    const int res = resident_blocks_of(kernel) / kNumXcd * kNumXcd;
    return (res >= kNumXcd && nblocks > res) ? res : nblocks;
}

template <bool CHECK, bool RB, bool TRACK>
void launch_sweep_2d_math(int math, int nblocks, hipStream_t stream, const Sweep2dArgs &a)
{
    void (*kernel)(Sweep2dArgs) = math == kMathFast      ? sweep2d_kernel<CHECK, kMathFast, RB, TRACK>
                                  : math == kMathTraffic ? sweep2d_kernel<CHECK, kMathTraffic, RB, TRACK>
                                  : math == kMathTol     ? sweep2d_kernel<CHECK, kMathTol, RB, TRACK>
                                                         : sweep2d_kernel<CHECK, kMathPrecise, RB, TRACK>;
    if (TRACK && a.wake.list_in) nblocks = sweep_2d_list_blocks((size_t)a.ntasks, resident_blocks_of((const void *)kernel));
    else if (math == kMathTol) nblocks = resident_grid(nblocks, (const void *)kernel);
    const dim3 grid(nblocks), block(kWave * kWavesPerBlock);
    hipLaunchKernelGGL(kernel, grid, block, 0, stream, a);
}
template <bool CHECK, bool RB>
void launch_sweep_2d_track(int math, int nblocks, hipStream_t stream, const Sweep2dArgs &a)
{
    if (a.wake.list_out) launch_sweep_2d_math<CHECK, RB, true>(math, nblocks, stream, a);
    else launch_sweep_2d_math<CHECK, RB, false>(math, nblocks, stream, a);
}
}

hipError_t launch_sweep_2d(const float *in, float *out, const uint32_t *maskw, int rows, int pitch, int row_begin,
                           int row_end, int rows_per_task, int math, int parity, unsigned *delta_bits,
                           hipStream_t stream, const Activity *act, int check_begin, int check_end)
{
    if (row_end <= row_begin) return hipSuccess;
    if (pitch <= 0 || (pitch % 256) != 0 || rows <= 0 || row_begin < 0 || row_end > rows || rows_per_task <= 0)
        return hipErrorInvalidValue;
    if ((parity >= 0) != (in == out)) return hipErrorInvalidValue;
    if (math != kMathPrecise && math != kMathFast && math != kMathTraffic && math != kMathTol) return hipErrorInvalidValue;
    const long long max_rows = 0x7fffffffLL / ((long long)pitch * 4) - 16;
    if (max_rows < 1) return hipErrorInvalidValue;
    rows_per_task = (int)std::min<long long>(rows_per_task, max_rows);
    Sweep2dArgs a;
    a.in = in;
    a.out = out;
    a.maskw = maskw;
    a.maskf = nullptr;
    a.delta_bits = delta_bits;
    a.rows = rows;
    a.pitch = pitch;
    a.row_begin = row_begin;
    a.row_end = row_end;
    a.rows_per_task = rows_per_task;
    a.chunk_rem = 0;
    a.nstrips = (pitch + kStripCols - 1) / kStripCols;
    const int nchunks = (row_end - row_begin + rows_per_task - 1) / rows_per_task;
    a.ntasks = a.nstrips * nchunks;
    a.parity = parity < 0 ? 0 : (parity & 1);
    a.flags = sweep_flags();
    a.nchunks = nchunks;
    const bool whole = row_begin == 0 && row_end == rows;
    a.wake = wake_args(whole ? act : nullptr, (size_t)a.ntasks);
    int nblocks = (a.ntasks + kWavesPerBlock - 1) / kWavesPerBlock;
    a.nblocks = nblocks;
    a.check_lo = check_begin < 0 ? row_begin : check_begin;
    a.check_hi = check_begin < 0 ? row_end : check_end;
    if (parity < 0) {
        if (delta_bits) launch_sweep_2d_track<true, false>(math, nblocks, stream, a);
        else launch_sweep_2d_track<false, false>(math, nblocks, stream, a);
    } else {
        if (delta_bits) launch_sweep_2d_track<true, true>(math, nblocks, stream, a);
        else launch_sweep_2d_track<false, true>(math, nblocks, stream, a);
    }
    return hipGetLastError();
}

namespace {
template <int MATH>
void launch_rb_fused_2d_math(const Sweep2dArgs &a, bool fmask, hipStream_t stream)
{
    const bool track = a.wake.list_out != nullptr, check = a.delta_bits != nullptr;
    void (*kernel)(Sweep2dArgs);
    if (track) kernel = check ? (fmask ? rb_fused2d_kernel<MATH, true, true, true> : rb_fused2d_kernel<MATH, false, true, true>)
                              : (fmask ? rb_fused2d_kernel<MATH, true, true, false> : rb_fused2d_kernel<MATH, false, true, false>);
    else kernel = check ? (fmask ? rb_fused2d_kernel<MATH, true, false, true> : rb_fused2d_kernel<MATH, false, false, true>)
                        : (fmask ? rb_fused2d_kernel<MATH, true, false, false> : rb_fused2d_kernel<MATH, false, false, false>);
    int nblocks = a.nblocks;
    if (track && a.wake.list_in) nblocks = sweep_2d_list_blocks((size_t)a.ntasks, resident_blocks_of((const void *)kernel));
    hipLaunchKernelGGL(kernel, dim3(nblocks), dim3(kWave * kWavesPerBlock), 0, stream, a);
}
}

hipError_t launch_rb_fused_2d(const float *in, float *out, const uint32_t *maskw, int rows, int pitch, int rows_per_task,
                              int math, int parity, hipStream_t stream, const uint32_t *maskf, const Activity *act, unsigned *delta_bits,
                              int check_begin, int check_end)
{
    if (pitch <= 0 || (pitch % 256) != 0 || rows <= 0 || rows_per_task <= 0 || in == out) return hipErrorInvalidValue;
    if (math != kMathPrecise && math != kMathFast && math != kMathTraffic) return hipErrorInvalidValue;
    if (math == kMathTraffic && (act || delta_bits)) return hipErrorInvalidValue;
    const long long max_rows = 0x7fffffffLL / ((long long)pitch * 4) - 8;
    if (max_rows < 1) return hipErrorInvalidValue;
    rows_per_task = (int)std::min<long long>(rows_per_task, max_rows);
    Sweep2dArgs a;
    a.in = in;
    a.out = out;
    a.maskw = maskw;
    a.maskf = maskf;
    a.check_lo = check_begin < 0 ? 0 : check_begin;
    a.check_hi = check_begin < 0 ? rows : check_end;
    a.delta_bits = delta_bits;
    a.rows = rows;
    a.pitch = pitch;
    a.row_begin = 0;
    a.row_end = rows;
    a.rows_per_task = rows_per_task;
    a.chunk_rem = 0;
    a.nstrips = fused_2d_strips(pitch);
    a.nchunks = (rows + rows_per_task - 1) / rows_per_task;
    a.flags = sweep_flags();
    a.ntasks = a.nstrips * a.nchunks;
    a.parity = parity & 1;
    a.wake = wake_args(act, (size_t)a.ntasks);
    a.nblocks = (a.ntasks + kWavesPerBlock - 1) / kWavesPerBlock;
    if (math == kMathFast) launch_rb_fused_2d_math<kMathFast>(a, maskf != nullptr, stream);
    else if (math == kMathTraffic) {
        void (*kernel)(Sweep2dArgs) = maskf ? rb_fused2d_kernel<kMathTraffic, true, false, false> : rb_fused2d_kernel<kMathTraffic, false, false, false>;
        hipLaunchKernelGGL(kernel, dim3(a.nblocks), dim3(kWave * kWavesPerBlock), 0, stream, a);
    } else launch_rb_fused_2d_math<kMathPrecise>(a, maskf != nullptr, stream);
    return hipGetLastError();
}

__global__ void wake_tile_range_kernel(WakeArgs w, int t_lo, int t_hi)
{
    const int t = t_lo + (int)(blockIdx.x * blockDim.x + threadIdx.x);
    wake_push(w, t, t < t_hi);
}

hipError_t launch_wake_tile_range(const Activity *next_as_out, size_t tiles, int t_lo, int t_hi, hipStream_t stream)
{
    if (!next_as_out || !next_as_out->list_out || t_hi <= t_lo) return hipSuccess;
    WakeArgs w = wake_args(next_as_out, tiles);
    w.list_in = nullptr;
    hipLaunchKernelGGL(wake_tile_range_kernel, dim3((unsigned)((t_hi - t_lo + 255) / 256)), dim3(256), 0, stream, w, t_lo, t_hi);
    return hipGetLastError();
}

hipError_t launch_fuse_masks_2d(const uint32_t *maskw, int rows, int pitch, uint32_t *maskf, hipStream_t stream)
{
    if (!maskw || !maskf || rows <= 0 || pitch <= 0 || (pitch % 256) != 0) return hipErrorInvalidValue;
    const size_t n = mask_words_fused_2d(rows, pitch) / 2;
    hipLaunchKernelGGL(fuse_masks_2d_kernel, dim3((unsigned)((n + 255) / 256)), dim3(256), 0, stream, maskw, rows, pitch, maskf);
    return hipGetLastError();
}

hipError_t launch_jacobi_fused_2d(const float *in, float *out, const uint32_t *maskw, int rows, int pitch, int rows_per_task,
                                  int math, hipStream_t stream, int parity, const uint32_t *maskf, const Activity *act, unsigned *delta_bits,
                                  int check_begin, int check_end)
{
    if (pitch <= 0 || (pitch % 256) != 0 || rows <= 0 || rows_per_task <= 0 || in == out) return hipErrorInvalidValue;
    if (math != kMathTol) return hipErrorInvalidValue;
    if ((act || delta_bits) && !maskf) return hipErrorInvalidValue;
    const long long max_rows = 0x7fffffffLL / ((long long)pitch * 4) - 8;
    if (max_rows < 1) return hipErrorInvalidValue;
    rows_per_task = (int)std::min<long long>(rows_per_task, max_rows);
    Sweep2dArgs a;
    a.in = in;
    a.out = out;
    a.maskw = maskw;
    a.maskf = nullptr;
    a.check_lo = check_begin < 0 ? 0 : check_begin;
    a.check_hi = check_begin < 0 ? rows : check_end;
    a.delta_bits = delta_bits;
    a.rows = rows;
    a.pitch = pitch;
    a.row_begin = 0;
    a.row_end = rows;
    a.rows_per_task = rows_per_task;
    a.chunk_rem = 0;
    a.nstrips = fused_2d_strips(pitch);
    a.nchunks = (rows + rows_per_task - 1) / rows_per_task;
    a.flags = sweep_flags();
    if (!act) tighten_chunks(a, rows);
    a.ntasks = a.nstrips * a.nchunks;
    a.parity = parity < 0 ? 0 : parity & 1;
    a.wake = wake_args(act, (size_t)a.ntasks);
    a.nblocks = (a.ntasks + kWavesPerBlock - 1) / kWavesPerBlock;
    a.maskf = maskf;
    const bool track = a.wake.list_out != nullptr, check = delta_bits != nullptr, rb = parity >= 0;
    void (*kernel)(Sweep2dArgs);
    if (!track && !check)
        kernel = !rb ? (maskf ? jacobi_fused2d_kernel<kMathTol, true> : jacobi_fused2d_kernel<kMathTol, false>)
                     : (maskf ? rb_tol_fused2d_kernel<true> : rb_tol_fused2d_kernel<false>);
    else if (rb)
        kernel = track ? (check ? tol_fused2d_tracked_kernel<true, true, true> : tol_fused2d_tracked_kernel<true, true, false>)
                       : tol_fused2d_tracked_kernel<true, false, true>;
    else
        kernel = track ? (check ? tol_fused2d_tracked_kernel<false, true, true> : tol_fused2d_tracked_kernel<false, true, false>)
                       : tol_fused2d_tracked_kernel<false, false, true>;
    const int nblocks = track && a.wake.list_in ? sweep_2d_list_blocks((size_t)a.ntasks, resident_blocks_of((const void *)kernel))
                                                : resident_grid(a.nblocks, (const void *)kernel);
    hipLaunchKernelGGL(kernel, dim3(nblocks), dim3(kWave * kWavesPerBlock), 0, stream, a);
    return hipGetLastError();
}

hipError_t launch_pack_mask_2d(const uint32_t *locked, int rows, int cols, int pitch, int ghost_top,
                               int ghost_bottom, uint32_t *maskw, hipStream_t stream)
{
    const int nstrips = pitch / kStripCols;
    dim3 grid(rows, (nstrips + kWavesPerBlock - 1) / kWavesPerBlock);
    hipLaunchKernelGGL(pack_mask_2d_kernel, grid, dim3(kWave * kWavesPerBlock), 0, stream, locked, rows, cols, pitch,
                       ghost_top, ghost_bottom, maskw);
    return hipGetLastError();
}

hipError_t launch_fill(float *p, size_t n, float v, hipStream_t stream)
{
    if (n == 0) return hipSuccess;
    const int blocks = (int)((n + 255) / 256 < 4096 ? (n + 255) / 256 : 4096);
    hipLaunchKernelGGL(fill_kernel, dim3(blocks), dim3(256), 0, stream, p, n, v);
    return hipGetLastError();
}

hipError_t launch_set_cells_2d(float *u, uint32_t *maskw, int rows, int cols, int pitch, unsigned k,
                               const unsigned *v, const unsigned *types, hipStream_t stream, int row0, int grid_rows,
                               int pin_top, int pin_bottom)
{
    if (k == 0) return hipSuccess;
    if (grid_rows <= 0) grid_rows = rows;
    hipLaunchKernelGGL(set_cells_2d_kernel, dim3((k + 255) / 256), dim3(256), 0, stream, u, maskw, rows, cols, pitch, k,
                       v, types, row0, grid_rows, pin_top, pin_bottom);
    return hipGetLastError();
}

}
```

Before: 770,900.

## Add per-XCD atomic work queue with tall/tail row chunks for fused sweeps

Introduces a FusedQueue schedule for the fused Jacobi/red-black tol kernels: rows are split into tall chunks plus shorter tail chunks, grouped into eight bands (one per XCD), and waves pull tasks through per-band atomic ticket counters, stealing from other bands when their own runs dry. The aim is to cut load imbalance and the tail of idle CUs that a static block-to-task mapping leaves. The auto-tuner now times both static and queue schedules and keeps the queue only if it wins. In exchange it adds atomics per task, a last-workgroup reset of the counters, graph invalidation when the queue is rebuilt, and extra device allocations.

```diff
diff --git a/epic_amd/csrc/driver.h b/epic_amd/csrc/driver.h
--- a/epic_amd/csrc/driver.h
+++ b/epic_amd/csrc/driver.h
@@ -116,6 +116,8 @@
     hipStream_t stream = nullptr;
     int rows_per_task = 0;
     int tuned_rows[3] = {0, 0, 0};
+    bool tuned_static[2] = {false, false};
+    epic_hip::FusedQueue fq;
     unsigned finish_from = 0;
     int math = 0;
     struct Replay { hipGraphExec_t exec; int cur_flip; double work; int tile_delta_n; };
@@ -145,6 +147,7 @@
         hipEvent_t ev_prev = nullptr, ev_band = nullptr, ev_comm = nullptr, ev_stage = nullptr;
         Track trk;
         Track trk_f;
+        epic_hip::FusedQueue fq;
         bool peer_up = true;
         float *bounce[2] = {nullptr, nullptr};
         int first() const { return g_top; }
@@ -206,6 +209,8 @@
 bool fuses_rb_tol(const Ctx *c);
 bool fuses_rb_precise(const Ctx *c);
 int jacobi_fused_rows_per_task(const Ctx *c);
+int fused_tail_rows(const Ctx *c, int tall);
+epic_hip::Activity fused_queue_act(Ctx *c,epic_hip::FusedQueue &q, int rows, int tall, hipStream_t stream);
 void tune_fused_rows(Ctx *c, int kind, unsigned iteration);
 epic_hip::TilePlan tile_plan(const Ctx *c);
 bool tile_checks(const Ctx *c, const epic_hip::TilePlan &tp);
diff --git a/epic_amd/csrc/driver_config.cpp b/epic_amd/csrc/driver_config.cpp
--- a/epic_amd/csrc/driver_config.cpp
+++ b/epic_amd/csrc/driver_config.cpp
@@ -79,6 +79,8 @@
     if (e && atoll(e) >= 0) c.fuse_min_cells = atoll(e);
     e = senv("EPIC_HIP_FUSED_ROWS");
     if (e && atoi(e) > 0) c.fused_rows = atoi(e);
+    e = senv("EPIC_HIP_FUSED_TAIL_ROWS");
+    if (e && atoi(e) >= 0) c.fused_tail_rows = atoi(e);
     c.tune = !sis_zero("EPIC_HIP_TUNE");
     c.tune_debug = sgiven("EPIC_HIP_TUNE_DEBUG");
     c.tile = !sis_zero("EPIC_HIP_TILE");
@@ -129,12 +131,12 @@
     out += dev;
     snprintf(t, sizeof t,
              "\", \"halo\": %d, \"no_peer\": %s, "
-             "\"threads\": %s, \"spin_us\": %d, \"no_fuse\": %s, \"no_graph\": %s, \"fuse_min_cells\": %lld, \"fused_rows\": %d, \"tune\": %s, "
+             "\"threads\": %s, \"spin_us\": %d, \"no_fuse\": %s, \"no_graph\": %s, \"fuse_min_cells\": %lld, \"fused_rows\": %d, \"fused_tail_rows\": %d, \"tune\": %s, "
              "\"tile\": %s, \"tile_max_cells\": %lld, \"tile_rows\": %d, \"tile_width\": %d, \"tile_halo\": %d, \"tile_pipeline\": %s, \"defer\": %s, "
              "\"track_pairs\": %s, \"track_pair_rows\": %d, \"track_switch\": %g, \"tol_finish\": %d, \"tol_finish_factor\": %g, "
              "\"flags\": %d, \"list_waves\": %zu, \"pair3d\": %s, \"pair3d_rows\": %d, \"march_x0\": %s}",
              halo, no_peer ? "true" : "false",
-             threads ? "true" : "false", spin_us, no_fuse ? "true" : "false", no_graph ? "true" : "false", fuse_min_cells, fused_rows,
+             threads ? "true" : "false", spin_us, no_fuse ? "true" : "false", no_graph ? "true" : "false", fuse_min_cells, fused_rows, fused_tail_rows,
              tune ? "true" : "false", tile ? "true" : "false", tile_max_cells, tile_rows, tile_width, tile_halo, tile_pipeline ? "true" : "false",
              defer ? "true" : "false",
              track_pairs ? "true" : "false", track_pair_rows, track_switch, tol_finish, (double)tol_finish_factor, launch.flags, launch.list_waves,
diff --git a/epic_amd/csrc/driver_config.h b/epic_amd/csrc/driver_config.h
--- a/epic_amd/csrc/driver_config.h
+++ b/epic_amd/csrc/driver_config.h
@@ -35,6 +35,7 @@
     bool no_graph = false;
     long long fuse_min_cells = -1;
     int fused_rows = 0;
+    int fused_tail_rows = -1;
     bool tune = true;
     bool tune_debug = false;
     bool tile = true;
diff --git a/epic_amd/csrc/driver_enqueue.hip b/epic_amd/csrc/driver_enqueue.hip
--- a/epic_amd/csrc/driver_enqueue.hip
+++ b/epic_amd/csrc/driver_enqueue.hip
@@ -135,8 +135,10 @@
         if (count >= 2) tune_fused_rows(c, 0, first);
         while (i < count) {
             if (count - i >= 2) {
+                const int rpt = jacobi_fused_rows_per_task(c);
+                const epic_hip::Activity qa = fused_queue_act(c, c->fq, c->rows, rpt, c->stream);
                 hipError_t e = epic_hip::launch_jacobi_fused_2d(c->buf[c->cur], c->buf[c->cur ^ 1], c->maskw, c->rows, c->pitch,
-                                                                jacobi_fused_rows_per_task(c), c->math, c->stream, -1, c->maskf());
+                                                                rpt, c->math, c->stream, -1, c->maskf(), qa.queue ? &qa : nullptr);
                 if (e != hipSuccess) return e;
                 c->cur ^= 1;
                 c->work_full += 2.0;
@@ -152,9 +154,11 @@
     if (!no_fuse && fuses_rb_tol(c) && count - i >= 2) tune_fused_rows(c, 1, first);
     if (fuse && count - i >= 2) tune_fused_rows(c, 2, first);
     while (!no_fuse && fuses_rb_tol(c) && count - i >= 2) {
+        const int rpt = jacobi_fused_rows_per_task(c);
+        const epic_hip::Activity qa = fused_queue_act(c, c->fq, c->rows, rpt, c->stream);
         hipError_t e = epic_hip::launch_jacobi_fused_2d(c->buf[c->cur], c->buf[c->cur ^ 1], c->maskw, c->rows, c->pitch,
-                                                        jacobi_fused_rows_per_task(c), c->math, c->stream, (int)((first + i) & 1u),
-                                                        c->maskf());
+                                                        rpt, c->math, c->stream, (int)((first + i) & 1u),
+                                                        c->maskf(), qa.queue ? &qa : nullptr);
         if (e != hipSuccess) return e;
         c->cur ^= 1;
         c->work_full += 2.0;
@@ -192,8 +196,9 @@
             act = c->trk_f.next(tiles, rpt, c->stream, nullptr);
         }
         const int parity = (int)((first + 2 * p) & 1u);
+        if (tol && !act.list_out) act = fused_queue_act(c, c->fq, c->rows, rpt, c->stream);
         e = tol ? epic_hip::launch_jacobi_fused_2d(c->buf[c->cur], c->buf[c->cur ^ 1], c->maskw, c->rows, c->pitch, rpt, c->math, c->stream,
-                                                   c->redblack ? parity : -1, c->maskf(), act.list_out ? &act : nullptr, check ? c->d_delta : nullptr)
+                                                   c->redblack ? parity : -1, c->maskf(), act.list_out || act.queue ? &act : nullptr, check ? c->d_delta : nullptr)
                 : epic_hip::launch_rb_fused_2d(c->buf[c->cur], c->buf[c->cur ^ 1], c->maskw, c->rows, c->pitch, rpt, c->math, parity, c->stream,
                                                c->maskf(), act.list_out ? &act : nullptr, check ? c->d_delta : nullptr);
         if (e != hipSuccess) return e;
@@ -219,6 +224,7 @@
     const auto key = std::make_tuple(2u * count + (check_last ? 1u : 0u), c->cur + 2 * (c->track ? 1 + c->trk.phase : 0), (int)(first & 1u), c->math,
                                      (int)c->redblack, auto_rows_per_task(c), fuse_cfg);
     if (c->graphs_broken) return enqueue_plain_run(c, count, first, check_last);
+    if (tp.halo == 0 && fuses_tol(c)) (void)fused_queue_act(c, c->fq, c->rows, jacobi_fused_rows_per_task(c), c->stream);
     auto it = c->graphs.find(key);
     if (it == c->graphs.end()) {
         const int cur0 = c->cur, phase0 = c->trk.phase, force0 = c->trk.force;
diff --git a/epic_amd/csrc/driver_multi.hip b/epic_amd/csrc/driver_multi.hip
--- a/epic_amd/csrc/driver_multi.hip
+++ b/epic_amd/csrc/driver_multi.hip
@@ -99,6 +99,7 @@
         if (sl.stream) (void)hipStreamSynchronize(sl.stream);
         if (sl.comm) (void)hipStreamSynchronize(sl.comm);
         for (float *&b : sl.buf) { if (b) (void)hipFree(b); b = nullptr; }
+        sl.fq.release();
     }
 }
 void multi_free_mask(Ctx *c)
@@ -376,7 +377,8 @@
             const int cur0 = c->cur;
             if (fuse && n_calm >= 2) tune_fused_rows(c, fuse_rb ? 2 : c->redblack ? 1 : 0, it0);
             const int fused_rpt = !fuse ? 0 : fuse_rb ? fused_rows_per_task(c) : jacobi_fused_rows_per_task(c);
-            hipError_t e = for_each_slab(c, [&, it0, chk, cur0, fused_rpt, n_calm](int k) -> hipError_t {
+            const int flags = epic_hip::process_launch_knobs().flags;
+            hipError_t e = for_each_slab(c, [&, it0, chk, cur0, fused_rpt, n_calm, flags](int k) -> hipError_t {
                 Ctx::Slab &sl = c->slabs[k];
                 int cur = cur0;
                 hipError_t e = hipSuccess;
@@ -384,10 +386,15 @@
                     const bool check = chk && i == 0;
                     if (fuse && !check && n_calm - i >= 2) {
                         const int parity = c->redblack ? (int)((it0 + i + (unsigned)sl.top()) & 1u) : -1;
+                        epic_hip::Activity qa = {nullptr, nullptr, nullptr, nullptr, nullptr, nullptr, nullptr, nullptr};
+                        const int tk = c->redblack ? 1 : 0;
+                        if (!fuse_rb && !(flags & 8) && !(c->tuned_static[tk] && c->tuned_rows[tk] == fused_rpt) &&
+                            epic_hip::fused_queue_prepare(sl.fq, sl.rows, c->pitch, fused_rpt, fused_tail_rows(c, fused_rpt), flags, sl.stream))
+                            qa.queue = &sl.fq;
                         e = fuse_rb ? epic_hip::launch_rb_fused_2d(sl.buf[cur], sl.buf[cur ^ 1], sl.maskw, sl.rows, c->pitch, fused_rpt, c->math,
                                                                    parity, sl.stream, c->maskf(sl))
                                     : epic_hip::launch_jacobi_fused_2d(sl.buf[cur], sl.buf[cur ^ 1], sl.maskw, sl.rows, c->pitch, fused_rpt,
-                                                                       c->math, sl.stream, parity, c->maskf(sl));
+                                                                       c->math, sl.stream, parity, c->maskf(sl), qa.queue ? &qa : nullptr);
                         cur ^= 1;
                         i += 2;
                         continue;
diff --git a/epic_amd/csrc/driver_plan.hip b/epic_amd/csrc/driver_plan.hip
--- a/epic_amd/csrc/driver_plan.hip
+++ b/epic_amd/csrc/driver_plan.hip
@@ -63,6 +63,24 @@
     if (tuned > 0) return tuned;
     const long long rows = c->multi() ? c->rows / (long long)c->slabs.size() : c->rows;
     return epic_hip::jacobi_fused_auto_rows((int)rows, c->pitch);
+}
+
+int fused_tail_rows(const Ctx *c, int tall)
+{
+    if (c->cfg.fused_tail_rows >= 0) return std::min(c->cfg.fused_tail_rows, tall);
+    return std::min(tall, std::max(8, tall / 4));
+}
+
+epic_hip::Activity fused_queue_act(Ctx *c, epic_hip::FusedQueue &q, int rows, int tall, hipStream_t stream)
+{
+    epic_hip::Activity act = {nullptr, nullptr, nullptr, nullptr, nullptr, nullptr, nullptr, nullptr};
+    const int flags = epic_hip::process_launch_knobs().flags;
+    if (flags & 8) return act;
+    if (c->tuned_static[c->redblack ? 1 : 0] && c->tuned_rows[c->redblack ? 1 : 0] == tall) return act;
+    bool replaced = false;
+    if (epic_hip::fused_queue_prepare(q, rows, c->pitch, tall, fused_tail_rows(c, tall), flags, stream, &replaced)) act.queue = &q;
+    if (replaced) drop_graphs(c);
+    return act;
 }
 
 void tune_fused_rows(Ctx *c, int kind, unsigned iteration)
@@ -86,37 +104,58 @@
     hipEvent_t e0 = nullptr, e1 = nullptr;
     if (hipEventCreate(&e0) != hipSuccess) return;
     if (hipEventCreate(&e1) != hipSuccess) { (void)hipEventDestroy(e0); return; }
-    auto launch = [&](int height) -> hipError_t {
+    auto launch = [&](int height, bool use_queue) -> hipError_t {
         if (kind == 2) return epic_hip::launch_rb_fused_2d(in, out, maskw, rows, c->pitch, height, c->math, 0, stream, maskf);
-        return epic_hip::launch_jacobi_fused_2d(in, out, maskw, rows, c->pitch, height, c->math, stream, kind == 1 ? 0 : -1, maskf);
+        epic_hip::Activity act = {nullptr, nullptr, nullptr, nullptr, nullptr, nullptr, nullptr, nullptr};
+        if (use_queue) act = fused_queue_act(c, multi ? c->slabs[0].fq : c->fq, rows, height, stream);
+        if (use_queue && !act.queue) return hipErrorUnknown;
+        return epic_hip::launch_jacobi_fused_2d(in, out, maskw, rows, c->pitch, height, c->math, stream, kind == 1 ? 0 : -1, maskf, act.queue ? &act : nullptr);
     };
-    auto timed = [&](int height, float *ms) -> bool {
-        if (launch(height) != hipSuccess) return false;
+    auto timed = [&](int height, bool use_queue, float *ms) -> bool {
+        if (launch(height, use_queue) != hipSuccess) return false;
         if (hipEventRecord(e0, stream) != hipSuccess) return false;
         for (int i = 0; i < 2; ++i)
-            if (launch(height) != hipSuccess) return false;
+            if (launch(height, use_queue) != hipSuccess) return false;
         return hipEventRecord(e1, stream) == hipSuccess && hipEventSynchronize(e1) == hipSuccess &&
                hipEventElapsedTime(ms, e0, e1) == hipSuccess;
     };
     static const int kCandidates[] = {20, 23, 26, 29, 32, 35, 38, 40, 41, 43, 46, 49, 52, 58, 64, 80, 96, 128};
     const bool say = c->cfg.tune_debug;
-    float best_ms = 0.0f, dflt_ms = 0.0f;
-    int best = 0;
-    bool ok = timed(dflt, &dflt_ms);
-    if (say && ok) fprintf(stderr, "[epic_hip tune] kind %d, %d x %d%s: rule %d rows %.1f us", kind, rows, c->cols, multi ? " (first slab)" : "", dflt, dflt_ms * 500.0f);
-    for (int r : kCandidates) {
-        if (!ok) break;
-        if (r == dflt || r > rows) continue;
-        float ms = 0.0f;
-        ok = timed(r, &ms);
-        if (say && ok) fprintf(stderr, ", %d: %.1f", r, ms * 500.0f);
-        if (ok && (best == 0 || ms < best_ms)) { best = r; best_ms = ms; }
+    const bool try_queue = kind != 2 && !(epic_hip::process_launch_knobs().flags & 8);
+    int choice = dflt;
+    float choice_ms = 0.0f;
+    bool ok = true, queue_won = false;
+    for (int pass = 0; pass < (try_queue ? 2 : 1) && ok; ++pass) {
+        const bool q = pass == 1;
+        float best_ms = 0.0f, dflt_ms = 0.0f;
+        int best = 0;
+        bool pass_ok = timed(dflt, q, &dflt_ms);
+        if (say && pass_ok) fprintf(stderr, "[epic_hip tune] kind %d, %d x %d%s, %s: rule %d rows %.1f us", kind, rows, c->cols, multi ? " (first slab)" : "", q ? "queue" : "static", dflt, dflt_ms * 500.0f);
+        for (int r : kCandidates) {
+            if (!pass_ok) break;
+            if (r == dflt || r > rows) continue;
+            float ms = 0.0f;
+            pass_ok = timed(r, q, &ms);
+            if (say && pass_ok) fprintf(stderr, ", %d: %.1f", r, ms * 500.0f);
+            if (pass_ok && (best == 0 || ms < best_ms)) { best = r; best_ms = ms; }
+        }
+        if (say) fprintf(stderr, "\n");
+        if (!pass_ok) {
+            (void)hipGetLastError();
+            if (!q) ok = false;
+            break;
+        }
+        const bool cand = best > 0 && best_ms < 0.99f * dflt_ms;
+        const int pick = cand ? best : dflt;
+        const float pick_ms = cand ? best_ms : dflt_ms;
+        if (!q) { choice = pick; choice_ms = pick_ms; }
+        else if (pick_ms < 0.99f * choice_ms) { choice = pick; choice_ms = pick_ms; queue_won = true; }
     }
-    if (say) fprintf(stderr, "\n");
     (void)hipEventDestroy(e0);
     (void)hipEventDestroy(e1);
-    if (!ok) { (void)hipGetLastError(); return; }
-    c->tuned_rows[kind] = (best > 0 && best_ms < 0.99f * dflt_ms) ? best : dflt;
+    if (!ok) return;
+    c->tuned_rows[kind] = choice;
+    if (kind != 2) c->tuned_static[kind] = try_queue && !queue_won;
 }
 
 epic_hip::TilePlan tile_plan(const Ctx *c)
diff --git a/epic_amd/csrc/driver_registry.hip b/epic_amd/csrc/driver_registry.hip
--- a/epic_amd/csrc/driver_registry.hip
+++ b/epic_amd/csrc/driver_registry.hip
@@ -67,6 +67,7 @@
             drop_graphs(c);
             if (c->multi()) multi_destroy(c);
             for (float *&b : c->buf) { if (b) (void)hipFree(b); b = nullptr; }
+            c->fq.release();
             free_spare(c);
             if (c->maskw) (void)hipFree(c->maskw);
             if (c->d_m) (void)hipFree(c->d_m);
@@ -292,6 +293,7 @@
     c->ahead.live = false;
     drop_graphs(c);
     for (float *&b : c->buf) { if (b) (void)hipFree(b); b = nullptr; }
+    c->fq.release();
     free_spare(c);
     if (c->multi()) { DeviceGuard g; multi_free_u(c); }
     dims_into_ctx(harmonic, c);
@@ -347,6 +349,7 @@
             }
             b = nullptr;
         }
+        c->fq.release();
         free_spare(c);
     }
     harmonic->d_u = nullptr;
diff --git a/epic_amd/csrc/fused_schedule.h b/epic_amd/csrc/fused_schedule.h
--- /dev/null
+++ b/epic_amd/csrc/fused_schedule.h
@@ -0,0 +1,71 @@
+#pragma once
+#include <algorithm>
+#include <vector>
+
+namespace epic_hip {
+
+constexpr int kFusedBands = 8;
+
+inline int fused_tighten(int rows, int nstrips, int height, int round_waves, int waves_per_block, int *q, int *rem)
+{
+    int nchunks = (rows + height - 1) / height;
+    *q = height;
+    *rem = 0;
+    if (round_waves <= 0 || nstrips <= 0) return nchunks;
+    const long long blocks = ((long long)nchunks * nstrips + waves_per_block - 1) / waves_per_block;
+    const long long round_blocks = round_waves / waves_per_block;
+    if (round_blocks <= 0) return nchunks;
+    const long long rounds = (blocks + round_blocks - 1) / round_blocks;
+    long long n = rounds * round_waves / nstrips;
+    n = std::min<long long>(n, rows / std::max(8, height / 2));
+    if (n <= nchunks) return nchunks;
+    *q = rows / (int)n;
+    *rem = rows % (int)n;
+    return (int)n;
+}
+
+struct FusedSchedule {
+    std::vector<int> row_start;
+    int band_chunk[kFusedBands + 1];
+    int tall_chunks;
+    int nchunks() const { return (int)row_start.size() - 1; }
+};
+
+inline FusedSchedule fused_schedule(int rows, int nstrips, int resident_waves, int tall, int tail, int round_waves, int waves_per_block)
+{
+    FusedSchedule s;
+    s.tall_chunks = 0;
+    s.row_start.push_back(0);
+    if (tail <= 0) {
+        int q = tall, rem = 0;
+        const int n = fused_tighten(rows, nstrips, tall, round_waves, waves_per_block, &q, &rem);
+        for (int k = 0, r = 0; k < n; ++k) {
+            r = std::min(rows, r + q + (k < rem ? 1 : 0));
+            s.row_start.push_back(r);
+        }
+        for (int b = 0; b <= kFusedBands; ++b) s.band_chunk[b] = (int)((long long)n * b / kFusedBands);
+        return s;
+    }
+    tail = std::min(tail, tall);
+    const int tall_total = (int)std::min<long long>(resident_waves / nstrips, rows / tall);
+    int row = 0;
+    for (int b = 0; b < kFusedBands; ++b) {
+        s.band_chunk[b] = s.nchunks();
+        int left = rows / kFusedBands + (b < rows % kFusedBands ? 1 : 0);
+        const int nt = std::min(tall_total / kFusedBands + (b < tall_total % kFusedBands ? 1 : 0), left / tall);
+        for (int k = 0; k < nt; ++k) s.row_start.push_back(row += tall);
+        s.tall_chunks += nt;
+        left -= nt * tall;
+        const int k = std::max(1, (2 * left + tall + tail - 1) / (tall + tail));
+        for (int j = 0; left > 0; ++j) {
+            int h = j < k ? tall - (int)(((long long)(tall - tail) * (2 * j + 1) + k) / (2 * k)) : tail;
+            h = std::min(std::max(h, tail), left);
+            s.row_start.push_back(row += h);
+            left -= h;
+        }
+    }
+    s.band_chunk[kFusedBands] = s.nchunks();
+    return s;
+}
+
+}
diff --git a/epic_amd/csrc/kernels.h b/epic_amd/csrc/kernels.h
--- a/epic_amd/csrc/kernels.h
+++ b/epic_amd/csrc/kernels.h
@@ -4,7 +4,11 @@
 #include <stdint.h>
 #include <stdlib.h>
 
+#include <algorithm>
+#include <vector>
+
 #include "driver_config.h"
+#include "fused_schedule.h"
 
 namespace epic_hip {
 
@@ -19,6 +23,7 @@
     uint32_t *queued_in;
     uint32_t *queued_out;
     unsigned long long *total;
+    const struct FusedQueue *queue = nullptr;
 };
 inline size_t sweep_2d_tiles(int rows, int pitch, int rows_per_task)
 {
@@ -61,6 +66,64 @@
 hipError_t launch_jacobi_fused_2d(const float *in, float *out, const uint32_t *maskw, int rows, int pitch, int rows_per_task,
                                   int math, hipStream_t stream, int parity = -1, const uint32_t *maskf = nullptr,
                                   const Activity *act = nullptr, unsigned *delta_bits = nullptr, int check_begin = -1, int check_end = -1);
+constexpr int kFusedTableHead = 16, kFusedCounterStride = 32, kFusedQueueWords = (2 * kFusedBands + 1) * kFusedCounterStride;
+struct FusedQueue {
+    int *table = nullptr;
+    unsigned *words = nullptr;
+    int nchunks = 0;
+    int rows = 0, pitch = 0, tall = 0, tail = 0, resident_waves = 0, round_waves = 0;
+    void release()
+    {
+        if (table) (void)hipFree(table);
+        if (words) (void)hipFree(words);
+        table = nullptr;
+        words = nullptr;
+        nchunks = rows = 0;
+    }
+};
+inline bool fused_queue_prepare(FusedQueue &q, int rows, int pitch, int tall, int tail, int flags, hipStream_t stream, bool *replaced = nullptr)
+{
+    if (replaced) *replaced = false;
+    if (rows <= 0 || pitch <= 0 || tall <= 0) return false;
+    const long long max_rows = 0x7fffffffLL / ((long long)pitch * 4) - 8;
+    if (max_rows < 1) return false;
+    tall = (int)std::min<long long>(tall, max_rows);
+    tail = std::max(0, std::min(tail, tall));
+    const int resident_waves = resident_blocks_of(nullptr) * 4;
+    int dev = 0, cus = 0;
+    if (resident_waves <= 0 || hipGetDevice(&dev) != hipSuccess || hipDeviceGetAttribute(&cus, hipDeviceAttributeMultiprocessorCount, dev) != hipSuccess || cus < 1) {
+        (void)hipGetLastError();
+        return false;
+    }
+    const int round_waves = (flags & 4) ? cus * 4 : 0;
+    if (q.table && q.rows == rows && q.pitch == pitch && q.tall == tall && q.tail == tail && q.resident_waves == resident_waves &&
+        q.round_waves == round_waves)
+        return true;
+    hipStreamCaptureStatus cap = hipStreamCaptureStatusNone;
+    if (hipStreamIsCapturing(stream, &cap) != hipSuccess || cap != hipStreamCaptureStatusNone || hipStreamSynchronize(stream) != hipSuccess) {
+        (void)hipGetLastError();
+        return false;
+    }
+    if (replaced) *replaced = q.table != nullptr;
+    q.release();
+    const int nstrips = fused_2d_strips(pitch);
+    const FusedSchedule s = fused_schedule(rows, nstrips, resident_waves, tall, tail, round_waves, 4);
+    if ((long long)s.nchunks() * nstrips > 0x7fffffffLL) return false;
+    std::vector<int> host(kFusedTableHead + s.row_start.size(), 0);
+    for (int b = 0; b <= kFusedBands; ++b) host[b] = s.band_chunk[b] * nstrips;
+    std::copy(s.row_start.begin(), s.row_start.end(), host.begin() + kFusedTableHead);
+    const std::vector<unsigned> zeros(kFusedQueueWords, 0u);
+    if (hipMalloc((void **)&q.table, host.size() * sizeof(int)) != hipSuccess || hipMalloc((void **)&q.words, kFusedQueueWords * sizeof(unsigned)) != hipSuccess ||
+        hipMemcpy(q.table, host.data(), host.size() * sizeof(int), hipMemcpyHostToDevice) != hipSuccess ||
+        hipMemcpy(q.words, zeros.data(), zeros.size() * sizeof(unsigned), hipMemcpyHostToDevice) != hipSuccess) {
+        (void)hipGetLastError();
+        q.release();
+        return false;
+    }
+    q.nchunks = s.nchunks();
+    q.rows = rows; q.pitch = pitch; q.tall = tall; q.tail = tail; q.resident_waves = resident_waves; q.round_waves = round_waves;
+    return true;
+}
 inline size_t mask_words_fused_2d(int rows, int pitch) { return (size_t)rows * (size_t)fused_2d_strips(pitch) * 8u; }
 hipError_t launch_fuse_masks_2d(const uint32_t *maskw, int rows, int pitch, uint32_t *maskf, hipStream_t stream);
 hipError_t launch_eval_math(const float *in, float *out, size_t n, int which, hipStream_t stream);
diff --git a/epic_amd/csrc/kernels_2d.hip b/epic_amd/csrc/kernels_2d.hip
--- a/epic_amd/csrc/kernels_2d.hip
+++ b/epic_amd/csrc/kernels_2d.hip
@@ -48,6 +48,7 @@
     int nblocks;
     int check_lo, check_hi;
 };
+static_assert(kNumXcd == kFusedBands, "one band of the queue's schedule per XCD");
 
 __device__ __forceinline__ int xcd_contiguous_block(int b, int nblk)
 {
@@ -508,6 +509,8 @@
 template <bool RB, bool FMASK, bool TRACK = false, bool CHECK = false>
 __device__ __forceinline__ void tol_fused_pass(const Sweep2dArgs &a, TolLnEntry *math_lds)
 {
+    __shared__ unsigned wg_left;
+    if (!TRACK && threadIdx.x == 0) wg_left = 0;
     TolLn<4>::stage(math_lds);
     const TolLnEntry *const tl = math_lds;
     const int lane = threadIdx.x & (kWave - 1);
@@ -517,9 +520,54 @@
     WakeCursor cursor = {};
     float dmax = 0.0f;
     const bool have_work = !listed || wake_begin(a.wake, lane, wave, kWavesPerBlock, cursor);
+    const bool queued = !TRACK && a.wake.count_zero != nullptr;
+    typedef const __attribute__((address_space(4))) int ci32;
+    ci32 *const q_table = (ci32 *)a.wake.count_in;
+    unsigned *const q_words = a.wake.count_zero;
+    int band = 0, moves = 0;
+    unsigned ticket = 0;
+    if (queued) {
+        band = (int)(blockIdx.x % kNumXcd);
+        ticket = (blockIdx.x / kNumXcd) * kWavesPerBlock + (unsigned)wave;
+    }
+    auto uniform = [](int v) -> int { return __builtin_amdgcn_readfirstlane(v); };
+    auto band_first = [&](int b) -> unsigned { return (gridDim.x + (unsigned)(kNumXcd - 1 - b)) / kNumXcd * kWavesPerBlock; };
+    auto grab = [&](int b) -> unsigned {
+        unsigned v = 0;
+        if (lane == 0) v = __hip_atomic_fetch_add(q_words + b * kFusedCounterStride, 1u, __ATOMIC_RELAXED, __HIP_MEMORY_SCOPE_AGENT);
+        return v;
+    };
+    auto bands_with_tickets = [&]() -> unsigned {
+        bool has = false;
+        if (lane < kNumXcd) {
+            const unsigned seen = __hip_atomic_load(q_words + lane * kFusedCounterStride, __ATOMIC_RELAXED, __HIP_MEMORY_SCOPE_AGENT);
+            has = seen + band_first(lane) < (unsigned)(a.wake.count_in[lane + 1] - a.wake.count_in[lane]);
+        }
+        return (unsigned)__builtin_amdgcn_ballot_w64(has) & ((1u << kNumXcd) - 1u);
+    };
     if (have_work)
     for (int vb = blockIdx.x;;) {
-    int task;
+    int task = 0;
+    unsigned next_ticket = 0;
+    if (!TRACK) vb = uniform(vb);
+    if (queued) {
+        bool none = false;
+        for (;;) {
+            band = uniform(band);
+            moves = uniform(moves);
+            ticket = (unsigned)uniform((int)ticket);
+            const unsigned t0 = (unsigned)q_table[band], t1 = (unsigned)q_table[band + 1];
+            if (ticket < t1 - t0) { task = (int)(t0 + ticket); break; }
+            if (++moves > kNumXcd) { none = true; break; }
+            const unsigned open = bands_with_tickets() & ~(1u << band);
+            if (open == 0) { none = true; break; }
+            const unsigned ahead = open >> (band + 1), wrapped = open & ((2u << band) - 1u);
+            band = ahead ? band + 1 + __builtin_ctz(ahead) : __builtin_ctz(wrapped);
+            ticket = (unsigned)__builtin_amdgcn_readfirstlane((int)grab(band)) + band_first(band);
+        }
+        if (none) break;
+        next_ticket = grab(band);
+    } else {
     if (listed) task = wake_tile(a.wake, cursor);
     else task = xcd_contiguous_block(vb, a.nblocks) * kWavesPerBlock + wave;
     if (task >= a.ntasks) {
@@ -528,11 +576,13 @@
         if (vb >= a.nblocks) break;
         continue;
     }
+    }
+    if (!TRACK) task = uniform(task);
     if (TRACK && lane == 0) a.wake.queued_in[task] = 0;
     const int strip = task % a.nstrips;
     const int chunk = task / a.nstrips;
-    const int r0 = a.row_begin + chunk * a.rows_per_task + min(chunk, a.chunk_rem);
-    const int r1 = min(r0 + a.rows_per_task + (chunk < a.chunk_rem ? 1 : 0), a.row_end);
+    const int r0 = queued ? a.row_begin + q_table[kFusedTableHead + chunk] : a.row_begin + chunk * a.rows_per_task + min(chunk, a.chunk_rem);
+    const int r1 = queued ? a.row_begin + q_table[kFusedTableHead + chunk + 1] : min(r0 + a.rows_per_task + (chunk < a.chunk_rem ? 1 : 0), a.row_end);
     const int col = fused_2d_col(strip, lane);
     const int lcol = min(col, a.pitch - kColsPerLane);
     const bool owner = fused_2d_owns(strip, lane, col, a.pitch);
@@ -654,6 +704,7 @@
     su[0] = tol_split4(u[3]);
     m[1] = level(u[1], u[2], u[3], su[1], su[2], su[0], k[1], odd_cols_of(r0, 0), r0, false, true);
     sm[1] = tol_split4(m[1]);
+    if (queued) ticket = (unsigned)__builtin_amdgcn_readfirstlane((int)next_ticket) + band_first(band);
     const int nrows = r1 - r0;
     for (int i = 0; i < nrows; i += kTrip) {
         auto step = [&](auto jc) {
@@ -690,7 +741,16 @@
         wake_push(a.wake, t, want && lane < 9);
     }
     if (listed) { if (!wake_next(cursor)) break; }
-    else { vb += gridDim.x; if (vb >= a.nblocks) break; }
+    else if (!queued) { vb += gridDim.x; if (vb >= a.nblocks) break; }
+    }
+    if (queued && lane == 0 &&
+        __hip_atomic_fetch_add(&wg_left, 1u, __ATOMIC_ACQ_REL, __HIP_MEMORY_SCOPE_WORKGROUP) == kWavesPerBlock - 1) {
+        const unsigned group = blockIdx.x % kNumXcd, in_group = (gridDim.x + (kNumXcd - 1 - group)) / kNumXcd;
+        const unsigned groups = min(gridDim.x, (unsigned)kNumXcd);
+        unsigned *const left_all = q_words + kNumXcd * kFusedCounterStride, *const left_group = left_all + (1 + group) * kFusedCounterStride;
+        if (__hip_atomic_fetch_add(left_group, 1u, __ATOMIC_ACQ_REL, __HIP_MEMORY_SCOPE_AGENT) == in_group - 1 &&
+            __hip_atomic_fetch_add(left_all, 1u, __ATOMIC_ACQ_REL, __HIP_MEMORY_SCOPE_AGENT) == groups - 1)
+            for (int w = 0; w < 2 * kNumXcd + 1; ++w) __hip_atomic_store(q_words + w * kFusedCounterStride, 0u, __ATOMIC_RELAXED, __HIP_MEMORY_SCOPE_AGENT);
     }
     if (CHECK) {
         dmax = wave_max(dmax);
@@ -831,6 +891,7 @@
 {
     static std::mutex mu;
     static std::map<std::pair<int, const void *>, int> cache;
+    if (!kernel) kernel = (const void *)jacobi_fused2d_kernel<kMathTol, true>;
     int dev = 0;
     const int cus = current_device_cus(&dev);
     std::lock_guard<std::mutex> lk(mu);
@@ -851,14 +912,7 @@
     if (!(a.flags & 4)) return;
     const int cus = current_device_cus();
     if (cus <= 0 || a.nstrips <= 0) return;
-    const long long blocks = ((long long)a.nchunks * a.nstrips + kWavesPerBlock - 1) / kWavesPerBlock;
-    const long long per_cu = (blocks + cus - 1) / cus;
-    long long n = per_cu * cus * kWavesPerBlock / a.nstrips;
-    n = std::min<long long>(n, rows / std::max(8, a.rows_per_task / 2));
-    if (n <= a.nchunks) return;
-    a.nchunks = (int)n;
-    a.rows_per_task = rows / (int)n;
-    a.chunk_rem = rows % (int)n;
+    a.nchunks = fused_tighten(rows, a.nstrips, a.rows_per_task, cus * kWavesPerBlock, kWavesPerBlock, &a.rows_per_task, &a.chunk_rem);
 }
 
 hipError_t launch_eval_math(const float *in, float *out, size_t n, int which, hipStream_t stream)
@@ -1048,10 +1102,18 @@
     a.nstrips = fused_2d_strips(pitch);
     a.nchunks = (rows + rows_per_task - 1) / rows_per_task;
     a.flags = sweep_flags();
-    if (!act) tighten_chunks(a, rows);
+    const FusedQueue *queue = act && !act->list_out ? act->queue : nullptr;
+    if (queue && (!queue->table || !queue->words || queue->rows != rows || queue->pitch != pitch || queue->nchunks < 1 || (a.flags & 8))) queue = nullptr;
+    if (queue) a.nchunks = queue->nchunks;
+    else if (!act || !act->list_out) tighten_chunks(a, rows);
+    if ((long long)a.nstrips * a.nchunks > 0x7fffffffLL) return hipErrorInvalidValue;
     a.ntasks = a.nstrips * a.nchunks;
     a.parity = parity < 0 ? 0 : parity & 1;
     a.wake = wake_args(act, (size_t)a.ntasks);
+    if (queue) {
+        a.wake.count_in = reinterpret_cast<const uint32_t *>(queue->table);
+        a.wake.count_zero = queue->words;
+    }
     a.nblocks = (a.ntasks + kWavesPerBlock - 1) / kWavesPerBlock;
     a.maskf = maskf;
     const bool track = a.wake.list_out != nullptr, check = delta_bits != nullptr, rb = parity >= 0;
```

Result: no change. 768,500 (-0.3%).
